# gau-nernst/llama-x

Hardware: AMD Instinct MI355X
Metric: train tokens/sec Llama-3.1-8B seq4096 at 1/2/4/8 MI355X; p50 step ms (higher is better)
Workload: dtype bf16; 1 GPU; Llama-3.1-8B text-only LoRA r=16 bf16, seq=4096, 1 sequence per GPU, causal mask, base+LM head frozen (BASELINE.json configs[1]); random-init weights at 8B dimensions; seq_len=4096, parallelism=dp1, launch=hipGraph replay (fwd+bwd+AdamW), lm_head_rows=labelled only

## Files before the change

### include/llx.h

```cpp
#ifndef LLX_H
#define LLX_H

#include <stdint.h>

#ifdef __cplusplus
extern "C" {
#endif

typedef void* llx_stream_t;

int llx_version(void);
const char* llx_last_error_string(void);
int llx_device_info(int device, char* name, int len);

int llx_rmsnorm_fwd(const void* x, const void* w, void* y, float* rstd, int64_t rows, int64_t dim, float eps, llx_stream_t s);
int llx_rmsnorm_fwd_quant(const void* x, const void* w, void* y, float* rstd, void* q, int64_t ldq, void* qscale, int64_t rows, int64_t dim,
                          float eps, llx_stream_t s);
int64_t llx_rmsnorm_bwd_workspace_bytes(int64_t rows, int64_t dim);
int llx_rmsnorm_bwd(const void* dy, const void* x, const void* w, const float* rstd, void* dx, void* dw ,
                    int dw_accumulate, void* workspace, const void* dres ,
                    int64_t rows, int64_t dim, llx_stream_t s);

int llx_gemm_nt_bf16(const void* A, int64_t lda, const void* B, int64_t ldb, void* C, int64_t ldc, int64_t M, int64_t N, int64_t K,
                     const void* A2, int64_t lda2, const void* B2, int64_t ldb2, int64_t K2, int epilogue, const void* E, int64_t lde,
                     llx_stream_t s);
int llx_gemm_nt_bf16_rows(const void* A, int64_t lda, const void* B, int64_t ldb, void* C, int64_t ldc, int64_t M, int64_t N, int64_t K,
                          const void* A2, int64_t lda2, const void* B2, int64_t ldb2, int64_t K2, int epilogue, const void* E, int64_t lde,
                          const int32_t* m_valid, llx_stream_t s);
int llx_gemm_nt_bf16_splitk(const void* A, int64_t lda, const void* B, int64_t ldb, float* partial, int64_t M, int64_t N, int64_t K, int splits,
                            const int32_t* m_valid, llx_stream_t s);
int llx_splitk_combine(const float* partial, int splits, int64_t M, int64_t N, const int32_t* inv, const float* scale, void* out, int64_t ld_out,
                       llx_stream_t s);
int llx_gemm_nt_bf16_rope(const void* A, int64_t lda, const void* B, int64_t ldb, void* C, int64_t ldc, int64_t M, int64_t N, int64_t K,
                          const void* A2, int64_t lda2, const void* B2, int64_t ldb2, int64_t K2, const float* rope_table, int64_t rope_S,
                          int64_t rope_cols, llx_stream_t s);

int llx_gemm_tn_bf16(const void* A, int64_t lda, const void* B, int64_t ldb, void* C, int64_t ldc, int64_t M, int64_t N1, int64_t N2,
                     llx_stream_t s);
int llx_gemm_tn_bf16_rows(const void* A, int64_t lda, const void* B, int64_t ldb, void* C, int64_t ldc, int64_t M, int64_t N1, int64_t N2,
                          const int32_t* m_valid, llx_stream_t s);

int llx_int8_mm_dequant(const void* A, int64_t lda, const void* B, int64_t ldb, void* C, int64_t ldc, int64_t M, int64_t N, int64_t K,
                        const void* a_scale, const void* b_scale, llx_stream_t s);
int llx_int8_mm_dequant_f32(const void* A, int64_t lda, const void* B, int64_t ldb, float* C, int64_t ldc, int64_t M, int64_t N, int64_t K,
                            const float* a_scale, const float* b_scale, llx_stream_t s);
int llx_int8_mm_dequant_ext(const void* A, int64_t lda, const void* B, int64_t ldb, void* C, int64_t ldc, int64_t M, int64_t N, int64_t K,
                            const void* a_scale, const void* b_scale, const void* A2, int64_t lda2, const void* B2, int64_t ldb2, int64_t K2,
                            int epilogue, const void* E, int64_t lde, const float* rope_table, int64_t rope_S, int64_t rope_cols,
                            llx_stream_t s);

int llx_quantize_int8_rowwise(const void* x, int64_t ldx, void* q, int64_t ldq, void* scale, int64_t rows, int64_t cols, int is_f32,
                              llx_stream_t s);

int64_t llx_attn_flags_bytes(int64_t B, int64_t S);
int llx_attn_tile_flags(const int* doc_ids, const int* prefix_len, void* flags, int64_t B, int64_t S, llx_stream_t s);
int llx_attn_fwd(const void* q, int64_t q_sb, int64_t q_ss, const void* k, int64_t k_sb, int64_t k_ss, const void* v, int64_t v_sb,
                 int64_t v_ss, void* o, int64_t o_sb, int64_t o_ss, float* lse, const int* doc_ids, const int* prefix_len,
                 const void* flags, int64_t B, int64_t S, int64_t H, int64_t KVH, int64_t head_dim, float scale, llx_stream_t s);
int64_t llx_attn_bwd_workspace_bytes(int64_t B, int64_t S, int64_t H, int64_t KVH);
int64_t llx_attn_bwd_ds_bytes(int64_t B, int64_t S, int64_t H);
int llx_attn_bwd(const void* q, int64_t q_sb, int64_t q_ss, const void* k, int64_t k_sb, int64_t k_ss, const void* v, int64_t v_sb,
                 int64_t v_ss, const void* o, int64_t o_sb, int64_t o_ss, const void* d_o, int64_t do_sb, int64_t do_ss, const float* lse,
                 float* delta , void* dq, int64_t dq_sb, int64_t dq_ss, void* dk, int64_t dk_sb, int64_t dk_ss,
                 void* dv, int64_t dv_sb, int64_t dv_ss, const int* doc_ids, const int* prefix_len, const void* flags,
                 const float* rope ,
                 void* ds ,
                 int64_t B, int64_t S, int64_t H, int64_t KVH, int64_t head_dim, float scale, llx_stream_t s);

int llx_attn_fwd_dropout(const void* q, int64_t q_sb, int64_t q_ss, const void* k, int64_t k_sb, int64_t k_ss, const void* v, int64_t v_sb,
                         int64_t v_ss, void* o, int64_t o_sb, int64_t o_ss, float* lse, const int* doc_ids, const int* prefix_len,
                         const void* flags, int64_t B, int64_t S, int64_t H, int64_t KVH, int64_t head_dim, float scale, int64_t threshold,
                         const void* rng, int64_t stream_id, llx_stream_t s);
int llx_attn_bwd_dropout(const void* q, int64_t q_sb, int64_t q_ss, const void* k, int64_t k_sb, int64_t k_ss, const void* v, int64_t v_sb,
                         int64_t v_ss, const void* o, int64_t o_sb, int64_t o_ss, const void* d_o, int64_t do_sb, int64_t do_ss,
                         const float* lse, float* delta, void* dq, int64_t dq_sb, int64_t dq_ss, void* dk, int64_t dk_sb, int64_t dk_ss,
                         void* dv, int64_t dv_sb, int64_t dv_ss, const int* doc_ids, const int* prefix_len, const void* flags,
                         const float* rope, void* ds, int64_t B, int64_t S, int64_t H, int64_t KVH, int64_t head_dim, float scale,
                         int64_t threshold, const void* rng, int64_t stream_id, llx_stream_t s);
int llx_attn_dropout_keep(void* keep, int64_t B, int64_t H, int64_t Sq, int64_t Skv, int64_t threshold, const void* rng, int64_t stream_id,
                          llx_stream_t s);

int llx_attn_dense_fwd(const void* q, int64_t q_sb, int64_t q_sh, int64_t q_ss, const void* k, int64_t k_sb, int64_t k_sh, int64_t k_ss,
                       const void* v, int64_t v_sb, int64_t v_sh, int64_t v_ss, void* o, int64_t o_sb, int64_t o_sh, int64_t o_ss,
                       const void* mask, int64_t m_sb, int64_t m_sh, int64_t m_sq, int64_t B, int64_t H, int64_t KVH, int64_t Sq, int64_t Skv,
                       int64_t head_dim, float scale, llx_stream_t s);

int64_t llx_attn_mask_flags_bytes(int64_t B, int64_t Sq, int64_t Skv);
int llx_attn_mask_tile_flags(const void* mask, int64_t m_sb, int64_t m_sq, void* flags, int64_t B, int64_t Sq, int64_t Skv, llx_stream_t s);
int llx_attn_mask_fwd(const void* q, int64_t q_sb, int64_t q_ss, const void* k, int64_t k_sb, int64_t k_sh, int64_t k_ss, const void* v,
                      int64_t v_sb, int64_t v_sh, int64_t v_ss, void* o, int64_t o_sb, int64_t o_ss, float* lse ,
                      const void* mask, int64_t m_sb, int64_t m_sq, const void* flags, int64_t B, int64_t Sq, int64_t Skv, int64_t H,
                      int64_t KVH, int64_t head_dim, float scale, llx_stream_t s);

int llx_attn_mask_bwd(const void* q, int64_t q_sb, int64_t q_ss, const void* k, int64_t k_sb, int64_t k_ss, const void* v, int64_t v_sb,
                      int64_t v_ss, const void* o, int64_t o_sb, int64_t o_ss, const void* d_o, int64_t do_sb, int64_t do_ss,
                      const float* lse, float* delta , void* dq, int64_t dq_sb,
                      int64_t dq_ss, void* dk, int64_t dk_sb, int64_t dk_ss, void* dv, int64_t dv_sb, int64_t dv_ss, const void* mask,
                      int64_t m_sb, int64_t m_sq, const void* flags, const float* rope , int64_t B,
                      int64_t S, int64_t H, int64_t KVH, int64_t head_dim, float scale, llx_stream_t s);

int llx_gemv_bf16(const void* w0, int64_t ldw0, int64_t n0, const void* w1, int64_t ldw1, int64_t n1, const void* w2, int64_t ldw2, int64_t n2,
                  const void* x, int64_t ldx, int64_t M, int64_t K, const void* norm_w, float eps, int epilogue, void* out, int64_t ldo,
                  const void* res, int64_t ldr, const float* rope, int64_t n_q, int64_t n_k, void* k_cache, void* v_cache, int64_t c_sh,
                  int64_t c_ss, const int64_t* input_pos, const void* bext0, const void* bext1, const void* bext2, int64_t rank0, int64_t rank1,
                  int64_t rank2, const void* t, int64_t ldt, float lora_scale, llx_stream_t s);
int llx_gemv_i8(const void* w0, int64_t ldw0, int64_t n0, const void* w1, int64_t ldw1, int64_t n1, const void* w2, int64_t ldw2, int64_t n2,
                const void* x, int64_t ldx, int64_t M, int64_t K, const void* norm_w, float eps, int epilogue, void* out, int64_t ldo,
                const void* res, int64_t ldr, const float* rope, int64_t n_q, int64_t n_k, void* k_cache, void* v_cache, int64_t c_sh,
// ... 19 lines not shown
                         int64_t c_sh, int64_t c_ss, int64_t Smax, const int64_t* pos, void* workspace, int64_t workspace_bytes, llx_stream_t s);
int64_t llx_gemm_rows16_i8_workspace_bytes(int64_t M, int64_t N, int64_t K, int epilogue);
int llx_gemm_rows16_i8(const void* w0, int64_t ldw0, int64_t n0, const void* w1, int64_t ldw1, int64_t n1, const void* w2, int64_t ldw2, int64_t n2,
                       const void* x, int64_t ldx, int64_t M, int64_t K, const void* norm_w, float eps, int epilogue, void* out, int64_t ldo,
                       const void* res, int64_t ldr, const float* rope, int64_t n_q, int64_t n_k, void* k_cache, void* v_cache, int64_t c_sb,
                       int64_t c_sh, int64_t c_ss, int64_t Smax, const int64_t* pos, void* workspace, int64_t workspace_bytes,
                       const void* scale0, const void* scale1, const void* scale2, llx_stream_t s);
int llx_gemm_rows16_bf16_lora(const void* w0, int64_t ldw0, int64_t n0, const void* w1, int64_t ldw1, int64_t n1, const void* w2, int64_t ldw2,
                              int64_t n2, const void* x, int64_t ldx, int64_t M, int64_t K, const void* norm_w, float eps, int epilogue, void* out,
                              int64_t ldo, const void* res, int64_t ldr, const float* rope, int64_t n_q, int64_t n_k, void* k_cache, void* v_cache,
                              int64_t c_sb, int64_t c_sh, int64_t c_ss, int64_t Smax, const int64_t* pos, void* workspace, int64_t workspace_bytes,
                              const void* bext0, const void* bext1, const void* bext2, int64_t rank0, int64_t rank1, int64_t rank2, const void* t,
                              int64_t ldt, float lora_scale, const void* colscale0, const void* colscale1, const void* colscale2, llx_stream_t s);
int llx_gemm_rows16_i8_lora(const void* w0, int64_t ldw0, int64_t n0, const void* w1, int64_t ldw1, int64_t n1, const void* w2, int64_t ldw2,
                            int64_t n2, const void* x, int64_t ldx, int64_t M, int64_t K, const void* norm_w, float eps, int epilogue, void* out,
                            int64_t ldo, const void* res, int64_t ldr, const float* rope, int64_t n_q, int64_t n_k, void* k_cache, void* v_cache,
                            int64_t c_sb, int64_t c_sh, int64_t c_ss, int64_t Smax, const int64_t* pos, void* workspace, int64_t workspace_bytes,
                            const void* scale0, const void* scale1, const void* scale2, const void* bext0, const void* bext1, const void* bext2,
                            int64_t rank0, int64_t rank1, int64_t rank2, const void* t, int64_t ldt, float lora_scale, llx_stream_t s);
int64_t llx_attn_decode_workspace_bytes(int64_t B, int64_t H, int64_t M, int64_t nsplit);
int llx_attn_decode(const void* q, int64_t q_sb, int64_t q_sh, int64_t q_ss, const void* k_cache, const void* v_cache, int64_t c_sb, int64_t c_sh,
                    int64_t c_ss, void* o, int64_t o_sb, int64_t o_sh, int64_t o_ss, const void* mask, int64_t m_sb, int64_t m_sh, int64_t m_sq,
                    const int* extent, float* workspace, int64_t B, int64_t H, int64_t KVH, int64_t M, int64_t Skv, int64_t nsplit,
                    int64_t head_dim, float scale, llx_stream_t s);

int llx_rope(const void* x, int64_t x_sb, int64_t x_ss, void* y, int64_t y_sb, int64_t y_ss, const float* table, int64_t B, int64_t S,
             int64_t nheads, int64_t head_dim, int backward, llx_stream_t s);

int llx_swiglu_fwd(const void* g, int64_t g_ld, const void* u, int64_t u_ld, void* h, int64_t h_ld, int64_t rows, int64_t cols, llx_stream_t s);
int llx_swiglu_bwd(const void* dh, int64_t dh_ld, const void* g, int64_t g_ld, const void* u, int64_t u_ld, void* dg, int64_t dg_ld,
                   void* du, int64_t du_ld, int64_t rows, int64_t cols, llx_stream_t s);

int llx_embedding_fwd(const int64_t* ids, const void* table, void* out, int64_t n_tok, int64_t dim, int64_t vocab, int64_t tok_per_batch,
                      int64_t out_sb, int64_t out_ss, llx_stream_t s);
int llx_embedding_bwd(const int64_t* ids, const void* dy, float* dtable_f32, int64_t n_tok, int64_t dim, int64_t vocab,
                      int64_t tok_per_batch, int64_t dy_sb, int64_t dy_ss, llx_stream_t s);

int64_t llx_ce_workspace_bytes(int64_t T);
int llx_ce_fwd_bwd(const void* logits, int64_t ld, void* dlogits, int64_t dld, const int64_t* labels, float* loss, void* workspace,
                   int64_t T, int64_t V, llx_stream_t s);
int llx_head_compact_index(const int64_t* labels, int32_t* idx, int32_t* inv, int64_t* labels_c, int32_t* count, int64_t T, llx_stream_t s);
int llx_gather_rows(const void* src, int64_t ld_src, const int32_t* idx, const int32_t* count, void* dst, int64_t ld_dst, int64_t T, int64_t D,
                    llx_stream_t s);
int llx_scatter_rows(const void* src, int64_t ld_src, const int32_t* inv, const float* scale , void* dst, int64_t ld_dst,
                     int64_t T, int64_t D, llx_stream_t s);
int llx_ce_fwd_bwd_rows(const void* logits, int64_t ld, void* dlogits, int64_t dld, const int64_t* labels, float* loss, void* workspace,
                        int64_t T, int64_t V, const int32_t* rows, llx_stream_t s);
int llx_ce_fwd_bwd_part(const void* logits, int64_t ld, void* dlogits, int64_t dld, const int64_t* labels, float* loss, void* workspace, int64_t T,
                        int64_t V, int64_t row0, int64_t nrows, const int32_t* rows, int phase, llx_stream_t s);

int llx_logprob_rows_fwd(const void* logits, int64_t ld, const int64_t* labels, float* logp, float* lse, int32_t* top1 ,
                         int64_t T, int64_t V, const int32_t* rows , llx_stream_t s);
int llx_logprob_rows_bwd(const void* logits, int64_t ld, void* dlogits, int64_t dld, const int64_t* labels, const float* lse, const float* g,
                         int64_t T, int64_t V, const int32_t* rows , llx_stream_t s);
int llx_logprob_map_rows(const int32_t* map, const float* src_f, float* dst_f, float fill_f, const int32_t* src_i ,
                         int32_t* dst_i , int32_t fill_i, int64_t T, llx_stream_t s);

int llx_skinny_nt(const void* X, int64_t ldx, const void* W, int64_t ldw, void* out, int64_t M, int64_t K, int64_t R,
                  const int32_t* kranges , llx_stream_t s);
int llx_skinny_nt_scaled(const void* X, int64_t ldx, const void* W, int64_t ldw, void* out, int64_t M, int64_t K, int64_t R,
                         const int32_t* kranges, const void* colscale, void* G, int64_t ldg, llx_stream_t s);
int llx_rmsnorm_skinny_nt(const void* x, const void* g, const void* W, int64_t ldw, void* y, float* rstd, void* t, int64_t M, int64_t D,
                          int64_t R, float eps, llx_stream_t s);
int64_t llx_skinny_tn_workspace_bytes(int64_t M, int64_t N, int64_t R);
int llx_skinny_tn(const void* U, const void* Y, int64_t ldy, void* out, int64_t out_ld, int64_t M, int64_t N, int64_t R, float scale,
                  int transpose_out, int accumulate, void* workspace,
                  const int32_t* segs , int seg_count, llx_stream_t s);
int llx_skinny_tn_partial(const void* U, const void* Y, int64_t ldy, int64_t M, int64_t N, int64_t R, void* workspace, const int32_t* segs,
                          int seg_count, llx_stream_t s);
int llx_skinny_tn_partial_many(int n, const void* const* U, const void* const* Y, const int64_t* ldy, const int64_t* M, const int64_t* N,
                               const int64_t* R, void* const* workspaces, const int32_t* const* segs, const int* seg_count, llx_stream_t s);
int64_t llx_skinny_u_workspace_bytes(int64_t M, int64_t N);
int llx_skinny_tn_partial_many_u(int n, const void* const* U, const void* const* Y, const int64_t* ldy, const int64_t* M, const int64_t* N,
                                 const int64_t* R, void* const* workspaces, const int32_t* const* segs, const int* seg_count,
                                 const void* const* Bt, const int64_t* ldb, void* const* upart, llx_stream_t s);
int llx_skinny_u_reduce(const void* upart, void* out, int64_t M, int64_t N, int64_t R, const int32_t* segs, int seg_count, llx_stream_t s);
int llx_skinny_tn_partial_many_us(int n, const void* const* U, const void* const* Y, const int64_t* ldy, const int64_t* M, const int64_t* N,
                                  const int64_t* R, void* const* workspaces, const int32_t* const* segs, const int* seg_count,
                                  const void* const* Bt, const int64_t* ldb, void* const* upart, const void* const* colscale,
                                  void* const* G, const int64_t* ldg, llx_stream_t s);
int llx_skinny_tn_reduce_many(int n, const void* const* workspaces, void* const* outs, const int64_t* out_ld, const int64_t* M, const int64_t* N,
                              const int64_t* R, const float* scale, const int* transpose_out, const int* accumulate,
                              const int32_t* const* segs, const int* seg_count, llx_stream_t s);
int llx_pad64(const void* in, int64_t ld, void* out, int64_t R, int64_t C, float scale, int transpose, llx_stream_t s);
int llx_lora_group_pack(const void* const* lora_a, const void* const* lora_b, const int64_t* Ns, const int64_t* ranks, int nm, int64_t K,
                        float scale, void* a_cat, void* b2, void* bT, void* a2t, llx_stream_t s);
int llx_lora_groups_pack(const void* const* lora_a, const void* const* lora_b, const int64_t* Ns, const int64_t* ranks, const int* nm,
                         const int64_t* K, const float* scale, void* const* a_cat, void* const* b2, void* const* bT, void* const* a2t, int ng,
                         llx_stream_t s);
int llx_lora_pack(const void* in, int64_t ld, void* out, int64_t out_ld, int64_t R, int64_t C, int64_t row_off, int64_t col_off, float scale,
                  int transpose, llx_stream_t s);

int llx_rownorm2(const void* W, int64_t ld, float* out, int64_t rows, int64_t cols, llx_stream_t s);
int llx_dora_colscale(const float* wn2, const void* G , const void* b2 , const void* AAt ,
                      const void* m , void* c , float* inv_norm , int64_t N, int64_t R, llx_stream_t s);
int64_t llx_colsum_mul_workspace_bytes(int64_t N);
int llx_colsum_mul(const void* a, int64_t lda, const void* b, int64_t ldb, const float* colscale , void* out ,
                   void* workspace, int64_t M, int64_t N, llx_stream_t s);
int llx_colscale_bias(const void* x, int64_t x_ld, void* y, int64_t y_ld, const void* colscale , const void* bias ,
                      int64_t rows, int64_t cols, llx_stream_t s);

int llx_mel_spectrogram(const float* audio, int64_t B, int64_t L, const float* twiddle, const float* window, const float* fbank, float* mel,
                        int64_t n_frames, int64_t hop, int64_t n_mels, llx_stream_t s);
int llx_logmel_cmn(const float* mel, void* feat , int64_t B, int64_t n_frames, int64_t n_mels, llx_stream_t s);
int llx_gelu_fwd(const void* z, int64_t z_ld, void* y, int64_t y_ld, int64_t rows, int64_t cols, llx_stream_t s);
int llx_gelu_bwd(const void* dy, int64_t dy_ld, const void* z, int64_t z_ld, void* dz, int64_t dz_ld, int64_t rows, int64_t cols, llx_stream_t s);
int llx_col2im3(const void* dA, void* dpad, int64_t M, int64_t C, int64_t P, int64_t stride, llx_stream_t s);
int llx_conv_w_reorder(const void* in, void* out, int64_t D, int64_t C, int to_gemm, llx_stream_t s);

int llx_sample_rows(const void* logits, int dtype, int64_t ld, int64_t R, int64_t V, float temperature, int64_t top_k, float top_p,
                    uint64_t seed, int64_t* pos, int64_t* token_out, int64_t* history, int64_t hist_ld, int64_t hist_cap, int64_t hist_base,
                    int advance, int64_t eos_id, int32_t* finished, float* aux_u, float* aux_thresh, int32_t* aux_kept, llx_stream_t s);

int llx_sample_rows_ext(const void* logits, int dtype, int64_t ld, int64_t R, int64_t V, float temperature, int64_t top_k, float top_p,
                        uint64_t seed, int64_t* pos, int64_t* token_out, int64_t* history, int64_t hist_ld, int64_t hist_cap, int64_t hist_base,
                        int advance, int64_t eos_id, int32_t* finished, float* aux_u, float* aux_thresh, int32_t* aux_kept, int32_t* counts,
                        int64_t ldc, float repetition_penalty, float presence_penalty, float frequency_penalty, float* logprob_history,
                        llx_stream_t s);

int llx_lookup_step(const int64_t* picks, int64_t* seq, int64_t cap, int64_t* len, int64_t* step_tok, int64_t* step_pos, int32_t* finished,
                    int64_t* counters, int64_t P, int64_t n, int k, int g, int64_t eos_id, int init, llx_stream_t s);

int llx_beam_rows(const void* logits, int dtype, int64_t ld, int64_t W, int64_t V, float* cand_score, int32_t* cand_token, llx_stream_t s);
int llx_beam_merge(const float* cand_score, const int32_t* cand_token, float* s, int32_t* parent, int64_t* tok, int64_t* hist, int64_t hist_ld,
                   int64_t* bank_tok, int64_t bank_ld, int32_t* bank_len, float* bank_score, int32_t* meta, int64_t W, int64_t n,
                   int64_t eos_id, float length_penalty, int init, llx_stream_t stream);
int llx_kv_reorder_rows(const void* const* table, int64_t n_caches, int64_t sb, int64_t sh, int64_t ss, const int32_t* parent, int64_t W,
                        int64_t KVH, int64_t len, int64_t Smax, int64_t head_dim, llx_stream_t s);

int llx_scale(const void* x, int64_t x_ld, void* y, int64_t y_ld, const float* dev_scalar, float host_scale, const void* colscale,
              int64_t rows, int64_t cols, llx_stream_t s);
int llx_add(const void* x, const void* y, void* z, int64_t n, llx_stream_t s);
int llx_transpose(const void* in, int64_t in_ld, void* out, int64_t out_ld, int64_t R, int64_t C, int src_is_i8, llx_stream_t s);
int llx_i8_to_bf16(const void* in, void* out, int64_t n, llx_stream_t s);

#ifdef __cplusplus
}
#endif
#endif
```

### llama-x_amd/csrc/common.h

```cpp
#pragma once
#include <hip/hip_runtime.h>
#include <stdint.h>
#include <stdarg.h>
#include <stdio.h>

#define LLX_OK 0
#define LLX_ERR_ARG -1
#define LLX_ERR_LAUNCH -2
#define LLX_ERR_UNSUPPORTED -3

void llx_set_error(const char* fmt, ...);

#define LLX_REQUIRE(cond, ...)            \
  do {                                    \
    if (!(cond)) {                        \
      llx_set_error(__VA_ARGS__);         \
      return LLX_ERR_ARG;                 \
    }                                     \
  } while (0)

#define LLX_LAUNCH_CHECK(name)                                              \
  do {                                                                      \
    hipError_t e__ = hipGetLastError();                                     \
    if (e__ != hipSuccess) {                                                \
// ... 110 lines not shown
      const float uu = p ? bfhi(uv[e]) : bflo(uv[e]);
      const float dd = p ? bfhi(dv[e]) : bflo(dv[e]);
      const float sg = sigmoidf_(gg);
      const float silu = bf2f(f2bf(gg * sg));
      dus[p] = dd * silu;
      const float ds = bf2f(f2bf(dd * uu));
      dgs[p] = ds * (sg * (1.f + gg * (1.f - sg)));
    }
    og[e] = pack_bf2(dgs[0], dgs[1]);
    ou[e] = pack_bf2(dus[0], dus[1]);
  }
}

__device__ __forceinline__ u32x4_t rope8(const u32x4_t& v, const f32x4_t& t0, const f32x4_t& t1, float sign) {
  const float cs[4] = {t0[0], t0[2], t1[0], t1[2]};
  const float sn[4] = {t0[1] * sign, t0[3] * sign, t1[1] * sign, t1[3] * sign};
  u32x4_t o;
#pragma unroll
  for (int e = 0; e < 4; ++e) {
    const float x0 = bflo(v[e]), x1 = bfhi(v[e]);
    o[e] = pack_bf2(x0 * cs[e] - x1 * sn[e], x1 * cs[e] + x0 * sn[e]);
  }
  return o;
}

__device__ __forceinline__ u32x4_t rope8(const u32x4_t& v, const float* __restrict__ tp, float sign) {
  const f32x4_t t0 = *reinterpret_cast<const f32x4_t*>(tp);
  const f32x4_t t1 = *reinterpret_cast<const f32x4_t*>(tp + 4);
  const float cs[4] = {t0[0], t0[2], t1[0], t1[2]};
  const float sn[4] = {t0[1] * sign, t0[3] * sign, t1[1] * sign, t1[3] * sign};
  u32x4_t o;
#pragma unroll
  for (int e = 0; e < 4; ++e) {
    const float x0 = bflo(v[e]), x1 = bfhi(v[e]);
    o[e] = pack_bf2(x0 * cs[e] - x1 * sn[e], x1 * cs[e] + x0 * sn[e]);
  }
  return o;
}

typedef __attribute__((ext_vector_type(8))) short llx_s16x8_t;
template <int OFF>
__device__ __forceinline__ void lds_tr_read(s16x4_t& dst, uint32_t addr) {
  asm volatile("ds_read_b64_tr_b16 %0, %1 offset:%2" : "=v"(dst) : "v"(addr), "n"(OFF));
}
__device__ __forceinline__ void lds_tr_read_rt(s16x4_t& dst, uint32_t addr, int off) {
  asm volatile("ds_read_b64_tr_b16 %0, %1 offset:%2" : "=v"(dst) : "v"(addr), "n"(off));
}
template <int N>
__device__ __forceinline__ void lds_tr_wait4(s16x4_t& a, s16x4_t& b, s16x4_t& c, s16x4_t& d) {
  asm volatile("s_waitcnt lgkmcnt(%4)" : "+v"(a), "+v"(b), "+v"(c), "+v"(d) : "n"(N));
  __builtin_amdgcn_sched_barrier(0);
}
template <int N>
__device__ __forceinline__ void lds_tr_wait8(s16x4_t (&c)[4], s16x4_t (&d)[4]) {
  asm volatile("s_waitcnt lgkmcnt(%8)" : "+v"(c[0]), "+v"(c[1]), "+v"(c[2]), "+v"(c[3]), "+v"(d[0]), "+v"(d[1]), "+v"(d[2]), "+v"(d[3]) : "n"(N));
  __builtin_amdgcn_sched_barrier(0);
}
__device__ __forceinline__ void lds_read16_rt(i32x4_t& dst, uint32_t addr, int off) {
  asm volatile("ds_read_b128 %0, %1 offset:%2" : "=v"(dst) : "v"(addr), "n"(off));
}
template <typename T>
__device__ __forceinline__ void lds_pin1(T& x) { asm volatile("" : "+v"(x)); }
template <typename T, int N>
__device__ __forceinline__ void lds_pin1(T (&x)[N]) {
#pragma unroll
  for (int i = 0; i < N; ++i) asm volatile("" : "+v"(x[i]));
}
template <typename... T>
__device__ __forceinline__ void lds_pin(T&... x) {
  (lds_pin1(x), ...);
  __builtin_amdgcn_sched_barrier(0);
}
template <int N, typename... T>
__device__ __forceinline__ void lds_wait(T&... x) {
  asm volatile("s_waitcnt lgkmcnt(%0)" : : "n"(N));
  (lds_pin1(x), ...);
  __builtin_amdgcn_sched_barrier(0);
}
__device__ __forceinline__ bf16x8_t frag_of(const s16x4_t& lo, const s16x4_t& hi) {
  const llx_s16x8_t v = {lo[0], lo[1], lo[2], lo[3], hi[0], hi[1], hi[2], hi[3]};
  return __builtin_bit_cast(bf16x8_t, v);
}

typedef __attribute__((address_space(3))) void llx_lds_void;
__device__ __forceinline__ __amdgpu_buffer_rsrc_t lds_dma_rsrc(const void* base, uint32_t bytes) {
  return __builtin_amdgcn_make_buffer_rsrc(const_cast<void*>(base), 0, (int)bytes, 0x00020000);
}
__device__ __forceinline__ void lds_dma16(__amdgpu_buffer_rsrc_t rsrc, llx_lds_void* dst, uint32_t lane_off, uint32_t wave_off) {
  __builtin_amdgcn_raw_ptr_buffer_load_lds(rsrc, dst, 16, (int)lane_off, (int)wave_off, 0, 0);
}
```

### llama-x_amd/csrc/gemm_bf16.hip

```cpp
#include "common.h"
#include <type_traits>
#include <mutex>

#define BM 256
#define BN 256
#define BK 64
#define STAGE_BYTES (2 * 256 * BK * 2)
#define A_TILE_BYTES (256 * BK * 2)
#define EPI_ROW_BYTES 528
#define GEMM_LDS_BYTES (256 * EPI_ROW_BYTES)

enum { EPI_NONE = 0, EPI_RESIDUAL = 1, EPI_BIAS = 2, EPI_BIAS_GELU = 3, EPI_COLSCALE = 4, EPI_ROWCOLSCALE = 5, EPI_SWIGLU_BWD = 6, EPI_SWIGLU_FWD = 7, EPI_ROPE = 8, EPI_SPLITK = 9, EPI_ROWCOLSCALE_F32 = 10 };

struct GemmArgs {
  const bf16_t* A; const bf16_t* B; bf16_t* C;
  const bf16_t* A2; const bf16_t* B2;
  const bf16_t* E;
  const bf16_t* E2;
  int64_t lda, ldb, ldc, lde, lda2, ldb2;
  int M, N, K, K2;
  int grid_m, grid_n;
  int col0, col_end;
  const bf16_t* sa; const bf16_t* sb;
  const float* rope;
  int rope_S, rope_cols;
  const int* m_valid;
  float* C32;
  int splits;
};

typedef __attribute__((address_space(3))) void lds_void;
typedef const __attribute__((address_space(1))) void gbl_void;

__device__ __forceinline__ float gelu_erf(float x) { return 0.5f * x * (1.0f + erff(x * 0.70710678118654752440f)); }

template <int EPI, bool I8, int PIPE, int BNT = 256>
__global__ __launch_bounds__(512, 2) void gemm_nt_kernel(const GemmArgs g) {
  static_assert(BNT == 256 || BNT == 128, "tile width");
  static_assert(PIPE == 1, "the four-phase main loop is the only one");
  static_assert(BNT == 256 || EPI != EPI_SWIGLU_FWD, "the SwiGLU-forward epilogue needs the full tile");
  constexpr int ESZ = I8 ? 1 : 2;
  constexpr int TK = 128 / ESZ;
  constexpr int WNG = BNT / 64;
  constexpr int WR = 256 / (8 / WNG);
  constexpr int MI = WR / 16;
  constexpr int MH = MI / 2;
  constexpr int BSI = BNT / 64;
  constexpr int EROW = BNT * 2 + 16;
  extern __shared__ __attribute__((aligned(16))) char smem[];
  const int tid = threadIdx.x;
  const int lane = tid & 63;
  const int wave = __builtin_amdgcn_readfirstlane(tid >> 6);
  const int wm = wave / WNG, wn = wave % WNG;

  int grid_m = g.grid_m;
  if (g.m_valid != nullptr) grid_m = min(grid_m, (*g.m_valid + BM - 1) / BM);
  const int nsplit = EPI == EPI_SPLITK ? g.splits : 1;
  const int nwg = grid_m * g.grid_n * nsplit;
  int bid = blockIdx.x;
  if (bid >= nwg) return;
  {
    const int q = nwg >> 3, r = nwg & 7, x = bid & 7;
    bid = (x < r ? x * (q + 1) : r * (q + 1) + (x - r) * q) + (bid >> 3);
  }
  const int split = EPI == EPI_SPLITK ? bid / (grid_m * g.grid_n) : 0;
  if constexpr (EPI == EPI_SPLITK) bid -= split * (grid_m * g.grid_n);
  const int GROUP_M = 4;
  const int width = GROUP_M * g.grid_n;
  const int group = bid / width;
  const int gsz = min(grid_m - group * GROUP_M, GROUP_M);
  const int pid_m = group * GROUP_M + ((bid % width) % gsz);
  const int pid_n = (bid % width) / gsz;
  constexpr bool SPLITN = EPI == EPI_SWIGLU_FWD;
  const int halfN = g.N >> 1;
  const int m0 = pid_m * BM, n0 = SPLITN ? pid_n * (BN / 2) : g.col0 + pid_n * BNT;
  auto col_of = [&](int nl) { return SPLITN ? (nl < BN / 2 ? n0 + nl : halfN + n0 + nl - BN / 2) : min(n0 + nl, g.col_end - 1); };

  const int srow = tid >> 3;
  const int schunk = (tid & 7) ^ ((tid >> 4) & 7);
  int arow[4], brow[4];
#pragma unroll
  for (int i = 0; i < 4; ++i) {
    arow[i] = min(m0 + i * 64 + srow, g.M - 1);
    brow[i] = SPLITN ? (i < 2 ? n0 + i * 64 + srow : halfN + n0 + (i - 2) * 64 + srow) : min(n0 + (i % BSI) * 64 + srow, g.col_end - 1);
  }
  const int nk1 = g.K / TK / nsplit;
  const int nk = nk1 + g.K2 / 64;
  const int kofs = split * nk1;

  uint32_t aoff[4], boff[4];
#pragma unroll
  for (int i = 0; i < 4; ++i) {
    aoff[i] = (uint32_t)((int64_t)arow[i] * g.lda * ESZ + schunk * 16);
    boff[i] = (uint32_t)((int64_t)brow[i] * g.ldb * ESZ + schunk * 16);
  }
  const __amdgpu_buffer_rsrc_t rsA = lds_dma_rsrc(g.A, (uint32_t)(((int64_t)(g.M - 1) * g.lda + g.K) * ESZ));
  const __amdgpu_buffer_rsrc_t rsB = lds_dma_rsrc(g.B, (uint32_t)(((int64_t)(g.N - 1) * g.ldb + g.K) * ESZ));

  const int frow = lane & 15;
  const int fsw = (lane >> 1) & 7;
  const int fq = lane >> 4;
  const int a_base = (wm * WR + frow) * 128;
  const int b_base = (wn * 64 + frow) * 128;
  const int slot0 = ((0 * 4 + fq) ^ fsw) * 16;
  const int slot1 = ((1 * 4 + fq) ^ fsw) * 16;
  const uint32_t sbase = (uint32_t)(uintptr_t)(__attribute__((address_space(3))) char*)smem;
  const uint32_t fa0 = sbase + a_base + slot0, fa1 = sbase + a_base + slot1;
  const uint32_t fb0 = sbase + A_TILE_BYTES + b_base + slot0, fb1 = sbase + A_TILE_BYTES + b_base + slot1;
  constexpr bool EARLY_AHI = !I8;

  using acc_t = typename std::conditional<I8, i32x4_t, f32x4_t>::type;
  acc_t acc[MI][4];
#pragma unroll
  for (int i = 0; i < MI; ++i)
#pragma unroll
    for (int j = 0; j < 4; ++j) acc[i][j] = acc_t{0, 0, 0, 0};

  auto stage_q = [&](auto steady_tag, int kt, int which) {
    constexpr bool steady = decltype(steady_tag)::value;
    if constexpr (!steady) {
      if (kt >= nk) return;
    }
    const int half = which >> 1, hi = which & 1;
    const int np = half ? BSI / 2 : 2;
    char* sT = smem + (kt & 1) * STAGE_BYTES + half * A_TILE_BYTES + hi * np * 8192;
    if (steady || kt < nk1) {
      const uint32_t koff = (uint32_t)(kt + kofs) * 128;
#pragma unroll
      for (int j = 0; j < 2; ++j) {
        if (j < np) {
          if (half) lds_dma16(rsB, (llx_lds_void*)(sT + (j * 512 + wave * 64) * 16), boff[np * hi + j], koff);
          else lds_dma16(rsA, (llx_lds_void*)(sT + (j * 512 + wave * 64) * 16), aoff[2 * hi + j], koff);
        }
      }
    } else {
      const char* base = (const char*)(half ? g.B2 : g.A2) + (int64_t)(kt - nk1) * 128;
      const int64_t l = (half ? g.ldb2 : g.lda2) * 2;
#pragma unroll
      for (int j = 0; j < 2; ++j) {
        if (j < np) {
          const char* src = base + (int64_t)(half ? brow[np * hi + j] : arow[2 * hi + j]) * l + schunk * 16;
          __builtin_amdgcn_global_load_lds((gbl_void*)src, (lds_void*)(sT + (j * 512 + wave * 64) * 16), 16, 0, 0);
        }
      }
    }
  };
  auto mfma_t = [&](auto ext_tag, const i32x4_t& b, const i32x4_t& a, acc_t& c) {
    constexpr bool ext_phase = decltype(ext_tag)::value;
    if constexpr (I8) {
      if constexpr (ext_phase) {
        f32x4_t cf = __builtin_bit_cast(f32x4_t, c);
        cf = __builtin_amdgcn_mfma_f32_16x16x32_bf16(__builtin_bit_cast(bf16x8_t, b), __builtin_bit_cast(bf16x8_t, a), cf, 0, 0, 0);
        c = __builtin_bit_cast(acc_t, cf);
      } else {
        c = __builtin_amdgcn_mfma_i32_16x16x64_i8(b, a, c, 0, 0, 0);
      }
// ... 96 lines not shown
    if constexpr (!EARLY_AHI) {
#pragma unroll
      for (int m4 = 0; m4 < MH; ++m4) lds_read16_rt(af[0][m4], pa0, (MH + m4) * 16 * 128);
    }
#pragma unroll
    for (int m4 = 0; m4 < MH; ++m4) lds_read16_rt(af[1][m4], pa1, (MH + m4) * 16 * 128);
    __builtin_amdgcn_s_setprio(1);
    lds_wait<MH>(ah);
#pragma unroll
    for (int m4 = 0; m4 < MH; ++m4)
#pragma unroll
      for (int n2 = 0; n2 < 2; ++n2) mfma(bfr[0][2 + n2], ah[m4], acc[MH + m4][2 + n2]);
    pin_acc(MH, 2);
    lds_wait<0>(af[1]);
#pragma unroll
    for (int m4 = 0; m4 < MH; ++m4)
#pragma unroll
      for (int n2 = 0; n2 < 2; ++n2) mfma(bfr[1][2 + n2], af[1][m4], acc[MH + m4][2 + n2]);
    __builtin_amdgcn_s_setprio(0);
    asm volatile("" ::: "memory");
    __builtin_amdgcn_s_barrier();
    asm volatile("" ::: "memory");
    stage_q(steady_tag, kt + 2, 0);
    __builtin_amdgcn_s_setprio(1);
#pragma unroll
    for (int ks = 0; ks < 2; ++ks)
#pragma unroll
      for (int m4 = 0; m4 < MH; ++m4)
#pragma unroll
        for (int n2 = 0; n2 < 2; ++n2) mfma(bfr[ks][n2], ks ? af[1][m4] : ah[m4], acc[MH + m4][n2]);
    __builtin_amdgcn_s_setprio(0);
  };
  const int nk_main = I8 ? nk1 : nk;
  int kt = 0;
#pragma unroll 1
  for (; kt + 2 < nk1; ++kt) ktile(kt, std::false_type{}, std::true_type{});
#pragma unroll 1
  for (; kt < nk_main; ++kt) ktile(kt, std::false_type{}, std::false_type{});
  if constexpr (I8) {
    if (nk > nk1) {
      dequant_in_place();
      for (kt = nk1; kt < nk; ++kt) ktile(kt, std::true_type{}, std::false_type{});
    }
  }
  __syncthreads();

  if constexpr (EPI == EPI_SPLITK) {
    float* P = g.C32 + (int64_t)split * g.M * g.N;
#pragma unroll
    for (int mi = 0; mi < MI; ++mi) {
      const int gm = m0 + wm * WR + mi * 16 + frow;
#pragma unroll
      for (int ni = 0; ni < 4; ++ni) {
        const int gn = n0 + wn * 64 + ni * 16 + fq * 4;
        if (gm < g.M && gn < g.col_end) *reinterpret_cast<f32x4_t*>(P + (int64_t)gm * g.N + gn) = acc[mi][ni];
      }
    }
    return;
  }
  if constexpr (EPI == EPI_ROWCOLSCALE_F32) {
    static_assert(I8, "int8 kernel only");
    float* Cf = reinterpret_cast<float*>(g.C);
    const float* saf = reinterpret_cast<const float*>(g.sa);
    const float* sbf = reinterpret_cast<const float*>(g.sb);
#pragma unroll
    for (int mi = 0; mi < MI; ++mi) {
      const int gm = m0 + wm * WR + mi * 16 + frow;
      const float rs = saf[min(gm, g.M - 1)];
#pragma unroll
      for (int ni = 0; ni < 4; ++ni) {
        const int gn = n0 + wn * 64 + ni * 16 + fq * 4;
        if (gm < g.M && gn < g.col_end) {
          const f32x4_t cs = *reinterpret_cast<const f32x4_t*>(sbf + gn);
          f32x4_t c;
#pragma unroll
          for (int e = 0; e < 4; ++e) c[e] = ((float)acc[mi][ni][e] * rs) * cs[e];
          *reinterpret_cast<f32x4_t*>(Cf + (int64_t)gm * g.ldc + gn) = c;
        }
      }
    }
    return;
  }
  constexpr int NIT = BNT / 16;
  constexpr int EB0 = (EPI == EPI_SWIGLU_BWD || EPI == EPI_ROPE) ? 4 : 8;
  constexpr int EB = EB0 < NIT / 2 ? EB0 : NIT / 2;
  constexpr bool AUX = EPI == EPI_RESIDUAL || EPI == EPI_BIAS || EPI == EPI_BIAS_GELU || EPI == EPI_SWIGLU_BWD || EPI == EPI_ROPE || EPI == EPI_COLSCALE;
  auto load_aux = [&](int it0, u32x4_t (&aux0)[EB], u32x4_t (&aux1)[EB]) {
    if constexpr (AUX) {
#pragma unroll
      for (int j = 0; j < EB; ++j) {
        const int q = (it0 + j) * 512 + tid;
        const int row = q / (BNT / 8), cc = q % (BNT / 8);
        const int gmc = min(m0 + row, g.M - 1), gnc = min(n0 + cc * 8, g.col_end - 8);
        if constexpr (EPI == EPI_RESIDUAL) {
          aux0[j] = *reinterpret_cast<const u32x4_t*>(g.E + (int64_t)gmc * g.lde + gnc);
        } else if constexpr (EPI == EPI_SWIGLU_BWD) {
          aux0[j] = *reinterpret_cast<const u32x4_t*>(g.E + (int64_t)gmc * g.lde + gnc);
          aux1[j] = *reinterpret_cast<const u32x4_t*>(g.E + (int64_t)gmc * g.lde + g.N + gnc);
        } else if constexpr (EPI == EPI_ROPE) {
          const float* tp = g.rope + ((int64_t)(gmc % g.rope_S) * 64 + ((gnc & 127) >> 1)) * 2;
          aux0[j] = *reinterpret_cast<const u32x4_t*>(tp);
          aux1[j] = *reinterpret_cast<const u32x4_t*>(tp + 4);
        } else {
          aux0[j] = *reinterpret_cast<const u32x4_t*>(g.E + gnc);
        }
      }
    }
  };
  u32x4_t auxA0[EB], auxA1[EB], auxB0[EB], auxB1[EB];
  if constexpr (!SPLITN) load_aux(0, auxA0, auxA1);
  float sbv[4][4], rsv[MI];
  if constexpr (I8) {
    if (g.K2 <= 0) {
#pragma unroll
      for (int ni = 0; ni < 4; ++ni)
#pragma unroll
        for (int e = 0; e < 4; ++e) sbv[ni][e] = bf2f(g.sb[col_of(wn * 64 + ni * 16 + fq * 4 + e)]);
#pragma unroll
      for (int mi = 0; mi < MI; ++mi) rsv[mi] = bf2f(g.sa[min(m0 + wm * WR + mi * 16 + frow, g.M - 1)]);
    }
  }
#pragma unroll
  for (int mi = 0; mi < MI; ++mi) {
    const int m = wm * WR + mi * 16 + frow;
    float rs = 1.f;
    if constexpr (I8) rs = rsv[mi];
#pragma unroll
    for (int ni = 0; ni < 4; ++ni) {
      const int n = wn * 64 + ni * 16 + fq * 4;
      float c[4];
      if constexpr (I8) {
        if (g.K2 > 0) {
          const f32x4_t cf = __builtin_bit_cast(f32x4_t, acc[mi][ni]);
#pragma unroll
          for (int e = 0; e < 4; ++e) c[e] = cf[e];
        } else {
#pragma unroll
          for (int e = 0; e < 4; ++e) c[e] = ((float)acc[mi][ni][e] * rs) * sbv[ni][e];
        }
      } else {
#pragma unroll
        for (int e = 0; e < 4; ++e) c[e] = acc[mi][ni][e];
      }
      u32x2_t pk;
      pk[0] = pack_bf2(c[0], c[1]);
      pk[1] = pack_bf2(c[2], c[3]);
      *reinterpret_cast<u32x2_t*>(smem + m * EROW + n * 2) = pk;
    }
  }
  __syncthreads();
  if constexpr (SPLITN) {
    bf16_t* H = const_cast<bf16_t*>(g.E);
#pragma unroll 4
    for (int it = 0; it < 8; ++it) {
      const int q = it * 512 + tid;
      const int row = q >> 4, cc = q & 15;
      const int gm = m0 + row, gn = n0 + cc * 8;
      if (gm < g.M) {
        const u32x4_t gv = *reinterpret_cast<const u32x4_t*>(smem + row * EPI_ROW_BYTES + cc * 16);
        const u32x4_t uv = *reinterpret_cast<const u32x4_t*>(smem + row * EPI_ROW_BYTES + (cc + 16) * 16);
        *reinterpret_cast<u32x4_t*>(g.C + (int64_t)gm * g.ldc + gn) = gv;
        *reinterpret_cast<u32x4_t*>(g.C + (int64_t)gm * g.ldc + halfN + gn) = uv;
        *reinterpret_cast<u32x4_t*>(H + (int64_t)gm * g.lde + gn) = swiglu_fwd8(gv, uv);
      }
    }
    return;
  }
  auto combine = [&](int it0, const u32x4_t (&aux0)[EB], const u32x4_t (&aux1)[EB]) {
#pragma unroll
    for (int j = 0; j < EB; ++j) {
      const int q = (it0 + j) * 512 + tid;
      const int row = q / (BNT / 8), cc = q % (BNT / 8);
      const int gm = m0 + row, gn = n0 + cc * 8;
      if (gm < g.M && gn < g.col_end) {
        u32x4_t v = *reinterpret_cast<const u32x4_t*>(smem + row * EROW + cc * 16);
        if constexpr (EPI == EPI_RESIDUAL) {
          const u32x4_t r = aux0[j];
#pragma unroll
          for (int e = 0; e < 4; ++e) v[e] = pack_bf2(bflo(v[e]) + bflo(r[e]), bfhi(v[e]) + bfhi(r[e]));
        } else if constexpr (EPI == EPI_BIAS || EPI == EPI_BIAS_GELU) {
          const u32x4_t bb = aux0[j];
#pragma unroll
          for (int e = 0; e < 4; ++e) {
            float lo = bflo(v[e]) + bflo(bb[e]), hi = bfhi(v[e]) + bfhi(bb[e]);
            if constexpr (EPI == EPI_BIAS_GELU) {
              lo = gelu_erf(bf2f(f2bf(lo)));
              hi = gelu_erf(bf2f(f2bf(hi)));
            }
            v[e] = pack_bf2(lo, hi);
          }
        } else if constexpr (EPI == EPI_SWIGLU_BWD) {
          u32x4_t og, ou;
          swiglu_bwd8(v, aux0[j], aux1[j], og, ou);
          *reinterpret_cast<u32x4_t*>(g.C + (int64_t)gm * g.ldc + g.N + gn) = ou;
          v = og;
        } else if constexpr (EPI == EPI_ROPE) {
          if (gn < g.rope_cols) v = rope8(v, __builtin_bit_cast(f32x4_t, aux0[j]), __builtin_bit_cast(f32x4_t, aux1[j]), 1.f);
        } else if constexpr (EPI == EPI_COLSCALE) {
          const u32x4_t sc = aux0[j];
#pragma unroll
          for (int e = 0; e < 4; ++e) v[e] = pack_bf2(bflo(v[e]) * bflo(sc[e]), bfhi(v[e]) * bfhi(sc[e]));
        }
        *reinterpret_cast<u32x4_t*>(g.C + (int64_t)gm * g.ldc + gn) = v;
      }
    }
  };
  static_assert((NIT / EB) % 2 == 0, "the batches alternate between two register sets");
#pragma unroll 1
  for (int it0 = 0; it0 < NIT; it0 += 2 * EB) {
    load_aux(it0 + EB, auxB0, auxB1);
    combine(it0, auxA0, auxA1);
    if (it0 + 2 * EB < NIT) load_aux(it0 + 2 * EB, auxA0, auxA1);
    combine(it0 + EB, auxB0, auxB1);
  }
}

template <int EPI, bool I8, int BNT = 256>
static int launch_gemm_p(const GemmArgs& a, hipStream_t stream) {
  auto kern = gemm_nt_kernel<EPI, I8, 1, BNT>;
  static std::once_flag attr_once;
  static hipError_t attr_err = hipSuccess;
  std::call_once(attr_once, [&] { attr_err = hipFuncSetAttribute((const void*)kern, hipFuncAttributeMaxDynamicSharedMemorySize, GEMM_LDS_BYTES); });
  if (attr_err != hipSuccess) {
    llx_set_error("llx_gemm_nt_bf16: cannot raise dynamic LDS limit: %s", hipGetErrorString(attr_err));
    return LLX_ERR_LAUNCH;
  }
  hipLaunchKernelGGL(kern, dim3(a.grid_m * a.grid_n * (EPI == EPI_SPLITK ? a.splits : 1)), dim3(512), GEMM_LDS_BYTES, stream, a);
  LLX_LAUNCH_CHECK("llx_gemm_nt_bf16");
  return LLX_OK;
}

template <int EPI, bool I8 = false>
static int launch_gemm(const GemmArgs& a, hipStream_t stream) {
  if constexpr (EPI != EPI_SWIGLU_FWD) {
    const int tiles = a.grid_m * a.grid_n, tail = tiles % 256;
    if (a.col0 == 0 && a.col_end == a.N && a.N % 256 == 0 && tiles > 256 && tail > 0 && tail <= 128 && tail % a.grid_m == 0) {
      const int tail_cols = tail / a.grid_m * 256;
      GemmArgs full = a, half = a;
      full.col_end = a.N - tail_cols;
      full.grid_n = a.grid_n - tail / a.grid_m;
      half.col0 = a.N - tail_cols;
      half.grid_n = tail_cols / 128;
      const int rc = launch_gemm_p<EPI, I8, 256>(full, stream);
      if (rc != LLX_OK) return rc;
      return launch_gemm_p<EPI, I8, 128>(half, stream);
    }
  }
  return launch_gemm_p<EPI, I8>(a, stream);
}

static GemmArgs make_args(const void* A, int64_t lda, const void* B, int64_t ldb, void* C, int64_t ldc, int64_t M, int64_t N, int64_t K) {
  GemmArgs a = {};
  a.A = (const bf16_t*)A; a.B = (const bf16_t*)B; a.C = (bf16_t*)C;
  a.lda = lda; a.ldb = ldb; a.ldc = ldc;
  a.M = (int)M; a.N = (int)N; a.K = (int)K;
  a.grid_m = (int)cdiv64(M, BM); a.grid_n = (int)cdiv64(N, BN);
  a.col_end = (int)N;
  a.splits = 1;
  return a;
}

static int check_extent(const char* who, int64_t M, int64_t N, int64_t K, int64_t lda, int64_t ldb, int esz) {
  LLX_REQUIRE(M < (1 << 30) && N < (1 << 30) && K < (1 << 30), "%s: dimension too large", who);
  LLX_REQUIRE(M * lda * esz < (int64_t)4294967296 && N * ldb * esz < (int64_t)4294967296, "%s: operand larger than 4 GiB (32-bit tile offsets)", who);
  return LLX_OK;
}

static int gemm_nt_bf16_impl(const void* A, int64_t lda, const void* B, int64_t ldb, void* C, int64_t ldc, int64_t M,
                             int64_t N, int64_t K, const void* A2, int64_t lda2, const void* B2, int64_t ldb2, int64_t K2,
                             int epilogue, const void* E, int64_t lde, const float* rope, int64_t rope_S, int64_t rope_cols,
                             hipStream_t stream, const int32_t* m_valid = nullptr) {
  LLX_REQUIRE(A && B && C, "llx_gemm_nt_bf16: null pointer");
  LLX_REQUIRE(M > 0 && N > 0 && K > 0, "llx_gemm_nt_bf16: empty problem M=%lld N=%lld K=%lld", (long long)M, (long long)N, (long long)K);
  LLX_REQUIRE(K % BK == 0 && K2 % BK == 0, "llx_gemm_nt_bf16: K=%lld and K2=%lld must be multiples of 64", (long long)K, (long long)K2);
  LLX_REQUIRE(N % 8 == 0, "llx_gemm_nt_bf16: N=%lld must be a multiple of 8", (long long)N);
  LLX_REQUIRE(lda % 8 == 0 && ldb % 8 == 0 && ldc % 8 == 0, "llx_gemm_nt_bf16: row strides must be multiples of 8 elements");
  LLX_REQUIRE(((uintptr_t)A | (uintptr_t)B | (uintptr_t)C) % 16 == 0, "llx_gemm_nt_bf16: pointers must be 16-byte aligned");
  LLX_REQUIRE(K2 == 0 || (A2 && B2 && lda2 % 8 == 0 && ldb2 % 8 == 0 && ((uintptr_t)A2 | (uintptr_t)B2) % 16 == 0),
              "llx_gemm_nt_bf16: bad K-extension operands");
  LLX_REQUIRE(epilogue == EPI_NONE || epilogue == EPI_ROPE || (E && (uintptr_t)E % 16 == 0), "llx_gemm_nt_bf16: epilogue operand missing/unaligned");
  LLX_REQUIRE(epilogue != EPI_ROPE || (rope && (uintptr_t)rope % 16 == 0 && rope_S > 0 && rope_cols >= 0 && rope_cols <= N && rope_cols % 128 == 0),
              "llx_gemm_nt_bf16_rope: need an aligned fp32 table, rope_S > 0 and rope_cols a multiple of 128 within N");
  LLX_REQUIRE((epilogue != EPI_RESIDUAL && epilogue != EPI_SWIGLU_BWD) || lde % 8 == 0, "llx_gemm_nt_bf16: residual / gate|up stride must be a multiple of 8");
  LLX_REQUIRE(epilogue != EPI_SWIGLU_BWD || (lde >= 2 * N && ldc >= 2 * N), "llx_gemm_nt_bf16: the SwiGLU-backward epilogue reads E[M,2N] (gate|up) and writes C[M,2N] (dg|du)");
  if (const int rc = check_extent("llx_gemm_nt_bf16", M, N, K, lda, ldb, 2); rc != LLX_OK) return rc;
  GemmArgs a = make_args(A, lda, B, ldb, C, ldc, M, N, K);
  a.A2 = (const bf16_t*)A2; a.B2 = (const bf16_t*)B2; a.lda2 = lda2; a.ldb2 = ldb2; a.K2 = (int)K2;
  a.E = (const bf16_t*)E; a.lde = lde;
  a.rope = rope; a.rope_S = (int)rope_S; a.rope_cols = (int)rope_cols;
  a.m_valid = m_valid;
  switch (epilogue) {
    case EPI_NONE: return launch_gemm<EPI_NONE>(a, stream);
    case EPI_RESIDUAL: return launch_gemm<EPI_RESIDUAL>(a, stream);
    case EPI_BIAS: return launch_gemm<EPI_BIAS>(a, stream);
    case EPI_BIAS_GELU: return launch_gemm<EPI_BIAS_GELU>(a, stream);
    case EPI_COLSCALE: return launch_gemm<EPI_COLSCALE>(a, stream);
    case EPI_SWIGLU_BWD: return launch_gemm<EPI_SWIGLU_BWD>(a, stream);
    case EPI_ROPE: return launch_gemm<EPI_ROPE>(a, stream);
    case EPI_SWIGLU_FWD:
      LLX_REQUIRE(N % 256 == 0 && lde % 8 == 0, "llx_gemm_nt_bf16: the SwiGLU-forward epilogue needs N = 2I with I a multiple of 128");
      a.grid_n = (int)(N / 256);
      return launch_gemm<EPI_SWIGLU_FWD>(a, stream);
    default: llx_set_error("llx_gemm_nt_bf16: unknown epilogue %d", epilogue); return LLX_ERR_UNSUPPORTED;
  }
}

extern "C" int llx_gemm_nt_bf16(const void* A, int64_t lda, const void* B, int64_t ldb, void* C, int64_t ldc, int64_t M,
                                int64_t N, int64_t K, const void* A2, int64_t lda2, const void* B2, int64_t ldb2, int64_t K2,
                                int epilogue, const void* E, int64_t lde, hipStream_t stream) {
  LLX_REQUIRE(epilogue != EPI_ROPE, "llx_gemm_nt_bf16: the RoPE epilogue is llx_gemm_nt_bf16_rope");
  return gemm_nt_bf16_impl(A, lda, B, ldb, C, ldc, M, N, K, A2, lda2, B2, ldb2, K2, epilogue, E, lde, nullptr, 0, 0, stream);
}

extern "C" int llx_gemm_nt_bf16_rows(const void* A, int64_t lda, const void* B, int64_t ldb, void* C, int64_t ldc, int64_t M,
                                     int64_t N, int64_t K, const void* A2, int64_t lda2, const void* B2, int64_t ldb2, int64_t K2,
                                     int epilogue, const void* E, int64_t lde, const int32_t* m_valid, hipStream_t stream) {
  LLX_REQUIRE(epilogue != EPI_ROPE, "llx_gemm_nt_bf16_rows: the RoPE epilogue is llx_gemm_nt_bf16_rope");
  LLX_REQUIRE(m_valid && (uintptr_t)m_valid % 4 == 0, "llx_gemm_nt_bf16_rows: m_valid must be a device int32 pointer");
  return gemm_nt_bf16_impl(A, lda, B, ldb, C, ldc, M, N, K, A2, lda2, B2, ldb2, K2, epilogue, E, lde, nullptr, 0, 0, stream, m_valid);
}

extern "C" int llx_gemm_nt_bf16_splitk(const void* A, int64_t lda, const void* B, int64_t ldb, float* partial, int64_t M, int64_t N,
                                       int64_t K, int splits, const int32_t* m_valid, hipStream_t stream) {
  LLX_REQUIRE(A && B && partial, "llx_gemm_nt_bf16_splitk: null pointer");
  LLX_REQUIRE(M > 0 && N > 0 && K > 0 && splits >= 1 && splits <= 16, "llx_gemm_nt_bf16_splitk: bad sizes");
  LLX_REQUIRE(K % ((int64_t)BK * splits) == 0, "llx_gemm_nt_bf16_splitk: K=%lld must be a multiple of 64 * splits (%d)", (long long)K, splits);
  LLX_REQUIRE(N % 8 == 0 && lda % 8 == 0 && ldb % 8 == 0, "llx_gemm_nt_bf16_splitk: N and the row strides must be multiples of 8");
  LLX_REQUIRE(((uintptr_t)A | (uintptr_t)B | (uintptr_t)partial) % 16 == 0, "llx_gemm_nt_bf16_splitk: pointers must be 16-byte aligned");
  if (const int rc = check_extent("llx_gemm_nt_bf16_splitk", M, N, K, lda, ldb, 2); rc != LLX_OK) return rc;
  LLX_REQUIRE(m_valid == nullptr || (uintptr_t)m_valid % 4 == 0, "llx_gemm_nt_bf16_splitk: m_valid must be a device int32 pointer");
  GemmArgs a = make_args(A, lda, B, ldb, nullptr, N, M, N, K);
  a.m_valid = m_valid;
  a.C32 = partial; a.splits = splits;
  return launch_gemm_p<EPI_SPLITK, false>(a, stream);
}

__global__ __launch_bounds__(256) void splitk_combine_kernel(const float* __restrict__ partial, int splits, int64_t MN, const int32_t* __restrict__ inv,
                                                             const float* __restrict__ scale, bf16_t* __restrict__ out, int64_t ldo, int N) {
  const int i = blockIdx.x, j = inv ? inv[i] : i;
  const float sc = scale ? scale[0] : 1.f;
  for (int c = threadIdx.x; c < (N >> 2); c += 256) {
    u32x2_t o = {0u, 0u};
    if (j >= 0) {
      f32x4_t v = *reinterpret_cast<const f32x4_t*>(partial + (int64_t)j * N + c * 4);
      for (int s2 = 1; s2 < splits; ++s2) {
        const f32x4_t w = *reinterpret_cast<const f32x4_t*>(partial + s2 * MN + (int64_t)j * N + c * 4);
#pragma unroll
        for (int e = 0; e < 4; ++e) v[e] += w[e];
      }
      if (scale) {
#pragma unroll
        for (int e = 0; e < 4; ++e) v[e] = bf2f(f2bf(v[e])) * sc;
      }
      o[0] = pack_bf2(v[0], v[1]);
      o[1] = pack_bf2(v[2], v[3]);
    }
    *reinterpret_cast<u32x2_t*>(out + (int64_t)i * ldo + c * 4) = o;
  }
}

extern "C" int llx_splitk_combine(const float* partial, int splits, int64_t M, int64_t N, const int32_t* inv, const float* scale, void* out,
                                  int64_t ld_out, hipStream_t stream) {
  LLX_REQUIRE(partial && out, "llx_splitk_combine: null pointer");
  LLX_REQUIRE(M > 0 && N > 0 && N % 4 == 0 && ld_out % 4 == 0 && splits >= 1 && splits <= 16, "llx_splitk_combine: bad sizes");
  LLX_REQUIRE(((uintptr_t)partial) % 16 == 0 && ((uintptr_t)out) % 8 == 0, "llx_splitk_combine: unaligned pointer");
  hipLaunchKernelGGL(splitk_combine_kernel, dim3((unsigned)M), dim3(256), 0, stream, partial, splits, M * N, inv, scale, (bf16_t*)out, ld_out, (int)N);
  LLX_LAUNCH_CHECK("llx_splitk_combine");
  return LLX_OK;
}

extern "C" int llx_gemm_nt_bf16_rope(const void* A, int64_t lda, const void* B, int64_t ldb, void* C, int64_t ldc, int64_t M, int64_t N,
                                     int64_t K, const void* A2, int64_t lda2, const void* B2, int64_t ldb2, int64_t K2,
                                     const float* rope_table, int64_t rope_S, int64_t rope_cols, hipStream_t stream) {
  return gemm_nt_bf16_impl(A, lda, B, ldb, C, ldc, M, N, K, A2, lda2, B2, ldb2, K2, EPI_ROPE, nullptr, 0, rope_table, rope_S, rope_cols, stream);
}

extern "C" int llx_int8_mm_dequant(const void* A, int64_t lda, const void* B, int64_t ldb, void* C, int64_t ldc, int64_t M, int64_t N,
                                   int64_t K, const void* a_scale, const void* b_scale, hipStream_t stream) {
  LLX_REQUIRE(A && B && C && a_scale && b_scale, "llx_int8_mm_dequant: null pointer");
  LLX_REQUIRE(M > 0 && N > 0 && K > 0, "llx_int8_mm_dequant: empty problem");
  LLX_REQUIRE(K % 128 == 0, "llx_int8_mm_dequant: K=%lld must be a multiple of 128", (long long)K);
  LLX_REQUIRE(N % 8 == 0 && ldc % 8 == 0, "llx_int8_mm_dequant: N and ldc must be multiples of 8");
  LLX_REQUIRE(lda % 16 == 0 && ldb % 16 == 0, "llx_int8_mm_dequant: int8 row strides must be multiples of 16");
  LLX_REQUIRE(((uintptr_t)A | (uintptr_t)B | (uintptr_t)C) % 16 == 0, "llx_int8_mm_dequant: pointers must be 16-byte aligned");
  if (const int rc = check_extent("llx_int8_mm_dequant", M, N, K, lda, ldb, 1); rc != LLX_OK) return rc;
  GemmArgs a = make_args(A, lda, B, ldb, C, ldc, M, N, K);
  a.sa = (const bf16_t*)a_scale; a.sb = (const bf16_t*)b_scale;
  return launch_gemm<EPI_ROWCOLSCALE, true>(a, stream);
}

extern "C" int llx_int8_mm_dequant_f32(const void* A, int64_t lda, const void* B, int64_t ldb, float* C, int64_t ldc, int64_t M, int64_t N,
                                       int64_t K, const float* a_scale, const float* b_scale, hipStream_t stream) {
  LLX_REQUIRE(A && B && C && a_scale && b_scale, "llx_int8_mm_dequant_f32: null pointer");
  LLX_REQUIRE(M > 0 && N > 0 && K > 0, "llx_int8_mm_dequant_f32: empty problem");
// ... 40 lines not shown
```

### llama-x_amd/csrc/skinny.hip

```cpp
#include "common.h"

typedef __attribute__((address_space(3))) s16x4_t lds_s16x4;
typedef __attribute__((ext_vector_type(8))) short s16x8_t;

#define SK_PAD 64

#define SNT_WAVES 8
#define SNT_UNROLL 8

struct SkinnyRanges { int lo[4], hi[4]; };

__device__ __forceinline__ void snt_scaled_store(const bf16x8_t& a, const bf16_t* cs, bf16_t* g) {
  const u32x4_t x = __builtin_bit_cast(u32x4_t, a);
  const u32x4_t c = *reinterpret_cast<const u32x4_t*>(cs);
  u32x4_t o;
#pragma unroll
  for (int e = 0; e < 4; ++e) o[e] = pack_bf2(bflo(x[e]) * bflo(c[e]), bfhi(x[e]) * bfhi(c[e]));
  *reinterpret_cast<u32x4_t*>(g) = o;
}

template <int NB, bool RANGED, bool SCALE = false>
__global__ __launch_bounds__(SNT_WAVES * 64) void skinny_nt_kernel(const bf16_t* __restrict__ X, int64_t ldx, const bf16_t* __restrict__ W,
                                                                   int64_t ldw, bf16_t* __restrict__ out, int M, int K, int R, SkinnyRanges kr,
                                                                   const bf16_t* __restrict__ cs = nullptr, bf16_t* __restrict__ G = nullptr,
                                                                   int64_t ldg = 0) {
  constexpr int SNT_UNROLL_ = NB == 4 ? 4 : SNT_UNROLL;
  __shared__ float part[SNT_WAVES][16][SK_PAD];
  const int lane = threadIdx.x & 63;
  const int wave = __builtin_amdgcn_readfirstlane(threadIdx.x >> 6);
  const int m0 = blockIdx.x * 16;
  const int fr = lane & 15, fq = lane >> 4;
  const bf16_t* xrow = X + (int64_t)min(m0 + fr, M - 1) * ldx;
  const bf16_t* wrow[NB];
#pragma unroll
  for (int nb = 0; nb < NB; ++nb) wrow[nb] = W + (int64_t)min(nb * 16 + fr, R - 1) * ldw;
  f32x4_t acc[NB];
#pragma unroll
  for (int nb = 0; nb < NB; ++nb) acc[nb] = f32x4_t{0.f, 0.f, 0.f, 0.f};
  const int npairs = K >> 6;
  const int rounds = npairs / ((SNT_UNROLL_ / 2) * SNT_WAVES);
  const int rot = rounds > 0 ? (int)((blockIdx.x * 7u + (blockIdx.x >> 3)) % (unsigned)rounds) : 0;
  for (int it0 = 0; it0 < rounds; ++it0) {
    const int it = (it0 + rot < rounds) ? it0 + rot : it0 + rot - rounds;
    const int pr = it * (SNT_UNROLL_ / 2) * SNT_WAVES + wave;
    bf16x8_t a[SNT_UNROLL_], b[SNT_UNROLL_][NB];
#pragma unroll
    for (int u = 0; u < SNT_UNROLL_; ++u) a[u] = *reinterpret_cast<const bf16x8_t*>(xrow + (pr + (u >> 1) * SNT_WAVES) * 64 + 16 * fq + 8 * (u & 1));
    if constexpr (SCALE) {
      if (m0 + fr < M) {
#pragma unroll
        for (int u = 0; u < SNT_UNROLL_; ++u) {
          const int k = (pr + (u >> 1) * SNT_WAVES) * 64 + 16 * fq + 8 * (u & 1);
          snt_scaled_store(a[u], cs + k, G + (int64_t)(m0 + fr) * ldg + k);
        }
      }
    }
#pragma unroll
    for (int u = 0; u < SNT_UNROLL_; ++u) {
      const int k0 = (pr + (u >> 1) * SNT_WAVES) * 64;
#pragma unroll
      for (int nb = 0; nb < NB; ++nb)
        if (!RANGED || (k0 >= kr.lo[nb] && k0 < kr.hi[nb])) b[u][nb] = *reinterpret_cast<const bf16x8_t*>(wrow[nb] + k0 + 16 * fq + 8 * (u & 1));
    }
#pragma unroll
    for (int u = 0; u < SNT_UNROLL_; ++u) {
      const int k0 = (pr + (u >> 1) * SNT_WAVES) * 64;
#pragma unroll
      for (int nb = 0; nb < NB; ++nb)
        if (!RANGED || (k0 >= kr.lo[nb] && k0 < kr.hi[nb])) acc[nb] = __builtin_amdgcn_mfma_f32_16x16x32_bf16(a[u], b[u][nb], acc[nb], 0, 0, 0);
    }
  }
  const int nks = K >> 5;
  {
    const int pr_done = rounds * (SNT_UNROLL_ / 2) * SNT_WAVES;
    for (int ks = 2 * pr_done + wave; ks < nks; ks += SNT_WAVES) {
      const bf16x8_t a = *reinterpret_cast<const bf16x8_t*>(xrow + ks * 32 + 8 * fq);
      if constexpr (SCALE) {
        if (m0 + fr < M) snt_scaled_store(a, cs + ks * 32 + 8 * fq, G + (int64_t)(m0 + fr) * ldg + ks * 32 + 8 * fq);
      }
#pragma unroll
      for (int nb = 0; nb < NB; ++nb) {
        if (RANGED && (ks * 32 < kr.lo[nb] || ks * 32 >= kr.hi[nb])) continue;
        const bf16x8_t b = *reinterpret_cast<const bf16x8_t*>(wrow[nb] + ks * 32 + 8 * fq);
        acc[nb] = __builtin_amdgcn_mfma_f32_16x16x32_bf16(a, b, acc[nb], 0, 0, 0);
      }
    }
  }
#pragma unroll
  for (int nb = 0; nb < NB; ++nb)
#pragma unroll
    for (int e = 0; e < 4; ++e) part[wave][fq * 4 + e][nb * 16 + fr] = acc[nb][e];
  __syncthreads();
  const int row = threadIdx.x >> 5, c0 = (threadIdx.x & 31) * 2;
  if (m0 + row < M) {
    float v[2];
#pragma unroll
    for (int e = 0; e < 2; ++e) {
      const int c = c0 + e;
      float s = 0.f;
      if (c < NB * 16 && c < R) {
#pragma unroll
        for (int w = 0; w < SNT_WAVES; ++w) s += part[w][row][c];
      }
      v[e] = s;
    }
    *reinterpret_cast<uint32_t*>(out + (int64_t)(m0 + row) * SK_PAD + c0) = pack_bf2(v[0], v[1]);
  }
}

extern "C" int llx_skinny_nt(const void* X, int64_t ldx, const void* W, int64_t ldw, void* out, int64_t M, int64_t K, int64_t R,
                             const int32_t* kranges, hipStream_t stream) {
  LLX_REQUIRE(X && W && out, "llx_skinny_nt: null pointer");
  LLX_REQUIRE(M > 0 && K > 0 && K % 32 == 0 && R > 0 && R <= 64, "llx_skinny_nt: need K%%32==0 and 0<R<=64 (K=%lld R=%lld)", (long long)K, (long long)R);
  LLX_REQUIRE(ldx % 8 == 0 && ldw % 8 == 0 && ((uintptr_t)X | (uintptr_t)W) % 16 == 0 && (uintptr_t)out % 8 == 0, "llx_skinny_nt: alignment");
  const dim3 grid((unsigned)cdiv64(M, 16)), block(SNT_WAVES * 64);
  const int nb = (int)cdiv64(R, 16);
  SkinnyRanges kr;
  for (int i = 0; i < 4; ++i) {
    kr.lo[i] = kranges ? kranges[2 * i] : 0;
    kr.hi[i] = kranges ? kranges[2 * i + 1] : (int)K;
    LLX_REQUIRE(kr.lo[i] % 64 == 0 && (kr.hi[i] % 64 == 0 || kr.hi[i] == (int)K) && kr.lo[i] >= 0 && kr.hi[i] <= (int)K,
                "llx_skinny_nt: k range %d of a block-diagonal W must be a multiple of 64 inside [0, K]", i);
  }
#define L(N, RG) hipLaunchKernelGGL((skinny_nt_kernel<N, RG>), grid, block, 0, stream, (const bf16_t*)X, ldx, (const bf16_t*)W, ldw, (bf16_t*)out, (int)M, (int)K, (int)R, kr)
  if (kranges) { if (nb == 1) L(1, true); else if (nb == 2) L(2, true); else L(4, true); }
  else { if (nb == 1) L(1, false); else if (nb == 2) L(2, false); else L(4, false); }
#undef L
  LLX_LAUNCH_CHECK("llx_skinny_nt");
  return LLX_OK;
}

extern "C" int llx_skinny_nt_scaled(const void* X, int64_t ldx, const void* W, int64_t ldw, void* out, int64_t M, int64_t K, int64_t R,
                                    const int32_t* kranges, const void* colscale, void* G, int64_t ldg, hipStream_t stream) {
  LLX_REQUIRE(X && W && out && colscale && G, "llx_skinny_nt_scaled: null pointer");
  LLX_REQUIRE(M > 0 && K > 0 && K % 32 == 0 && R > 0 && R <= 64, "llx_skinny_nt_scaled: need K%%32==0 and 0<R<=64 (K=%lld R=%lld)", (long long)K, (long long)R);
  LLX_REQUIRE(ldx % 8 == 0 && ldw % 8 == 0 && ldg % 8 == 0 && ((uintptr_t)X | (uintptr_t)W | (uintptr_t)colscale | (uintptr_t)G) % 16 == 0 && (uintptr_t)out % 8 == 0,
              "llx_skinny_nt_scaled: alignment");
  const dim3 grid((unsigned)cdiv64(M, 16)), block(SNT_WAVES * 64);
  const int nb = (int)cdiv64(R, 16);
  SkinnyRanges kr;
  for (int i = 0; i < 4; ++i) {
    kr.lo[i] = kranges ? kranges[2 * i] : 0;
    kr.hi[i] = kranges ? kranges[2 * i + 1] : (int)K;
    LLX_REQUIRE(kr.lo[i] % 64 == 0 && (kr.hi[i] % 64 == 0 || kr.hi[i] == (int)K) && kr.lo[i] >= 0 && kr.hi[i] <= (int)K,
                "llx_skinny_nt_scaled: k range %d of a block-diagonal W must be a multiple of 64 inside [0, K]", i);
  }
#define L(N, RG) hipLaunchKernelGGL((skinny_nt_kernel<N, RG, true>), grid, block, 0, stream, (const bf16_t*)X, ldx, (const bf16_t*)W, ldw, (bf16_t*)out, (int)M, (int)K, (int)R, kr, (const bf16_t*)colscale, (bf16_t*)G, ldg)
  if (kranges) { if (nb == 1) L(1, true); else if (nb == 2) L(2, true); else L(4, true); }
  else { if (nb == 1) L(1, false); else if (nb == 2) L(2, false); else L(4, false); }
#undef L
  LLX_LAUNCH_CHECK("llx_skinny_nt_scaled");
  return LLX_OK;
}

#define TN_NT 256
#define TN_MS 32
#define TN_YROW (TN_NT * 2 + 16)
#define TN_UROW (SK_PAD * 2 + 16)

__device__ __forceinline__ bf16x8_t tr16_frag(const char* tile, int rowbytes, int c0, int lane) {
  const int g = lane >> 4, i = lane & 15, q = i >> 2, p = i & 3;
  const char* base = tile + (8 * g + q) * rowbytes + (c0 + 4 * p) * 2;
  s16x4_t lo = __builtin_amdgcn_ds_read_tr16_b64_v4i16((lds_s16x4*)base);
  s16x4_t hi = __builtin_amdgcn_ds_read_tr16_b64_v4i16((lds_s16x4*)(base + 4 * rowbytes));
  s16x8_t v = {lo[0], lo[1], lo[2], lo[3], hi[0], hi[1], hi[2], hi[3]};
  return __builtin_bit_cast(bf16x8_t, v);
}

struct TnSegs { int n_lo[4], n_hi[4], r_lo[4], r_hi[4]; int64_t off[4]; int count; int rb_lo[4], rb_hi[4]; };

template <int NB>
__device__ __forceinline__ void skinny_tn_block(const bf16_t* __restrict__ U, const bf16_t* __restrict__ Y, int64_t ldy, float* __restrict__ partial,
                                                int M, int N, int rows_per_split, const TnSegs& sg, int ctile, int split, int nbl, char* sY, char* sU,
                                                const bf16_t* __restrict__ Bt = nullptr, int64_t ldb = 0, float* __restrict__ upart = nullptr, int brows = 0,
                                                const bf16_t* __restrict__ cs = nullptr, bf16_t* __restrict__ G = nullptr, int64_t ldg = 0) {
  const int tid = threadIdx.x, lane = tid & 63;
  const int wave = __builtin_amdgcn_readfirstlane(tid >> 6);
  const int n0 = ctile * TN_NT;
  const int m_begin = split * rows_per_split, m_end = min(M, m_begin + rows_per_split);
  const bool u_on = upart != nullptr && wave < nbl && n0 + TN_NT > sg.rb_lo[wave] && n0 < sg.rb_hi[wave];
  bf16x8_t ub[8];
  if (u_on) {
    const bf16_t* brow = Bt + (int64_t)min(wave * 16 + (lane & 15), brows - 1) * ldb;
#pragma unroll
    for (int ks = 0; ks < 8; ++ks) ub[ks] = *reinterpret_cast<const bf16x8_t*>(brow + min(n0 + ks * 32 + 8 * (lane >> 4), N - 8));
  }
  f32x4_t acc[NB][4];
#pragma unroll
  for (int rb = 0; rb < NB; ++rb)
#pragma unroll
    for (int cb = 0; cb < 4; ++cb) acc[rb][cb] = f32x4_t{0.f, 0.f, 0.f, 0.f};

  u32x4_t yv[2][4], uv[2];
  auto load_step = [&](int set, int ms) {
#pragma unroll
    for (int i = 0; i < 4; ++i) {
      const int q = i * 256 + tid;
      const int row = ms + (q >> 5), col = n0 + (q & 31) * 8;
      yv[set][i] = (row < m_end && col < N) ? *reinterpret_cast<const u32x4_t*>(Y + (int64_t)row * ldy + col) : u32x4_t{0u, 0u, 0u, 0u};
    }
    const int row = ms + (tid >> 3);
    uv[set] = (row < m_end) ? *reinterpret_cast<const u32x4_t*>(U + (int64_t)row * SK_PAD + (tid & 7) * 8) : u32x4_t{0u, 0u, 0u, 0u};
  };
  auto step = [&](int set, int ms) {
    __syncthreads();
#pragma unroll
    for (int i = 0; i < 4; ++i) {
      const int q = i * 256 + tid;
      *reinterpret_cast<u32x4_t*>(sY + (q >> 5) * TN_YROW + (q & 31) * 16) = yv[set][i];
      if (G) {
        const int row = ms + (q >> 5), col = n0 + (q & 31) * 8;
        if (row < m_end && col < N) {
          const u32x4_t c = *reinterpret_cast<const u32x4_t*>(cs + col);
          u32x4_t o;
#pragma unroll
          for (int e = 0; e < 4; ++e) o[e] = pack_bf2(bflo(yv[set][i][e]) * bflo(c[e]), bfhi(yv[set][i][e]) * bfhi(c[e]));
          *reinterpret_cast<u32x4_t*>(G + (int64_t)row * ldg + col) = o;
        }
      }
    }
    *reinterpret_cast<u32x4_t*>(sU + (tid >> 3) * TN_UROW + (tid & 7) * 16) = uv[set];
    __syncthreads();
    if (ms + 2 * TN_MS < m_end) load_step(set, ms + 2 * TN_MS);
    bf16x8_t a[NB];
#pragma unroll
    for (int rb = 0; rb < NB; ++rb) a[rb] = tr16_frag(sU, TN_UROW, rb * 16, lane);
#pragma unroll
    for (int cb = 0; cb < 4; ++cb) {
      const bf16x8_t b = tr16_frag(sY, TN_YROW, wave * 64 + cb * 16, lane);
#pragma unroll
      for (int rb = 0; rb < NB; ++rb)
        if (n0 + TN_NT > sg.rb_lo[rb] && n0 < sg.rb_hi[rb]) acc[rb][cb] = __builtin_amdgcn_mfma_f32_16x16x32_bf16(a[rb], b, acc[rb][cb], 0, 0, 0);
    }
    if (u_on) {
#pragma unroll
      for (int rf = 0; rf < 2; ++rf) {
        f32x4_t ua0 = {0.f, 0.f, 0.f, 0.f}, ua1 = {0.f, 0.f, 0.f, 0.f};
        const char* yrow = sY + (rf * 16 + (lane & 15)) * TN_YROW + (lane >> 4) * 16;
#pragma unroll
        for (int ks = 0; ks < 8; ks += 2) {
          ua0 = __builtin_amdgcn_mfma_f32_16x16x32_bf16(ub[ks], *reinterpret_cast<const bf16x8_t*>(yrow + ks * 64), ua0, 0, 0, 0);
          ua1 = __builtin_amdgcn_mfma_f32_16x16x32_bf16(ub[ks + 1], *reinterpret_cast<const bf16x8_t*>(yrow + (ks + 1) * 64), ua1, 0, 0, 0);
        }
        const int row = ms + rf * 16 + (lane & 15);
        if (row < m_end) {
#pragma unroll
          for (int e = 0; e < 4; ++e) upart[((int64_t)ctile * SK_PAD + wave * 16 + (lane >> 4) * 4 + e) * M + row] = ua0[e] + ua1[e];
        }
      }
    }
// ... 177 lines not shown
    const float* src = upart + (int64_t)c * M + min(m0 + ml, M - 1);
    int t = t_lo;
    for (; t + 8 <= t_hi; t += 8) {
      float v[8];
#pragma unroll
      for (int j = 0; j < 8; ++j) v[j] = src[(t + j) * stride];
#pragma unroll
      for (int j = 0; j < 8; ++j) sum += v[j];
    }
    for (; t < t_hi; ++t) sum += src[t * stride];
  }
  tile[cl][ml] = sum;
  __syncthreads();
  if (threadIdx.x < 64 && m0 + threadIdx.x < M) {
    u32x2_t pk;
    pk[0] = pack_bf2(tile[0][threadIdx.x], tile[1][threadIdx.x]);
    pk[1] = pack_bf2(tile[2][threadIdx.x], tile[3][threadIdx.x]);
    *reinterpret_cast<u32x2_t*>(out + (int64_t)(m0 + threadIdx.x) * SK_PAD + blockIdx.y * 4) = pk;
  }
}

extern "C" int llx_skinny_u_reduce(const void* upart, void* out, int64_t M, int64_t N, int64_t R, const int32_t* segs, int seg_count, hipStream_t stream) {
  LLX_REQUIRE(upart && out && M > 0 && N > 0 && R > 0 && R <= 64, "llx_skinny_u_reduce: bad arguments");
  TnSegs sg;
  int64_t total = 0;
  const int rc = tn_fill_segs(sg, segs, seg_count, N, R, &total);
  if (rc != LLX_OK) return rc;
  hipLaunchKernelGGL(skinny_u_reduce_kernel, dim3((unsigned)cdiv64(M, 64), SK_PAD / 4), dim3(256), 0, stream, (const float*)upart, (bf16_t*)out, (int)M, (int)R, sg);
  LLX_LAUNCH_CHECK("llx_skinny_u_reduce");
  return LLX_OK;
}

struct TnRed { const float* partial; bf16_t* out; int64_t out_ld, total; int nsplit, RP, R, N, transpose_out, accumulate, use_segs; float scale; TnSegs sg; };
struct TnRedMany { TnRed d[TN_MANY]; };

__global__ void skinny_tn_reduce_many_kernel(const TnRedMany m) {
  const TnRed& d = m.d[blockIdx.y];
  int64_t idx = (int64_t)blockIdx.x * blockDim.x + threadIdx.x;
  if (idx >= d.total) return;
  int r, n;
  bf16_t* dst;
  if (d.use_segs) {
    int s = 0;
    for (; s < d.sg.count; ++s) {
      const int64_t cnt = (int64_t)(d.sg.n_hi[s] - d.sg.n_lo[s]) * (d.sg.r_hi[s] - d.sg.r_lo[s]);
      if (idx < cnt) break;
      idx -= cnt;
    }
    if (s >= d.sg.count) return;
    const int rw = d.sg.r_hi[s] - d.sg.r_lo[s];
    n = d.sg.n_lo[s] + (int)(idx / rw);
    r = d.sg.r_lo[s] + (int)(idx % rw);
    dst = d.out + d.sg.off[s] + idx;
  } else {
    r = (int)(idx / d.N);
    n = (int)(idx % d.N);
    dst = d.transpose_out ? d.out + (int64_t)n * d.out_ld + r : d.out + (int64_t)r * d.out_ld + n;
  }
  float sum = 0.f;
  const float* src = d.partial + (int64_t)r * d.N + n;
  const int64_t stride = (int64_t)d.RP * d.N;
  int p = 0;
  for (; p + 8 <= d.nsplit; p += 8) {
    float v[8];
#pragma unroll
    for (int j = 0; j < 8; ++j) v[j] = src[(p + j) * stride];
#pragma unroll
    for (int j = 0; j < 8; ++j) sum += v[j];
  }
  if (p + 4 <= d.nsplit) {
    float v[4];
#pragma unroll
    for (int j = 0; j < 4; ++j) v[j] = src[(p + j) * stride];
#pragma unroll
    for (int j = 0; j < 4; ++j) sum += v[j];
    p += 4;
  }
  for (; p < d.nsplit; ++p) sum += src[p * stride];
  sum *= d.scale;
  if (d.accumulate) sum += bf2f(*dst);
  *dst = f2bf(sum);
}

extern "C" int llx_skinny_tn_reduce_many(int n, const void* const* workspaces, void* const* outs, const int64_t* out_ld, const int64_t* M,
                                         const int64_t* N, const int64_t* R, const float* scale, const int* transpose_out, const int* accumulate,
                                         const int32_t* const* segs, const int* seg_count, hipStream_t stream) {
  LLX_REQUIRE(n >= 1 && n <= TN_MANY && workspaces && outs && out_ld && M && N && R && scale && transpose_out && accumulate && segs && seg_count,
              "llx_skinny_tn_reduce_many: bad arguments (1..4 products)");
  TnRedMany m;
  int64_t most = 0;
  for (int i = 0; i < n; ++i) {
    TnRed& d = m.d[i];
    LLX_REQUIRE(workspaces[i] && outs[i] && M[i] > 0 && N[i] > 0 && R[i] > 0 && R[i] <= 64, "llx_skinny_tn_reduce_many: bad product %d", i);
    d.partial = (const float*)workspaces[i]; d.out = (bf16_t*)outs[i]; d.out_ld = out_ld[i];
    d.nsplit = tn_splits(M[i], N[i]); d.RP = (int)cdiv64(R[i], 16) * 16; d.R = (int)R[i]; d.N = (int)N[i];
    d.transpose_out = transpose_out[i]; d.accumulate = accumulate[i]; d.scale = scale[i];
    d.use_segs = segs[i] != nullptr;
    int64_t total = 0;
    const int rc = tn_fill_segs(d.sg, segs[i], seg_count[i], N[i], R[i], &total);
    if (rc != LLX_OK) return rc;
    d.total = d.use_segs ? total : R[i] * N[i];
    if (d.total > most) most = d.total;
  }
  hipLaunchKernelGGL(skinny_tn_reduce_many_kernel, dim3((unsigned)cdiv64(most, 256), (unsigned)n), dim3(256), 0, stream, m);
  LLX_LAUNCH_CHECK("llx_skinny_tn_reduce_many");
  return LLX_OK;
}

extern "C" int llx_skinny_tn(const void* U, const void* Y, int64_t ldy, void* out, int64_t out_ld, int64_t M, int64_t N, int64_t R,
                             float scale, int transpose_out, int accumulate, void* workspace, const int32_t* segs, int seg_count,
                             hipStream_t stream) {
  LLX_REQUIRE(out, "llx_skinny_tn: null pointer");
  int rc = llx_skinny_tn_partial(U, Y, ldy, M, N, R, workspace, segs, seg_count, stream);
  if (rc != LLX_OK) return rc;
  const void* ws[1] = {workspace};
  void* outs[1] = {out};
  return llx_skinny_tn_reduce_many(1, ws, outs, &out_ld, &M, &N, &R, &scale, &transpose_out, &accumulate, &segs, &seg_count, stream);
}

#define RSN_MAXPAIRS 8

template <int NB>
__global__ __launch_bounds__(SNT_WAVES * 64) void rmsnorm_skinny_nt_kernel(const bf16_t* __restrict__ X, const bf16_t* __restrict__ G,
                                                                           const bf16_t* __restrict__ W, int64_t ldw, bf16_t* __restrict__ Y,
                                                                           float* __restrict__ rstd_out, bf16_t* __restrict__ T, int M, int D,
                                                                           int R, float eps) {
  __shared__ float part[SNT_WAVES][16][SK_PAD];
  __shared__ float ssq[SNT_WAVES][16];
  const int lane = threadIdx.x & 63, wave = threadIdx.x >> 6;
  const int m0 = blockIdx.x * 16;
  const int fr = lane & 15, fq = lane >> 4;
  const int row = min(m0 + fr, M - 1);
  const int npw = D / (SNT_WAVES * 64);
  const bf16_t* xrow = X + (int64_t)row * D + wave * npw * 64 + 16 * fq;
  bf16x8_t a[RSN_MAXPAIRS][2];
  float ss = 0.f;
#pragma unroll
  for (int p = 0; p < RSN_MAXPAIRS; ++p) {
    if (p < npw) {
#pragma unroll
      for (int h = 0; h < 2; ++h) {
        a[p][h] = *reinterpret_cast<const bf16x8_t*>(xrow + p * 64 + 8 * h);
#pragma unroll
        for (int j = 0; j < 8; ++j) {
          const float v = (float)a[p][h][j];
          ss += v * v;
        }
      }
    }
  }
  const bf16_t* grow = G + wave * npw * 64 + 16 * fq;
  const bf16_t* wrow[NB];
#pragma unroll
  for (int nb = 0; nb < NB; ++nb) wrow[nb] = W + (int64_t)min(nb * 16 + fr, R - 1) * ldw + wave * npw * 64 + 16 * fq;
  bf16x8_t gv[RSN_MAXPAIRS][2];
#pragma unroll
  for (int p = 0; p < RSN_MAXPAIRS; ++p)
    if (p < npw) {
#pragma unroll
      for (int h = 0; h < 2; ++h) gv[p][h] = *reinterpret_cast<const bf16x8_t*>(grow + p * 64 + 8 * h);
    }
  constexpr int RSN_PRE = NB >= 3 ? 2 : 4;
  bf16x8_t bpre[RSN_PRE][2][NB];
#pragma unroll
  for (int p = 0; p < RSN_PRE; ++p)
    if (p < npw) {
#pragma unroll
      for (int h = 0; h < 2; ++h)
#pragma unroll
        for (int nb = 0; nb < NB; ++nb) bpre[p][h][nb] = *reinterpret_cast<const bf16x8_t*>(wrow[nb] + p * 64 + 8 * h);
    }
  ss += __shfl_xor(ss, 16, 64);
  ss += __shfl_xor(ss, 32, 64);
  if (fq == 0) ssq[wave][fr] = ss;
  __syncthreads();
  float tot = 0.f;
#pragma unroll
  for (int w = 0; w < SNT_WAVES; ++w) tot += ssq[w][fr];
  const float rstd = rsqrtf(tot / (float)D + eps);
  if (wave == 0 && fq == 0 && m0 + fr < M && rstd_out) rstd_out[m0 + fr] = rstd;
  bf16_t* yrow = Y + (int64_t)row * D + wave * npw * 64 + 16 * fq;
  f32x4_t acc[NB];
#pragma unroll
  for (int nb = 0; nb < NB; ++nb) acc[nb] = f32x4_t{0.f, 0.f, 0.f, 0.f};
#pragma unroll
  for (int p = 0; p < RSN_MAXPAIRS; ++p) {
    if (p < npw) {
#pragma unroll
      for (int h = 0; h < 2; ++h) {
// ... 51 lines not shown
```

### llama-x_amd/llx/_lib.py

```python
from __future__ import annotations

import ctypes
import os
from ctypes import c_char_p, c_float, c_int, c_int64, c_uint64, c_void_p

import torch

_HERE = os.path.dirname(os.path.abspath(__file__))
LIB_PATH = os.environ.get("LLX_LIB_PATH") or os.path.join(_HERE, "libllx_hip.so")

_lib = None

_P, _I, _L, _F = c_void_p, c_int, c_int64, c_float
SIGNATURES: dict[str, tuple] = {
    "llx_version": (c_int, []),
    "llx_last_error_string": (c_char_p, []),
    "llx_device_info": (c_int, [c_int, c_char_p, c_int]),
    "llx_rmsnorm_fwd": (c_int, [_P, _P, _P, _P, _L, _L, _F, _P]),
    "llx_rmsnorm_fwd_quant": (c_int, [_P, _P, _P, _P, _P, _L, _P, _L, _L, _F, _P]),
    "llx_rmsnorm_bwd_workspace_bytes": (c_int64, [_L, _L]),
    "llx_rmsnorm_bwd": (c_int, [_P, _P, _P, _P, _P, _P, _I, _P, _P, _L, _L, _P]),
    "llx_attn_flags_bytes": (c_int64, [_L, _L]),
    "llx_attn_tile_flags": (c_int, [_P, _P, _P, _L, _L, _P]),
    "llx_attn_fwd": (c_int, [_P, _L, _L, _P, _L, _L, _P, _L, _L, _P, _L, _L, _P, _P, _P, _P, _L, _L, _L, _L, _L, _F, _P]),
# ... 3 lines not shown
    "llx_attn_mask_flags_bytes": (c_int64, [_L, _L, _L]),
    "llx_attn_mask_tile_flags": (c_int, [_P, _L, _L, _P, _L, _L, _L, _P]),
    "llx_attn_mask_fwd": (c_int, [_P, _L, _L, _P, _L, _L, _L, _P, _L, _L, _L, _P, _L, _L, _P, _P, _L, _L, _P, _L, _L, _L, _L, _L, _L, _F, _P]),
    "llx_gemv_bf16": (c_int, [_P, _L, _L, _P, _L, _L, _P, _L, _L, _P, _L, _L, _L, _P, _F, _I, _P, _L, _P, _L, _P, _L, _L, _P, _P, _L, _L, _P,
                              _P, _P, _P, _L, _L, _L, _P, _L, _F, _P]),
    "llx_gemv_i8": (c_int, [_P, _L, _L, _P, _L, _L, _P, _L, _L, _P, _L, _L, _L, _P, _F, _I, _P, _L, _P, _L, _P, _L, _L, _P, _P, _L, _L, _P,
                            _P, _P, _P, _L, _L, _L, _P, _L, _F, _P, _P, _P, _I, _P]),
    "llx_gemv_bf16_dora": (c_int, [_P, _L, _L, _P, _L, _L, _P, _L, _L, _P, _L, _L, _L, _P, _F, _I, _P, _L, _P, _L, _P, _L, _L, _P, _P, _L, _L, _P,
                                   _P, _P, _P, _L, _L, _L, _P, _L, _F, _P, _P, _P, _P]),
    "llx_mask_extent": (c_int, [_P, _L, _L, _L, _P, _P]),
    "llx_kv_scatter": (c_int, [_P, _P, _L, _L, _L, _P, _P, _L, _L, _L, _P, _L, _L, _L, _L, _L, _P]),
    "llx_kv_scatter_rows": (c_int, [_P, _P, _L, _L, _L, _P, _P, _L, _L, _L, _P, _L, _L, _L, _L, _L, _L, _P]),
    "llx_gemm_rows16_workspace_bytes": (c_int64, [_L, _L, _L, _I]),
    "llx_gemm_rows16_bf16": (c_int, [_P, _L, _L, _P, _L, _L, _P, _L, _L, _P, _L, _L, _L, _P, _F, _I, _P, _L, _P, _L, _P, _L, _L, _P, _P, _L, _L, _L,
                                     _L, _P, _P, _L, _P]),
    "llx_gemm_rows16_i8_workspace_bytes": (c_int64, [_L, _L, _L, _I]),
    "llx_gemm_rows16_i8": (c_int, [_P, _L, _L, _P, _L, _L, _P, _L, _L, _P, _L, _L, _L, _P, _F, _I, _P, _L, _P, _L, _P, _L, _L, _P, _P, _L, _L, _L,
                                   _L, _P, _P, _L, _P, _P, _P, _P]),
    "llx_gemm_rows16_bf16_lora": (c_int, [_P, _L, _L, _P, _L, _L, _P, _L, _L, _P, _L, _L, _L, _P, _F, _I, _P, _L, _P, _L, _P, _L, _L, _P, _P, _L, _L, _L,
                                          _L, _P, _P, _L, _P, _P, _P, _L, _L, _L, _P, _L, _F, _P, _P, _P, _P]),
    "llx_gemm_rows16_i8_lora": (c_int, [_P, _L, _L, _P, _L, _L, _P, _L, _L, _P, _L, _L, _L, _P, _F, _I, _P, _L, _P, _L, _P, _L, _L, _P, _P, _L, _L, _L,
                                        _L, _P, _P, _L, _P, _P, _P, _P, _P, _P, _L, _L, _L, _P, _L, _F, _P]),
    "llx_attn_decode_workspace_bytes": (c_int64, [_L, _L, _L, _L]),
    "llx_attn_decode": (c_int, [_P, _L, _L, _L, _P, _P, _L, _L, _L, _P, _L, _L, _L, _P, _L, _L, _L, _P, _P, _L, _L, _L, _L, _L, _L, _L, _F, _P]),
    "llx_attn_bwd_workspace_bytes": (c_int64, [_L, _L, _L, _L]),
    "llx_attn_bwd_ds_bytes": (c_int64, [_L, _L, _L]),
    "llx_attn_bwd": (c_int, [_P, _L, _L, _P, _L, _L, _P, _L, _L, _P, _L, _L, _P, _L, _L, _P, _P, _P, _L, _L, _P, _L, _L, _P, _L, _L,
                             _P, _P, _P, _P, _P, _L, _L, _L, _L, _L, _F, _P]),
    "llx_attn_bwd_dropout": (c_int, [_P, _L, _L, _P, _L, _L, _P, _L, _L, _P, _L, _L, _P, _L, _L, _P, _P, _P, _L, _L, _P, _L, _L, _P, _L, _L,
                                     _P, _P, _P, _P, _P, _L, _L, _L, _L, _L, _F, _L, _P, _L, _P]),
    "llx_attn_mask_bwd": (c_int, [_P, _L, _L, _P, _L, _L, _P, _L, _L, _P, _L, _L, _P, _L, _L, _P, _P, _P, _L, _L, _P, _L, _L, _P, _L, _L,
                                  _P, _L, _L, _P, _P, _L, _L, _L, _L, _L, _F, _P]),
    "llx_embedding_fwd": (c_int, [_P, _P, _P, _L, _L, _L, _L, _L, _L, _P]),
    "llx_embedding_bwd": (c_int, [_P, _P, _P, _L, _L, _L, _L, _L, _L, _P]),
    "llx_rope": (c_int, [_P, _L, _L, _P, _L, _L, _P, _L, _L, _L, _L, _I, _P]),
    "llx_swiglu_fwd": (c_int, [_P, _L, _P, _L, _P, _L, _L, _L, _P]),
    "llx_swiglu_bwd": (c_int, [_P, _L, _P, _L, _P, _L, _P, _L, _P, _L, _L, _L, _P]),
    "llx_scale": (c_int, [_P, _L, _P, _L, _P, _F, _P, _L, _L, _P]),
    "llx_add": (c_int, [_P, _P, _P, _L, _P]),
    "llx_transpose": (c_int, [_P, _L, _P, _L, _L, _L, _I, _P]),
    "llx_i8_to_bf16": (c_int, [_P, _P, _L, _P]),
    "llx_quantize_int8_rowwise": (c_int, [_P, _L, _P, _L, _P, _L, _L, _I, _P]),
    "llx_int8_mm_dequant": (c_int, [_P, _L, _P, _L, _P, _L, _L, _L, _L, _P, _P, _P]),
    "llx_int8_mm_dequant_f32": (c_int, [_P, _L, _P, _L, _P, _L, _L, _L, _L, _P, _P, _P]),
    "llx_int8_mm_dequant_ext": (c_int, [_P, _L, _P, _L, _P, _L, _L, _L, _L, _P, _P, _P, _L, _P, _L, _L, _I, _P, _L, _P, _L, _L, _P]),
    "llx_mel_spectrogram": (c_int, [_P, _L, _L, _P, _P, _P, _P, _L, _L, _L, _P]),
    "llx_logmel_cmn": (c_int, [_P, _P, _L, _L, _L, _P]),
    "llx_gelu_fwd": (c_int, [_P, _L, _P, _L, _L, _L, _P]),
    "llx_gelu_bwd": (c_int, [_P, _L, _P, _L, _P, _L, _L, _L, _P]),
    "llx_col2im3": (c_int, [_P, _P, _L, _L, _L, _L, _P]),
    "llx_conv_w_reorder": (c_int, [_P, _P, _L, _L, _I, _P]),
    "llx_lora_group_pack": (c_int, [_P, _P, _P, _P, _I, _L, _F, _P, _P, _P, _P, _P]),
    "llx_lora_groups_pack": (c_int, [_P, _P, _P, _P, _P, _P, _P, _P, _P, _P, _P, _I, _P]),
    "llx_lora_pack": (c_int, [_P, _L, _P, _L, _L, _L, _L, _L, _F, _I, _P]),
    "llx_pad64": (c_int, [_P, _L, _P, _L, _L, _F, _I, _P]),
    "llx_rownorm2": (c_int, [_P, _L, _P, _L, _L, _P]),
    "llx_dora_colscale": (c_int, [_P, _P, _P, _P, _P, _P, _P, _L, _L, _P]),
    "llx_colsum_mul_workspace_bytes": (c_int64, [_L]),
    "llx_colsum_mul": (c_int, [_P, _L, _P, _L, _P, _P, _P, _L, _L, _P]),
    "llx_colscale_bias": (c_int, [_P, _L, _P, _L, _P, _P, _L, _L, _P]),
    "llx_ce_workspace_bytes": (c_int64, [_L]),
    "llx_ce_fwd_bwd": (c_int, [_P, _L, _P, _L, _P, _P, _P, _L, _L, _P]),
    "llx_ce_fwd_bwd_rows": (c_int, [_P, _L, _P, _L, _P, _P, _P, _L, _L, _P, _P]),
    "llx_ce_fwd_bwd_part": (c_int, [_P, _L, _P, _L, _P, _P, _P, _L, _L, _L, _L, _P, _I, _P]),
    "llx_logprob_rows_fwd": (c_int, [_P, _L, _P, _P, _P, _P, _L, _L, _P, _P]),
    "llx_logprob_rows_bwd": (c_int, [_P, _L, _P, _L, _P, _P, _P, _L, _L, _P, _P]),
    "llx_logprob_map_rows": (c_int, [_P, _P, _P, _F, _P, _P, _I, _L, _P]),
    "llx_head_compact_index": (c_int, [_P, _P, _P, _P, _P, _L, _P]),
    "llx_gather_rows": (c_int, [_P, _L, _P, _P, _P, _L, _L, _L, _P]),
    "llx_scatter_rows": (c_int, [_P, _L, _P, _P, _P, _L, _L, _L, _P]),
    "llx_skinny_nt": (c_int, [_P, _L, _P, _L, _P, _L, _L, _L, _P, _P]),
    "llx_skinny_nt_scaled": (c_int, [_P, _L, _P, _L, _P, _L, _L, _L, _P, _P, _P, _L, _P]),
    "llx_rmsnorm_skinny_nt": (c_int, [_P, _P, _P, _L, _P, _P, _P, _L, _L, _L, _F, _P]),
    "llx_skinny_tn_workspace_bytes": (c_int64, [_L, _L, _L]),
    "llx_skinny_tn": (c_int, [_P, _P, _L, _P, _L, _L, _L, _L, _F, _I, _I, _P, _P, _I, _P]),
    "llx_skinny_tn_partial": (c_int, [_P, _P, _L, _L, _L, _L, _P, _P, _I, _P]),
    "llx_skinny_tn_partial_many": (c_int, [_I, _P, _P, _P, _P, _P, _P, _P, _P, _P, _P]),
    "llx_skinny_u_workspace_bytes": (_L, [_L, _L]),
    "llx_skinny_tn_partial_many_u": (c_int, [_I, _P, _P, _P, _P, _P, _P, _P, _P, _P, _P, _P, _P, _P]),
    "llx_skinny_u_reduce": (c_int, [_P, _P, _L, _L, _L, _P, _I, _P]),
    "llx_skinny_tn_partial_many_us": (c_int, [_I, _P, _P, _P, _P, _P, _P, _P, _P, _P, _P, _P, _P, _P, _P, _P, _P]),
    "llx_skinny_tn_reduce_many": (c_int, [_I, _P, _P, _P, _P, _P, _P, _P, _P, _P, _P, _P, _P]),
    "llx_gemm_nt_bf16": (c_int, [_P, _L, _P, _L, _P, _L, _L, _L, _L, _P, _L, _P, _L, _L, _I, _P, _L, _P]),
    "llx_gemm_nt_bf16_splitk": (c_int, [_P, _L, _P, _L, _P, _L, _L, _L, _I, _P, _P]),
    "llx_splitk_combine": (c_int, [_P, _I, _L, _L, _P, _P, _P, _L, _P]),
    "llx_gemm_nt_bf16_rows": (c_int, [_P, _L, _P, _L, _P, _L, _L, _L, _L, _P, _L, _P, _L, _L, _I, _P, _L, _P, _P]),
    "llx_gemm_tn_bf16": (c_int, [_P, _L, _P, _L, _P, _L, _L, _L, _L, _P]),
    "llx_gemm_tn_bf16_rows": (c_int, [_P, _L, _P, _L, _P, _L, _L, _L, _L, _P, _P]),
    "llx_gemm_nt_bf16_rope": (c_int, [_P, _L, _P, _L, _P, _L, _L, _L, _L, _P, _L, _P, _L, _L, _P, _L, _L, _P]),
    "llx_sample_rows": (c_int, [_P, _I, _L, _L, _L, _F, _L, _F, c_uint64, _P, _P, _P, _L, _L, _L, _I, _L, _P, _P, _P, _P, _P]),
    "llx_sample_rows_ext": (c_int, [_P, _I, _L, _L, _L, _F, _L, _F, c_uint64, _P, _P, _P, _L, _L, _L, _I, _L, _P, _P, _P, _P, _P, _L, _F, _F, _F,
                                    _P, _P]),
    "llx_lookup_step": (c_int, [_P, _P, _L, _P, _P, _P, _P, _P, _L, _L, _I, _I, _L, _I, _P]),
    "llx_beam_rows": (c_int, [_P, _I, _L, _L, _L, _P, _P, _P]),
    "llx_beam_merge": (c_int, [_P, _P, _P, _P, _P, _P, _L, _P, _L, _P, _P, _P, _L, _L, _L, _F, _I, _P]),
    "llx_kv_reorder_rows": (c_int, [_P, _L, _L, _L, _L, _P, _L, _L, _L, _L, _L, _P]),
}

DEBUG_SIGNATURES: dict[str, tuple] = {
    "llx_debug_attn_fwd_occupancy": (c_int, []),
    "llx_debug_attn_bwd_set_stamps": (c_int, [_P]),
    "llx_debug_attn_fwd_stamps": (c_int, [_P, _P, _P, _P, _L, _L, _L, _P, _P]),
}


class LlxError(RuntimeError):
    pass


def load():
    global _lib
    if _lib is not None:
        return _lib
    if not os.path.exists(LIB_PATH):
        raise LlxError(
            f"{LIB_PATH} is missing: build it with `python -c 'import __graft_entry__ as g; g.build()'` "
            "(or `make -C llama-x_amd/csrc`). There is no fallback path."
        )
    lib = ctypes.CDLL(LIB_PATH)
    for name, (res, args) in {**SIGNATURES, **DEBUG_SIGNATURES}.items():
        fn = getattr(lib, name)
        fn.restype = res
        fn.argtypes = args
    _lib = lib
    return lib


def check(rc: int, what: str = ""):
    if rc != 0:
        msg = load().llx_last_error_string()
        raise LlxError(f"{what} failed (code {rc}): {msg.decode() if msg else '?'}")


_raw_stream = getattr(torch._C, "_cuda_getCurrentRawStream", None)


def stream() -> c_void_p:
    if _raw_stream is not None:
        return c_void_p(_raw_stream(torch.cuda.current_device()))
    return c_void_p(torch.cuda.current_stream().cuda_stream)


def ptr(t) -> c_void_p:
    if t is None:
        return c_void_p(0)
    return c_void_p(t.data_ptr())


def require_cuda(*tensors):
    for t in tensors:
        if t is not None and not t.is_cuda:
            raise LlxError("llx ops run on the HIP device only (tensor on %s); there is no CPU path" % t.device)
```

### llama-x_amd/llx/kernels.py

```python
from __future__ import annotations

import ctypes
import math
import os
from dataclasses import dataclass
from typing import Optional, Sequence

import torch
from torch import Tensor

from . import _lib as L

BF16 = torch.bfloat16
EPI_NONE, EPI_RESIDUAL, EPI_BIAS, EPI_BIAS_GELU, EPI_COLSCALE = 0, 1, 2, 3, 4
EPI_SWIGLU_BWD = 6
EPI_SWIGLU_FWD = 7
SK_PAD = 64
GEMM_TRACE = None
ATTN_TRACE = None


def _trace_begin(trace):
    if trace is None:
        return None
    ev = (torch.cuda.Event(enable_timing=True), torch.cuda.Event(enable_timing=True))
    ev[0].record()
    return ev


def _trace_end(trace, ev, *info):
    if ev is not None:
        ev[1].record()
        trace.append((ev[0], ev[1], *info))


def _lib():
    return L.load()


def gemm_kernel_launches(M: int, N: int, epilogue: int) -> int:
    gm, gn = -(-M // 256), -(-N // 256)
    tail = (gm * gn) % 256
    split = epilogue != EPI_SWIGLU_FWD and N % 256 == 0 and gm * gn > 256 and 0 < tail <= 128 and tail % gm == 0
    return 2 if split else 1


def _rows2d(x: Tensor) -> Tensor:
    if x.dim() == 2:
        return x if x.stride(1) == 1 else x.contiguous()
    y = x.reshape(-1, x.shape[-1])
    return y if y.stride(1) == 1 else y.contiguous()


def _chk_bf16(*ts):
    for t in ts:
        if t is not None:
            assert t.dtype is BF16, f"llx kernels compute in bf16 (got {t.dtype})"
    L.require_cuda(*ts)


def rmsnorm_fwd(x: Tensor, w: Tensor, eps: float, quant: bool = False):
    _chk_bf16(x, w)
    x2 = _rows2d(x)
    assert x2.stride(0) == x2.shape[1], "rmsnorm input rows must be dense"
    rows, dim = x2.shape
    assert w.shape == (dim,) and w.is_contiguous()
    y = torch.empty_like(x2)
    rstd = torch.empty(rows, device=x.device, dtype=torch.float32)
    if quant:
        q = torch.empty(rows, dim, device=x.device, dtype=torch.int8)
        qs = torch.empty(rows, device=x.device, dtype=BF16)
        L.check(_lib().llx_rmsnorm_fwd_quant(L.ptr(x2), L.ptr(w), L.ptr(y), L.ptr(rstd), L.ptr(q), dim, L.ptr(qs), rows, dim, eps, L.stream()),
                "llx_rmsnorm_fwd_quant")
        return y.view(x.shape), rstd, q, qs
    L.check(_lib().llx_rmsnorm_fwd(L.ptr(x2), L.ptr(w), L.ptr(y), L.ptr(rstd), rows, dim, eps, L.stream()), "llx_rmsnorm_fwd")
    return y.view(x.shape), rstd


def rmsnorm_skinny_ok(dim: int) -> bool:
    return dim % 512 == 0 and dim <= 4096


def rmsnorm_skinny_nt(x: Tensor, w: Tensor, eps: float, a_cat: Tensor) -> tuple[Tensor, Tensor, Tensor]:
    _chk_bf16(x, w, a_cat)
    x2 = _rows2d(x)
    rows, dim = x2.shape
    assert x2.stride(0) == dim and w.shape == (dim,) and w.is_contiguous() and rmsnorm_skinny_ok(dim)
    assert a_cat.dim() == 2 and a_cat.shape[1] == dim and a_cat.stride(1) == 1 and a_cat.shape[0] <= SK_PAD
    y = torch.empty_like(x2)
    rstd = torch.empty(rows, device=x.device, dtype=torch.float32)
    t = torch.empty(rows, SK_PAD, device=x.device, dtype=BF16)
    L.check(_lib().llx_rmsnorm_skinny_nt(L.ptr(x2), L.ptr(w), L.ptr(a_cat), a_cat.stride(0), L.ptr(y), L.ptr(rstd), L.ptr(t), rows, dim,
                                         a_cat.shape[0], eps, L.stream()), "llx_rmsnorm_skinny_nt")
    return y.view(x.shape), rstd, t


def rmsnorm_bwd(dy: Tensor, x: Tensor, w: Tensor, rstd: Tensor, need_dw: bool, dres: Optional[Tensor] = None,
                dw_out: Optional[Tensor] = None) -> tuple[Tensor, Optional[Tensor]]:
    _chk_bf16(dy, x, w, dres)
    x2, dy2 = _rows2d(x), _rows2d(dy)
    if dy2.stride(0) != dy2.shape[1]:
        dy2 = dy2.contiguous()
    rows, dim = x2.shape
    dx = torch.empty_like(x2)
    dw = ws = None
    if need_dw:
        dw = dw_out if dw_out is not None else torch.empty(dim, device=x.device, dtype=BF16)
        assert dw.shape == (dim,) and dw.is_contiguous() and dw.dtype is BF16
        ws = torch.empty(_lib().llx_rmsnorm_bwd_workspace_bytes(rows, dim), device=x.device, dtype=torch.uint8)
    if dres is not None:
        dres = _rows2d(dres)
        assert dres.shape == x2.shape and dres.stride(0) == dim
    L.check(_lib().llx_rmsnorm_bwd(L.ptr(dy2), L.ptr(x2), L.ptr(w), L.ptr(rstd), L.ptr(dx), L.ptr(dw), 0, L.ptr(ws), L.ptr(dres), rows, dim,
                                   L.stream()), "llx_rmsnorm_bwd")
    return dx.view(x.shape), dw


def gemm_nt(a: Tensor, b: Tensor, *, out: Optional[Tensor] = None, a2: Optional[Tensor] = None, b2: Optional[Tensor] = None,
            epilogue: int = EPI_NONE, e: Optional[Tensor] = None, rope: Optional[tuple[Tensor, int, int]] = None,
            k2_eff: Optional[float] = None, m_valid: Optional[Tensor] = None, m_expect: Optional[float] = None) -> Tensor:
    _chk_bf16(a, b, a2, b2, e, out)
    assert a.dim() == 2 and b.dim() == 2 and a.shape[1] == b.shape[1], (a.shape, b.shape)
    assert a.stride(1) == 1 and b.stride(1) == 1
    M, K = a.shape
    N = b.shape[0]
    if epilogue == EPI_SWIGLU_BWD:
        assert out is not None and e is not None and out.shape == (M, 2 * N) and e.shape == (M, 2 * N) and out.stride(1) == 1 and e.stride(1) == 1
    else:
        if out is None:
            out = torch.empty(M, N, device=a.device, dtype=BF16)
        assert out.shape == (M, N) and out.stride(1) == 1
    K2 = 0
    if a2 is not None:
        assert b2 is not None and a2.shape[0] == M and b2.shape[0] == N and a2.shape[1] == b2.shape[1]
        assert a2.stride(1) == 1 and b2.stride(1) == 1
        K2 = a2.shape[1]
    lde = 0
    if epilogue == EPI_RESIDUAL:
        assert e is not None and e.shape == (M, N) and e.stride(1) == 1
        lde = e.stride(0)
    elif epilogue == EPI_SWIGLU_BWD:
        lde = e.stride(0)
    elif epilogue == EPI_SWIGLU_FWD:
        assert e is not None and N % 256 == 0 and e.shape == (M, N // 2) and e.stride(1) == 1
        lde = e.stride(0)
    elif epilogue != EPI_NONE:
        assert e is not None and e.shape == (N,) and e.is_contiguous()
    ev = _trace_begin(GEMM_TRACE)
    if rope is not None:
        table, rs, rc = rope
        assert epilogue == EPI_NONE and table.dtype is torch.float32 and table.is_contiguous() and table.shape[0] >= rs and table.shape[1:] == (64, 2)
        L.check(_lib().llx_gemm_nt_bf16_rope(L.ptr(a), a.stride(0), L.ptr(b), b.stride(0), L.ptr(out), out.stride(0), M, N, K,
                                             L.ptr(a2), a2.stride(0) if a2 is not None else 0, L.ptr(b2), b2.stride(0) if b2 is not None else 0, K2,
                                             L.ptr(table), rs, rc, L.stream()), "llx_gemm_nt_bf16_rope")
    elif m_valid is not None:
        assert m_valid.dtype is torch.int32 and m_valid.numel() == 1 and m_valid.device == a.device
        L.check(_lib().llx_gemm_nt_bf16_rows(L.ptr(a), a.stride(0), L.ptr(b), b.stride(0), L.ptr(out), out.stride(0), M, N, K,
                                             L.ptr(a2), a2.stride(0) if a2 is not None else 0, L.ptr(b2), b2.stride(0) if b2 is not None else 0, K2,
                                             epilogue, L.ptr(e), lde, L.ptr(m_valid), L.stream()), "llx_gemm_nt_bf16_rows")
    else:
        L.check(_lib().llx_gemm_nt_bf16(L.ptr(a), a.stride(0), L.ptr(b), b.stride(0), L.ptr(out), out.stride(0), M, N, K,
                                        L.ptr(a2), a2.stride(0) if a2 is not None else 0, L.ptr(b2), b2.stride(0) if b2 is not None else 0, K2,
                                        epilogue, L.ptr(e), lde, L.stream()), "llx_gemm_nt_bf16")
    if ev is not None:
        kk = K + (K2 if k2_eff is None else min(float(k2_eff), K2))
        Mw = M if m_expect is None else float(m_expect)
        _trace_end(GEMM_TRACE, ev, 2.0 * Mw * N * kk, 2.0 * (Mw * kk + N * kk + Mw * N * (2 if epilogue == EPI_RESIDUAL else 1)), "bf16",
                   gemm_kernel_launches(M, N, 8 if rope is not None else epilogue))
    return out


def gemm_nt_splitk(a: Tensor, b: Tensor, splits: int, *, m_valid: Optional[Tensor] = None, inv: Optional[Tensor] = None,
                   dev_scalar: Optional[Tensor] = None, m_expect: Optional[float] = None) -> Tensor:
    _chk_bf16(a, b)
    assert a.dim() == 2 and b.dim() == 2 and a.shape[1] == b.shape[1] and a.stride(1) == 1 and b.stride(1) == 1
    M, K = a.shape
    N = b.shape[0]
    part = torch.empty(splits, M, N, device=a.device, dtype=torch.float32)
    ev = _trace_begin(GEMM_TRACE)
    L.check(_lib().llx_gemm_nt_bf16_splitk(L.ptr(a), a.stride(0), L.ptr(b), b.stride(0), L.ptr(part), M, N, K, splits, L.ptr(m_valid), L.stream()),
            "llx_gemm_nt_bf16_splitk")
    if ev is not None:
        Mw = M if m_expect is None else float(m_expect)
        _trace_end(GEMM_TRACE, ev, 2.0 * Mw * N * K, 2.0 * (Mw * K + N * K) + 4.0 * splits * Mw * N, "bf16", 1)
    out = torch.empty(M, N, device=a.device, dtype=BF16)
    assert inv is None or (inv.dtype is torch.int32 and inv.numel() == M)
    assert dev_scalar is None or (dev_scalar.dtype is torch.float32 and dev_scalar.numel() == 1)
    L.check(_lib().llx_splitk_combine(L.ptr(part), splits, M, N, L.ptr(inv), L.ptr(dev_scalar), L.ptr(out), N, L.stream()), "llx_splitk_combine")
    return out


def transpose(x: Tensor, pad_to: int = 1) -> Tensor:
    L.require_cuda(x)
    assert x.dim() == 2 and x.stride(1) == 1 and x.dtype in (BF16, torch.int8)
    R, C = x.shape
    Rp = (R + pad_to - 1) // pad_to * pad_to
    out = (torch.zeros if Rp != R else torch.empty)(C, Rp, device=x.device, dtype=BF16)
    L.check(_lib().llx_transpose(L.ptr(x), x.stride(0), L.ptr(out), Rp, R, C, int(x.dtype is torch.int8), L.stream()), "llx_transpose")
    return out


def pad64(x: Tensor, scale_: float = 1.0, transposed: bool = False) -> Tensor:
    _chk_bf16(x)
    assert x.dim() == 2 and x.stride(1) == 1
    R, C = (x.shape[1], x.shape[0]) if transposed else x.shape
    out = torch.empty(R, SK_PAD, device=x.device, dtype=BF16)
    L.check(_lib().llx_pad64(L.ptr(x), x.stride(0), L.ptr(out), R, C, scale_, int(transposed), L.stream()), "llx_pad64")
    return out


def lora_pack(x: Tensor, out: Tensor, row_off: int, col_off: int, scale_: float = 1.0, transposed: bool = False) -> None:
    _chk_bf16(x, out)
    assert x.dim() == 2 and x.stride(1) == 1 and out.dim() == 2 and out.stride(1) == 1
    R, C = x.shape
    rr, cc = (C, R) if transposed else (R, C)
    assert row_off + rr <= out.shape[0] and col_off + cc <= out.shape[1], (x.shape, out.shape, row_off, col_off, transposed)
    L.check(_lib().llx_lora_pack(L.ptr(x), x.stride(0), L.ptr(out), out.stride(0), R, C, row_off, col_off, scale_, int(transposed), L.stream()),
            "llx_lora_pack")


def lora_group_pack(lora_as: list, lora_bs: list, K_in: int, scale_: float):
    nm = len(lora_as)
    Ns = [b.shape[0] for b in lora_bs]
    ranks = [a.shape[0] for a in lora_as]
    for a, b in zip(lora_as, lora_bs):
        _chk_bf16(a, b)
        assert a.is_contiguous() and b.is_contiguous() and a.shape[1] == K_in and b.shape[1] == a.shape[0]
    N, R = sum(Ns), sum(ranks)
    dev = lora_as[0].device
    buf = torch.empty(R * K_in + N * SK_PAD + R * N + K_in * SK_PAD, device=dev, dtype=BF16)
    a_cat = buf[: R * K_in].view(R, K_in)
    o = R * K_in
    b2 = buf[o : o + N * SK_PAD].view(N, SK_PAD)
    o += N * SK_PAD
    bT = buf[o : o + R * N].view(R, N)
    o += R * N
    a2t = buf[o:].view(K_in, SK_PAD)
    PA = (ctypes.c_void_p * nm)(*[a.data_ptr() for a in lora_as])
    PB = (ctypes.c_void_p * nm)(*[b.data_ptr() for b in lora_bs])
    NS = (ctypes.c_int64 * nm)(*Ns)
    RS = (ctypes.c_int64 * nm)(*ranks)
    L.check(_lib().llx_lora_group_pack(PA, PB, NS, RS, nm, K_in, scale_, L.ptr(a_cat), L.ptr(b2), L.ptr(bT), L.ptr(a2t), L.stream()),
            "llx_lora_group_pack")
    return a_cat, b2, bT, a2t


def lora_groups_pack(groups: list) -> list:
    ng = len(groups)
    assert 1 <= ng <= 4
    sizes, metas = [], []
    for las, lbs, K_in, _ in groups:
# ... 872 lines not shown
    return logits if write_grad else None


def logprob_rows_fwd(logits: Tensor, labels: Tensor, rows: Optional[Tensor] = None, want_top1: bool = False):
    _chk_bf16(logits)
    L.require_cuda(labels)
    assert logits.dim() == 2 and logits.stride(1) == 1
    T, V = logits.shape
    labels = labels.reshape(-1).contiguous()
    assert labels.dtype is torch.int64 and labels.numel() == T and labels.device == logits.device
    assert rows is None or (rows.dtype is torch.int32 and rows.numel() == 1 and rows.device == logits.device)
    logp = torch.empty(T, device=logits.device, dtype=torch.float32)
    lse = torch.empty(T, device=logits.device, dtype=torch.float32)
    top1 = torch.empty(T, device=logits.device, dtype=torch.int32) if want_top1 else None
    L.check(_lib().llx_logprob_rows_fwd(L.ptr(logits), logits.stride(0), L.ptr(labels), L.ptr(logp), L.ptr(lse), L.ptr(top1), T, V, L.ptr(rows),
                                        L.stream()), "llx_logprob_rows_fwd")
    return logp, lse, top1


def logprob_rows_bwd(logits: Tensor, labels: Tensor, lse: Tensor, g: Tensor, rows: Optional[Tensor] = None, out: Optional[Tensor] = None) -> Tensor:
    _chk_bf16(logits, out)
    L.require_cuda(labels, lse, g)
    assert logits.dim() == 2 and logits.stride(1) == 1
    T, V = logits.shape
    labels = labels.reshape(-1).contiguous()
    assert labels.dtype is torch.int64 and labels.numel() == T and labels.device == logits.device
    assert lse.dtype is torch.float32 and lse.is_contiguous() and lse.numel() == T and lse.device == logits.device
    assert g.dtype is torch.float32 and g.is_contiguous() and g.numel() == T and g.device == logits.device
    assert rows is None or (rows.dtype is torch.int32 and rows.numel() == 1 and rows.device == logits.device)
    if out is None:
        out = logits
    assert out.shape == logits.shape and out.stride(1) == 1 and out.device == logits.device
    L.check(_lib().llx_logprob_rows_bwd(L.ptr(logits), logits.stride(0), L.ptr(out), out.stride(0), L.ptr(labels), L.ptr(lse), L.ptr(g), T, V,
                                        L.ptr(rows), L.stream()), "llx_logprob_rows_bwd")
    return out


def logprob_map_rows(index: Tensor, src: Tensor, fill: float = 0.0, src_i: Optional[Tensor] = None, fill_i: int = 0):
    L.require_cuda(index, src, src_i)
    T = index.numel()
    assert index.dtype is torch.int32 and index.is_contiguous() and src.dtype is torch.float32 and src.is_contiguous() and src.numel() == T
    assert src_i is None or (src_i.dtype is torch.int32 and src_i.is_contiguous() and src_i.numel() == T)
    dst = torch.empty_like(src)
    dst_i = torch.empty_like(src_i) if src_i is not None else None
    L.check(_lib().llx_logprob_map_rows(L.ptr(index), L.ptr(src), L.ptr(dst), float(fill), L.ptr(src_i), L.ptr(dst_i), int(fill_i), T, L.stream()),
            "llx_logprob_map_rows")
    return dst, dst_i


def skinny_nt(x: Tensor, w: Tensor, kranges: Optional[Sequence[int]] = None, colscale: Optional[Tensor] = None):
    _chk_bf16(x, w, colscale)
    assert x.dim() == 2 and w.dim() == 2 and x.shape[1] == w.shape[1] and x.stride(1) == 1 and w.stride(1) == 1
    M, K = x.shape
    R = w.shape[0]
    out = torch.empty(M, SK_PAD, device=x.device, dtype=BF16)
    kr = None
    if kranges is not None:
        assert len(kranges) == 8
        kr = (ctypes.c_int32 * 8)(*[int(v) for v in kranges])
    if colscale is not None:
        assert colscale.shape == (K,) and colscale.is_contiguous()
        g = torch.empty(M, K, device=x.device, dtype=BF16)
        L.check(_lib().llx_skinny_nt_scaled(L.ptr(x), x.stride(0), L.ptr(w), w.stride(0), L.ptr(out), M, K, R, kr, L.ptr(colscale), L.ptr(g), K,
                                            L.stream()), "llx_skinny_nt_scaled")
        return out, g
    L.check(_lib().llx_skinny_nt(L.ptr(x), x.stride(0), L.ptr(w), w.stride(0), L.ptr(out), M, K, R, kr, L.stream()), "llx_skinny_nt")
    return out


@dataclass
class TnQueued:
    ws: Tensor
    out: Tensor
    out_ld: int
    M: int
    N: int
    R: int
    scale: float
    transpose_out: int
    accumulate: int
    segs: Optional[ctypes.Array]
    n_segs: int
    upart: Optional[Tensor] = None


def skinny_tn(u: Tensor, y: Tensor, R: int, scale_: float, out: Tensor, transpose_out: bool, accumulate: bool = False,
              segs: Optional[Sequence[tuple[int, int, int, int]]] = None, pending: Optional[list] = None,
              u_from: Optional[Tensor] = None, scaled: Optional[tuple[Tensor, Tensor]] = None) -> Tensor:
    _chk_bf16(u, y, out)
    M, N = y.shape
    assert u.shape == (M, SK_PAD) and u.is_contiguous() and y.stride(1) == 1 and out.stride(-1) == 1
    sp, ns = None, 0
    if segs is not None:
        ns = len(segs)
        assert 1 <= ns <= 4 and out.is_contiguous() and out.numel() == sum((b - a) * (d - c) for a, b, c, d in segs)
        sp = (ctypes.c_int32 * (4 * ns))(*[int(v) for sgm in segs for v in sgm])
    else:
        assert out.shape == ((N, R) if transpose_out else (R, N))
    ws = torch.empty(_lib().llx_skinny_tn_workspace_bytes(M, N, R), device=y.device, dtype=torch.uint8)
    out_ld = out.stride(0) if out.dim() == 2 else 0
    if pending is None:
        assert u_from is None and scaled is None, "the fused u / scaled-copy outputs need the queued (pending=) form"
        L.check(_lib().llx_skinny_tn(L.ptr(u), L.ptr(y), y.stride(0), L.ptr(out), out_ld, M, N, R, scale_, int(transpose_out), int(accumulate),
                                     L.ptr(ws), sp, ns, L.stream()), "llx_skinny_tn")
        return out
    q = TnQueued(ws, out, out_ld, M, N, R, scale_, int(transpose_out), int(accumulate), sp, ns)
    if u_from is None:
        assert scaled is None
        L.check(_lib().llx_skinny_tn_partial(L.ptr(u), L.ptr(y), y.stride(0), M, N, R, L.ptr(ws), sp, ns, L.stream()), "llx_skinny_tn_partial")
    else:
        assert u_from.dtype is BF16 and u_from.dim() == 2 and u_from.shape == (R, N) and u_from.stride(1) == 1
        q.upart = torch.empty(_lib().llx_skinny_u_workspace_bytes(M, N) // 4, device=y.device, dtype=torch.float32)
        cs = g = None
        if scaled is not None:
            cs, g = scaled
            assert cs.dtype is BF16 and cs.numel() == N and g.shape == (M, N) and g.stride(1) == 1
        one = lambda ctype, v: (ctype * 1)(v)
        ptr = lambda t: one(ctypes.c_void_p, t.data_ptr() if t is not None else None)
        L.check(_lib().llx_skinny_tn_partial_many_us(1, ptr(u), ptr(y), one(ctypes.c_int64, y.stride(0)), one(ctypes.c_int64, M), one(ctypes.c_int64, N),
                                                     one(ctypes.c_int64, R), ptr(ws), one(ctypes.c_void_p, ctypes.cast(sp, ctypes.c_void_p).value if sp is not None else None),
                                                     one(ctypes.c_int, ns), ptr(u_from), one(ctypes.c_int64, u_from.stride(0)), ptr(q.upart), ptr(cs), ptr(g),
                                                     one(ctypes.c_int64, g.stride(0) if g is not None else 0), L.stream()), "llx_skinny_tn_partial_many")
    pending.append(q)
    if len(pending) == 4:
        skinny_tn_flush(pending)
    return out


def skinny_u_reduce(q: TnQueued) -> Tensor:
    assert q.upart is not None, "the product must have been queued with u_from"
    out = torch.empty(q.M, SK_PAD, device=q.upart.device, dtype=BF16)
    L.check(_lib().llx_skinny_u_reduce(L.ptr(q.upart), L.ptr(out), q.M, q.N, q.R, q.segs, q.n_segs, L.stream()), "llx_skinny_u_reduce")
    return out


def skinny_tn_flush(pending: list) -> None:
    while pending:
        chunk, pending[:] = pending[:4], pending[4:]
        n = len(chunk)
        WS = (ctypes.c_void_p * n)(*[q.ws.data_ptr() for q in chunk])
        OUT = (ctypes.c_void_p * n)(*[q.out.data_ptr() for q in chunk])
        LD = (ctypes.c_int64 * n)(*[q.out_ld for q in chunk])
        MM = (ctypes.c_int64 * n)(*[q.M for q in chunk])
        NN = (ctypes.c_int64 * n)(*[q.N for q in chunk])
        RR = (ctypes.c_int64 * n)(*[q.R for q in chunk])
        SC = (ctypes.c_float * n)(*[q.scale for q in chunk])
        TR = (ctypes.c_int * n)(*[q.transpose_out for q in chunk])
        AC = (ctypes.c_int * n)(*[q.accumulate for q in chunk])
        SG = (ctypes.c_void_p * n)(*[ctypes.cast(q.segs, ctypes.c_void_p).value if q.segs is not None else None for q in chunk])
        NS = (ctypes.c_int * n)(*[q.n_segs for q in chunk])
        L.check(_lib().llx_skinny_tn_reduce_many(n, WS, OUT, LD, MM, NN, RR, SC, TR, AC, SG, NS, L.stream()), "llx_skinny_tn_reduce_many")
```

### llama-x_amd/llx/ops.py

```python
from __future__ import annotations

import os

from typing import NamedTuple, Optional, Sequence

import torch
from torch import Tensor, nn
from torch.autograd import Function

from . import kernels as K
from ._lib import LlxError

BF16 = torch.bfloat16


def _cached_multi(tensors: Sequence[Tensor], tag: str, build):
    store = tensors[0].__dict__.setdefault("_llx_cache", {})
    key = tuple((t._version, str(t.device)) for t in tensors)
    hit = store.get(tag)
    if hit is not None and hit[0] == key:
        return hit[1]
    val = build()
    store[tag] = (key, val)
    return val
# ... 133 lines not shown


def dora_colscale(members: Sequence[LinearPlan], w_cat: Tensor, a_cat: Tensor, b2: Tensor, wn2_tag: str = "wn2") -> tuple[Tensor, Tensor]:
    N, R = w_cat.shape[0], a_cat.shape[0]
    wn2 = _cached_multi([m.weight for m in members], wn2_tag, lambda: K.rownorm2(w_cat))
    G = K.skinny_nt(w_cat, a_cat)
    AAt = K.skinny_nt(a_cat, a_cat)
    c = torch.empty(N, device=w_cat.device, dtype=BF16)
    inv = torch.empty(N, device=w_cat.device, dtype=torch.float32)
    off = 0
    for m in members:
        sl = slice(off, off + m.N)
        K.dora_colscale(wn2[sl], G[sl], b2[sl], AAt, m.dora_m.detach(), c[sl], inv[sl], R)
        off += m.N
    return c, inv


def dora_scale_cached(m) -> Tensor:
    plan = m if isinstance(m, LinearPlan) else None
    mag = plan.dora_m if plan is not None else m.m

    def build():
        p = plan if plan is not None else LinearPlan(m)
        c, _ = dora_colscale([p], p.weight.detach(), p.lora_a.detach(), K.pad64(p.lora_b.detach(), p.scale), wn2_tag="wn2m")
        return c

    return _cached_multi([m.weight, m.lora_a, m.lora_b, mag], "dora_c", build)


class GroupPlan:

    def __init__(self, mods: Sequence[nn.Linear]):
        self.members = [LinearPlan(m) for m in mods]
        m0 = self.members[0]
        self.K = m0.K
        self.Ns = [m.N for m in self.members]
        self.N = sum(self.Ns)
        self.n_off = [sum(self.Ns[:i]) for i in range(len(self.Ns))]
        self.ranks = [m.rank for m in self.members]
        self.R = sum(self.ranks)
        self.r_off = [sum(self.ranks[:i]) for i in range(len(self.ranks))]
        same_kind = all((m.int8, m.dynamic) == (m0.int8, m0.dynamic) for m in self.members)
        same_scale = len({m.scale for m in self.members if m.rank > 0}) <= 1
        lora_all_or_none = all(r > 0 for r in self.ranks) or self.R == 0
        dora_all_or_none = len({m.dora_m is not None for m in self.members}) == 1
        self.dora = all(m.dora_m is not None for m in self.members)
        self.fused = (same_kind and same_scale and lora_all_or_none and dora_all_or_none and self.R <= 64
                      and all(m.bias is None for m in self.members) and all(m.K == self.K for m in self.members))
        self.int8, self.dynamic = m0.int8, m0.dynamic
        self.packed = None
        self.scale = next((m.scale for m in self.members if m.rank > 0), 1.0)
        self.k2_fwd = sum(n * r for n, r in zip(self.Ns, self.ranks)) / self.N

    def tensors(self) -> list[Tensor]:
        return [t for m in self.members for t in m.tensors()]

    def _weights(self):
        return [(m.weight.int_data if m.int8 else m.weight) for m in self.members]

    def w_cat(self) -> Tensor:
        ws = self._weights()
        if self.int8 and self.dynamic:
            return _cached_multi(ws, "cat_i8", lambda: torch.cat([w.detach() for w in ws], 0))
        if self.int8:
            return _cached_multi(ws, "cat_bf16", lambda: K.i8_to_bf16(torch.cat([w.detach() for w in ws], 0)))
        return _cached_multi(ws, "cat", lambda: torch.cat([w.detach() for w in ws], 0) if len(ws) > 1 else ws[0].detach())

    def wt_cat(self) -> Tensor:
        ws = self._weights()
        return _cached_multi(ws, "cat_t", lambda: K.transpose(torch.cat([w.detach() for w in ws], 0) if len(ws) > 1 else ws[0].detach()))

    def scale_cat(self) -> Tensor:
        ss = [m.weight.scale for m in self.members]
        return _cached_multi(ss, "cat_scale", lambda: torch.cat(ss, 0) if len(ss) > 1 else ss[0])

    def dora_scale_cached(self) -> Tensor:
        if len(self.members) == 1:
            return dora_scale_cached(self.members[0])
        srcs = [t for m in self.members for t in (m.weight, m.lora_a, m.lora_b, m.dora_m)]
        return _cached_multi(srcs, "dora_c_cat", lambda: torch.cat([dora_scale_cached(m) for m in self.members], 0))

    def forward(self, x: Tensor, out: Optional[Tensor] = None, residual: Optional[Tensor] = None, swiglu_h: Optional[Tensor] = None,
                rope: Optional[tuple[Tensor, int, int]] = None, xq: Optional[tuple[Tensor, Tensor]] = None, t_pre: Optional[Tensor] = None,
                cached_scale: bool = False):
        if out is None:
            out = torch.empty(x.shape[0], self.N, device=x.device, dtype=BF16)
        return out, self._forward(x, out, residual, swiglu_h, rope, xq, t_pre, cached_scale)

    def norm_can_make_t(self, dim: int) -> bool:
        return self.fused and self.R > 0 and self.packed is not None and K.rmsnorm_skinny_ok(dim)

    def wants_quantized_input(self) -> bool:
        return self.fused and self.int8 and self.dynamic

    def rope_fusable(self) -> bool:
        return self.fused and (not self.int8 or self.dynamic) and not self.dora

    def swiglu_fusable(self) -> bool:
        return self.fused and (not self.int8 or self.dynamic) and not self.dora and len(self.members) == 2 and self.Ns[0] % 128 == 0

    def _forward(self, x: Tensor, out: Tensor, residual: Optional[Tensor], swiglu_h: Optional[Tensor] = None,
                 rope: Optional[tuple[Tensor, int, int]] = None, xq: Optional[tuple[Tensor, Tensor]] = None, t_pre: Optional[Tensor] = None,
                 cached_scale: bool = False):
        if not self.fused:
            assert residual is None or len(self.members) == 1
            return [m.forward(x, out=out[:, o : o + n], residual=residual, cached_scale=cached_scale)[1]
                    for m, o, n in zip(self.members, self.n_off, self.Ns)]
        t = b2 = None
        if self.R > 0:
            a_cat, b2, bT, a2t = self.packed or K.lora_group_pack([m.lora_a.detach() for m in self.members],
                                                                  [m.lora_b.detach() for m in self.members], self.K, self.scale)
            t = (t_pre if t_pre is not None else K.skinny_nt(x, a_cat), bT, a2t)
        if self.dora:
            assert swiglu_h is None and rope is None
            c, inv = (self.dora_scale_cached(), None) if cached_scale else dora_colscale(self.members, self.w_cat(), a_cat, b2)
            z = K.gemm_nt(x, self.w_cat(), a2=t[0], b2=b2, k2_eff=self.k2_fwd)
            K.scale(z, colscale=c, out=out)
            if residual is not None:
                K.add(out, residual, out=out)
            return (*t, z, c, inv)
        if not self.int8:
            if residual is not None:
                K.gemm_nt(x, self.w_cat(), out=out, a2=t[0] if t else None, b2=b2, epilogue=K.EPI_RESIDUAL, e=residual, k2_eff=self.k2_fwd)
            elif swiglu_h is not None:
                K.gemm_nt(x, self.w_cat(), out=out, a2=t[0] if t else None, b2=b2, epilogue=K.EPI_SWIGLU_FWD, e=swiglu_h, k2_eff=self.k2_fwd)
            else:
                K.gemm_nt(x, self.w_cat(), out=out, a2=t[0] if t else None, b2=b2, rope=rope, k2_eff=self.k2_fwd)
            return t
        if self.dynamic:
            from subclasses.int8 import quantize_int8_rowwise
            from subclasses.int8_mm import _launch as i8_gemm

            xi, xs = xq if xq is not None else quantize_int8_rowwise(x)
            a2, bb = (t[0], b2) if self.R > 0 else (None, None)
            if residual is not None:
                i8_gemm(xi, self.w_cat(), xs, self.scale_cat(), out=out, a2=a2, b2=bb, epilogue=K.EPI_RESIDUAL, e=residual)
            elif swiglu_h is not None:
                i8_gemm(xi, self.w_cat(), xs, self.scale_cat(), out=out, a2=a2, b2=bb, epilogue=K.EPI_SWIGLU_FWD, e=swiglu_h)
            else:
                i8_gemm(xi, self.w_cat(), xs, self.scale_cat(), out=out, a2=a2, b2=bb, rope=rope)
            return t
        else:
            direct = self.R == 0 and residual is None
            y0 = K.gemm_nt(x, self.w_cat(), out=out if direct else None, epilogue=K.EPI_COLSCALE, e=self.scale_cat())
        if self.R > 0:
            y0 = K.gemm_nt(t[0], b2, out=out if residual is None else None, epilogue=K.EPI_RESIDUAL, e=y0, k2_eff=0)
        if residual is not None:
            K.add(y0, residual, out=out)
        return t

    def _tn_segs(self) -> Optional[list[tuple[int, int, int, int]]]:
        if getattr(self, "_segs", None) is None:
            segs = [(no, no + n, ro, ro + r) for ro, r, no, n in zip(self.r_off, self.ranks, self.n_off, self.Ns) if r > 0]
            ok = 1 <= len(segs) <= 4 and all(a % 256 == 0 and (b % 256 == 0 or b == self.N) for a, b, _, _ in segs)
            self._segs = segs if ok else False
        return self._segs or None

    def _kranges(self) -> Optional[list[int]]:
        if getattr(self, "_kr", None) is None and len(self.members) == 1:
            self._kr = False
        if getattr(self, "_kr", None) is None:
            kr: list[int] = []
            for nb in range(4):
                lo, hi = None, None
                for ro, r, no, n in zip(self.r_off, self.ranks, self.n_off, self.Ns):
                    if r > 0 and ro < 16 * nb + 16 and ro + r > 16 * nb:
                        lo = no if lo is None else min(lo, no)
                        hi = no + n if hi is None else max(hi, no + n)
                kr += [lo or 0, hi or 0] if lo is not None else [0, 0]
            ok = all(v % 64 == 0 for v in kr)
            self._kr = kr if ok else False
        return self._kr or None

    def backward(self, dy: Tensor, x: Tensor, saved, needs: Sequence[bool], need_dx: bool, dx_out: Optional[Tensor] = None,
                 swiglu: Optional[tuple[Tensor, Tensor]] = None, pending: Optional[list] = None):
        if not self.fused:
            grads, dx, first = [], None, True
            ni = 0
            for m, o, n, t in zip(self.members, self.n_off, self.Ns, saved):
                cnt = len(m.tensors())
                d, g = m.backward(dy[:, o : o + n], x, t, needs[ni : ni + cnt], need_dx, dx_out, not first)
                ni += cnt
                grads += g
                dx = d if d is not None else dx
                first = False
            return dx, grads
        gM = None
        ni = iter(needs)
        need = []
        for m in self.members:
            cnt = len(m.tensors())
            need.append([next(ni) for _ in range(cnt)])
        ia = -3 if self.dora else -2
        dy_out = dy
        z = inv = None
        if self.dora:
            t, bT, a2t, z, c, inv = saved
            dy = K.scale(dy_out, colscale=c)
        else:
            t, bT, a2t = saved if saved is not None else (None, None, None)
        u = gA = gBt = g_scaled = None
        gB_views: Optional[list[Optional[Tensor]]] = None
        need_a, need_b = self.R > 0 and any(nd[ia] for nd in need), self.R > 0 and any(nd[ia + 1] for nd in need)
        if self.dora and any(nd[-1] for nd in need):
            gM = K.colsum_mul(dy_out, z, inv)
        if need_b:
            segs = self._tn_segs()
            if segs is not None:
                flat = _grad_dst([m.lora_b for m in self.members if m.rank > 0])
                if flat is None:
                    flat = torch.empty(sum((b - a) * (d - c_) for a, b, c_, d in segs), device=dy.device, dtype=BF16)
                sc = None
                if self.int8 and need_dx:
                    g_scaled = torch.empty_like(dy)
                    sc = (self.scale_cat(), g_scaled)
                K.skinny_tn(t, dy, self.R, self.scale, flat, transpose_out=True, segs=segs, pending=pending, u_from=bT, scaled=sc)
                u = K.skinny_u_reduce(pending[-1])
                gB_views, off = [], 0
                for m_, (a, b, c_, d) in zip([m for m in self.members if m.rank > 0], segs):
                    gB_views.append(flat[off : off + (b - a) * (d - c_)].view(b - a, d - c_))
                    off += (b - a) * (d - c_)
            else:
                gBt = torch.empty(self.N, self.R, device=dy.device, dtype=BF16)
                K.skinny_tn(t, dy, self.R, self.scale, gBt, transpose_out=True)
        if self.R > 0:
            if u is not None:
                pass
            elif self.int8 and need_dx:
                u, g_scaled = K.skinny_nt(dy, bT, self._kranges(), colscale=self.scale_cat())
            else:
                u = K.skinny_nt(dy, bT, self._kranges())
            if need_a:
                gA = _grad_dst([m.lora_a for m in self.members if m.rank > 0], (self.R, self.K))
                if gA is None:
                    gA = torch.empty(self.R, self.K, device=dy.device, dtype=BF16)
                K.skinny_tn(u, x, self.R, self.scale, gA, transpose_out=False, pending=pending)
        dx = None
        if need_dx:
            if self.int8:
                g = g_scaled if g_scaled is not None else K.scale(dy, colscale=self.scale_cat())
            else:
                g = dy
            if swiglu is not None:
                dx = K.gemm_nt(g, self.wt_cat(), out=swiglu[1], a2=u, b2=a2t if self.R > 0 else None, epilogue=K.EPI_SWIGLU_BWD, e=swiglu[0], k2_eff=self.R)
            else:
                dx = K.gemm_nt(g, self.wt_cat(), out=dx_out, a2=u, b2=a2t if self.R > 0 else None, k2_eff=self.R)
        grads: list[Optional[Tensor]] = []
        gb_i = 0
        for m, nd, ro, no, n in zip(self.members, need, self.r_off, self.n_off, self.Ns):
            j = 0
            if not m.int8:
                grads.append(K.gemm_tn(dy[:, no : no + n], x) if nd[j] else None)
                j += 1
            if m.rank > 0:
                grads.append(gA[ro : ro + m.rank] if nd[j] else None)
                if gB_views is not None:
                    grads.append(gB_views[gb_i] if nd[j + 1] else None)
                    gb_i += 1
                else:
                    grads.append(gBt[no : no + n, ro : ro + m.rank].contiguous() if nd[j + 1] else None)
                j += 2
            if m.dora_m is not None:
                grads.append(gM[no : no + n] if nd[j] else None)
        return dx, grads


def _grad_dst(params: Sequence[Optional[Tensor]], shape: Optional[tuple] = None) -> Optional[Tensor]:
    g0 = first = end = None
    for p in params:
        slot = getattr(p, "_llx_slot", None)
        if slot is None or p.grad is not None or getattr(p, "_llx_claimed", False):
            return None
        G, off, n = slot
        if g0 is None:
            g0, first = G, off
        elif G is not g0 or off != end:
            return None
        end = off + n
    if g0 is None:
        return None
    for p in params:
        p._llx_claimed = True
    out = g0[first:end]
    return out.view(shape) if shape is not None else out


def _enc(o, flat: list):
    if isinstance(o, Tensor):
        flat.append(o)
        return ("t", len(flat) - 1)
    if isinstance(o, (tuple, list)):
        return ("l", [_enc(x, flat) for x in o])
    return ("c", o)


def _dec(sp, flat):
    kind, v = sp
    if kind == "t":
        return flat[v]
    if kind == "l":
        return tuple(_dec(x, flat) for x in v)
    return v


def _save(ctx, *objs) -> None:
    flat: list[Tensor] = []
    ctx._llx_spec = [_enc(o, flat) for o in objs]
    ctx.save_for_backward(*flat)


def _load(ctx) -> list:
    flat = ctx.saved_tensors
    return [_dec(sp, flat) for sp in ctx._llx_spec]


def prepack(plans: Sequence[GroupPlan]) -> None:
    todo = [p for p in plans if p.fused and p.R > 0]
    for i in range(0, len(todo), 4):
        chunk = todo[i : i + 4]
        if len(chunk) < 2:
            break
        imgs = K.lora_groups_pack([([m.lora_a.detach() for m in p.members], [m.lora_b.detach() for m in p.members], p.K, p.scale) for p in chunk])
        for p, im in zip(chunk, imgs):
            p.packed = im


def _norm_prologue(meta, plan: GroupPlan, x2: Tensor, norm_w: Optional[Tensor]):
# ... 112 lines not shown
class AttnBlockFn(Function):
    @staticmethod
    def forward(ctx, x: Tensor, rope: Tensor, norm_w: Optional[Tensor], meta: AttnBlockMeta, ticket: Optional[Tensor], *tensors):
        K.L.require_cuda(x)
        B, S, D = x.shape
        H, KVH, hd = meta.H, meta.KVH, meta.hd
        x2 = K._rows2d(x.contiguous())
        xn, rstd, xq, t_pre = _norm_prologue(meta, meta.qkv, x2, norm_w)
        W = (H + 2 * KVH) * hd
        qkv = torch.empty(B * S, W, device=x.device, dtype=BF16)
        fuse_rope = meta.qkv.rope_fusable()
        infer = meta.no_grad or not any(ctx.needs_input_grad)
        _, tqkv = meta.qkv.forward(xn, qkv, rope=(rope, S, (H + KVH) * hd) if fuse_rope else None, xq=xq, t_pre=t_pre, cached_scale=infer)
        qkv3 = qkv.view(B, S, W)
        if not fuse_rope:
            K.rope_(qkv3, rope, H + KVH)
        q = qkv3[..., : H * hd].unflatten(-1, (H, hd))
        k = qkv3[..., H * hd : (H + KVH) * hd].unflatten(-1, (KVH, hd))
        v = qkv3[..., (H + KVH) * hd :].unflatten(-1, (KVH, hd))
        o, lse = K.attn_fwd(q, k, v, meta.mask, dropout=(meta.dropout[0], ticket, meta.dropout[1]) if meta.dropout else None)
        o2 = o.view(B * S, H * hd)
        y, to = meta.wo.forward(o2, None, x2 if meta.fuse_residual else None, cached_scale=infer)
        ctx.meta = meta
        _save(ctx, x, rope, norm_w, x2, xn if meta.fuse_norm else None, rstd, qkv3, o, lse, tqkv, to, ticket if meta.dropout else None)
        return y.view(B, S, D)

    @staticmethod
    def backward(ctx, dy: Tensor):
        meta: AttnBlockMeta = ctx.meta
        x, rope, norm_w, x2, xn, rstd, qkv3, o, lse, tqkv, to, ticket = _load(ctx)
        if xn is None:
            xn = x2
        B, S, D = x.shape
        H, KVH, hd = meta.H, meta.KVH, meta.hd
        dy2 = K._rows2d(dy.contiguous())
        needs = list(ctx.needs_input_grad[5:])
        n_qkv = len(meta.qkv.tensors())
        nqkv, no = needs[:n_qkv], needs[n_qkv:]
        pend = []
        do2, g_o = meta.wo.backward(dy2, o.view(B * S, H * hd), to, no, True, pending=pend)
        W = (H + 2 * KVH) * hd
        dqkv = torch.empty(B, S, W, device=x.device, dtype=BF16)
        q = qkv3[..., : H * hd].unflatten(-1, (H, hd))
        k = qkv3[..., H * hd : (H + KVH) * hd].unflatten(-1, (KVH, hd))
        v = qkv3[..., (H + KVH) * hd :].unflatten(-1, (KVH, hd))
        dq = dqkv[..., : H * hd].unflatten(-1, (H, hd))
        dk = dqkv[..., H * hd : (H + KVH) * hd].unflatten(-1, (KVH, hd))
        dv = dqkv[..., (H + KVH) * hd :].unflatten(-1, (KVH, hd))
        K.attn_bwd(q, k, v, o, do2.view(B, S, H, hd), lse, dq, dk, dv, meta.mask, rope=rope,
                   dropout=(meta.dropout[0], ticket, meta.dropout[1]) if meta.dropout else None)
        d2 = dqkv.view(B * S, W)
        need_dx = ctx.needs_input_grad[0]
        need_dxn = need_dx or (meta.fuse_norm and ctx.needs_input_grad[2])
        dxn = torch.empty(B * S, D, device=x.device, dtype=BF16) if need_dxn else None
        _, g_qkv = meta.qkv.backward(d2, xn, tqkv, nqkv, need_dxn, dxn, pending=pend)
        K.skinny_tn_flush(pend)
        dx, dnw = _norm_epilogue(dxn, x2, norm_w, rstd, ctx.needs_input_grad[2], dy2 if (need_dx and meta.fuse_residual) else None, meta.fuse_norm)
        return (dx.view(B, S, D) if (dx is not None and need_dx) else None, None, dnw, None, None, *g_qkv, *g_o)


_HEAD_COMPACT = os.environ.get("LLX_HEAD_COMPACT", "1") != "0"
_HEAD_SPLITK = max(1, int(os.environ.get("LLX_HEAD_SPLITK", "4")))
_HEAD_CHUNK_FORCED = "LLX_HEAD_CHUNK_ROWS" in os.environ
_HEAD_CHUNK_ROWS = max(256, int(os.environ.get("LLX_HEAD_CHUNK_ROWS", "8192")) // 256 * 256)


class MLPBlockMeta:
    def __init__(self, w13: GroupPlan, w2: GroupPlan, eps, fuse_norm, fuse_residual):
        self.w13, self.w2 = w13, w2
        self.eps, self.fuse_norm, self.fuse_residual = eps, fuse_norm, fuse_residual
        self.no_grad = not torch.is_grad_enabled()


class MLPBlockFn(Function):
    @staticmethod
    def forward(ctx, x: Tensor, norm_w: Optional[Tensor], meta: MLPBlockMeta, *tensors):
        K.L.require_cuda(x)
        shape = x.shape
        x2 = K._rows2d(x.contiguous())
        xn, rstd, xq, t_pre = _norm_prologue(meta, meta.w13, x2, norm_w)
        T, I = x2.shape[0], meta.w13.Ns[0]
        gu = torch.empty(T, 2 * I, device=x.device, dtype=BF16)
        infer = meta.no_grad or not any(ctx.needs_input_grad)
        if meta.w13.swiglu_fusable():
            h = torch.empty(T, I, device=x.device, dtype=BF16)
            _, t13 = meta.w13.forward(xn, gu, swiglu_h=h, xq=xq, t_pre=t_pre, cached_scale=infer)
        else:
            _, t13 = meta.w13.forward(xn, gu, xq=xq, t_pre=t_pre, cached_scale=infer)
            h = K.swiglu_fwd(gu[:, :I], gu[:, I:])
        y, t2 = meta.w2.forward(h, None, x2 if meta.fuse_residual else None, cached_scale=infer)
        ctx.meta = meta
        _save(ctx, x, norm_w, x2, xn if meta.fuse_norm else None, rstd, gu, h, t13, t2)
        return y.view(shape)

    @staticmethod
    def backward(ctx, dy: Tensor):
        meta: MLPBlockMeta = ctx.meta
        x, norm_w, x2, xn, rstd, gu, h, t13, t2 = _load(ctx)
        if xn is None:
            xn = x2
        T, I = x2.shape[0], meta.w13.Ns[0]
        dy2 = K._rows2d(dy.contiguous())
        needs = list(ctx.needs_input_grad[3:])
        n_13 = len(meta.w13.tensors())
        n13, n2 = needs[:n_13], needs[n_13:]
        dgu = torch.empty(T, 2 * I, device=x.device, dtype=BF16)
        pend = []
        if meta.w2.fused:
            _, g_2 = meta.w2.backward(dy2, h, t2, n2, True, swiglu=(gu, dgu), pending=pend)
        else:
            dh, g_2 = meta.w2.backward(dy2, h, t2, n2, True)
            K.swiglu_bwd(dh, gu[:, :I], gu[:, I:], dgu[:, :I], dgu[:, I:])
        need_dx = ctx.needs_input_grad[0]
        need_dxn = need_dx or (meta.fuse_norm and ctx.needs_input_grad[1])
        dxn = torch.empty_like(x2) if need_dxn else None
        _, g_13 = meta.w13.backward(dgu, xn, t13, n13, need_dxn, dxn, pending=pend)
        K.skinny_tn_flush(pend)
        dx, dnw = _norm_epilogue(dxn, x2, norm_w, rstd, ctx.needs_input_grad[1], dy2 if (need_dx and meta.fuse_residual) else None, meta.fuse_norm)
        return (dx.view(x.shape) if (dx is not None and need_dx) else None, dnw, None, *g_13, *g_2)


class HeadRoute(NamedTuple):
    plain_head: bool
    plain_trainable: bool
    compact: bool
    chunk: int


def _head_route(plan, weight_needs: bool, T: int, V: int) -> HeadRoute:
    plain = not plan.int8 and plan.rank == 0 and plan.bias is None and plan.dora_m is None
    chunk = _HEAD_CHUNK_ROWS if (_HEAD_CHUNK_FORCED or T * V * 2 >= 2**32) else 0
    return HeadRoute(plain and not weight_needs, plain and weight_needs and _HEAD_COMPACT, plain and _HEAD_COMPACT, chunk if T > chunk else 0)


def _head_rows(xn: Tensor, labels: Tensor, route: HeadRoute):
    if not route.compact:
        return xn, labels.reshape(-1).contiguous(), None, None, None
    idx, inv, labels_c, cnt = K.head_compact_index(labels)
    return K.gather_rows(xn, idx, cnt), labels_c, idx, inv, cnt


def _head_logits(plan: LinearPlan, rows_in: Tensor, route: HeadRoute, cnt: Optional[Tensor]):
    T = rows_in.shape[0]
    step = route.chunk or T
    for r0 in range(0, T, step):
        r1 = min(T, r0 + step)
        if not route.compact:
            logits, t = plan.forward(rows_in[r0:r1])
            yield r0, r1, logits, None, t, None
            continue
        m_expect = None
        if route.chunk:
            cnt_c = torch.clamp(cnt - r0, min=0, max=r1 - r0).to(torch.int32)
        else:
            cnt_c = cnt
            m_expect = float(cnt.item()) if K.GEMM_TRACE is not None else None
        logits = torch.empty(r1 - r0, plan.N, device=rows_in.device, dtype=BF16)
        K.gemm_nt(rows_in[r0:r1], plan.weight.detach(), out=logits, m_valid=cnt_c, m_expect=m_expect)
        yield r0, r1, logits, cnt_c, None, m_expect


def _head_dhidden(route: HeadRoute, plan: LinearPlan, dlogits, cnt, inv: Optional[Tensor], scalar: Optional[Tensor], m_expect) -> Tensor:
    wt = weight_t(plan.weight)
    split = wt.shape[1] % (64 * _HEAD_SPLITK) == 0
    if route.chunk:
        dxc = torch.empty(sum(dl.shape[0] for dl in dlogits), wt.shape[0], device=wt.device, dtype=BF16)
        for i, (dl, cnt_c) in enumerate(zip(dlogits, cnt)):
            part = K.gemm_nt_splitk(dl, wt, _HEAD_SPLITK, m_valid=cnt_c) if split else K.gemm_nt(dl, wt, m_valid=cnt_c)
            dxc[i * route.chunk : i * route.chunk + dl.shape[0]].copy_(part)
    elif split:
        return K.gemm_nt_splitk(dlogits, wt, _HEAD_SPLITK, m_valid=cnt, inv=inv, dev_scalar=scalar, m_expect=m_expect)
    else:
        dxc = K.gemm_nt(dlogits, wt, m_valid=cnt, m_expect=m_expect)
    if inv is not None:
        return K.scatter_rows(dxc, inv, scalar)
    return dxc if scalar is None else K.scale(dxc, dev_scalar=scalar)


def _head_backward(ctx, n_lead: int, saved, dlogits, inv, cnt, t, scalar: Optional[Tensor]):
    route, plan = ctx.route, ctx.plan
    x, norm_w, x2, xn, rstd = saved
    needs = ctx.needs_input_grad[n_lead:]
    need_dxn = ctx.needs_input_grad[0] or ctx.needs_input_grad[1]
    if route.plain_head or route.plain_trainable:
        dx = dnw = gw = None
        if need_dxn:
            dx, dnw = _norm_epilogue(_head_dhidden(route, plan, dlogits, cnt, inv, scalar, ctx.m_expect), x2, norm_w, rstd, ctx.needs_input_grad[1])
        if route.plain_trainable:
            gw = K.gemm_tn(dlogits, xn, m_valid=cnt, m_expect=ctx.m_expect)
            gw = gw if scalar is None else K.scale(gw, dev_scalar=scalar)
        grads = [gw] + [None] * (len(needs) - 1) if needs else []
    else:
        dxn, grads = plan.backward(dlogits, xn, t, needs, need_dx=need_dxn)
        if scalar is not None:
            grads = [None if g is None else K.scale(g, dev_scalar=scalar) for g in grads]
            if dxn is not None:
                K.scale(dxn, dev_scalar=scalar, out=dxn)
        dx, dnw = _norm_epilogue(dxn, x2, norm_w, rstd, ctx.needs_input_grad[1])
    return (dx.view(x.shape) if dx is not None else None, dnw, *([None] * (n_lead - 2)), *grads)
# ... 105 lines not shown
```

Baseline: 32450 tokens/s.

## Fuse LoRA adapter projections into SwiGLU forward and backward GEMM epilogues

The forward gate/up GEMM epilogue now also multiplies the freshly computed SwiGLU output h by the down-projection LoRA A matrix in-tile. It writes partial t products that are reduced instead of running a separate skinny pass over h. In the backward pass, the down-projection dgrad GEMM's SwiGLU-backward epilogue computes the gate/up LoRA partials, u = dgu·B^T and the dB weight partials from t13, using extra LDS and ds_read_tr16 transposed fragment loads. This removes re-reading the large T×2I activations in separate skinny kernels, at the cost of heavier epilogues, more LDS per block (possible occupancy loss), extra partial workspaces and reductions.

```diff
diff --git a/include/llx.h b/include/llx.h
--- a/include/llx.h
+++ b/include/llx.h
@@ -24,6 +24,14 @@
 int llx_gemm_nt_bf16(const void* A, int64_t lda, const void* B, int64_t ldb, void* C, int64_t ldc, int64_t M, int64_t N, int64_t K,
                      const void* A2, int64_t lda2, const void* B2, int64_t ldb2, int64_t K2, int epilogue, const void* E, int64_t lde,
                      llx_stream_t s);
+int llx_gemm_nt_bf16_swiglu_t(const void* A, int64_t lda, const void* B, int64_t ldb, void* C, int64_t ldc, int64_t M, int64_t N, int64_t K,
+                              const void* A2, int64_t lda2, const void* B2, int64_t ldb2, int64_t K2, void* H, int64_t ldh, const void* TA,
+                              int64_t ldta, int64_t R, float* tpart, llx_stream_t s);
+int64_t llx_gemm_swiglu_bwd_t_upart_bytes(int64_t M, int64_t N);
+int64_t llx_gemm_swiglu_bwd_t_wpart_bytes(int64_t M, int64_t N, int64_t R);
+int llx_gemm_nt_bf16_swiglu_bwd_t(const void* A, int64_t lda, const void* B, int64_t ldb, void* C, int64_t ldc, int64_t M, int64_t N, int64_t K,
+                                  const void* A2, int64_t lda2, const void* B2, int64_t ldb2, int64_t K2, const void* E, int64_t lde,
+                                  const void* T13, const void* BT, int64_t R1, int64_t R3, float* upart, float* wpart, llx_stream_t s);
 int llx_gemm_nt_bf16_rows(const void* A, int64_t lda, const void* B, int64_t ldb, void* C, int64_t ldc, int64_t M, int64_t N, int64_t K,
                           const void* A2, int64_t lda2, const void* B2, int64_t ldb2, int64_t K2, int epilogue, const void* E, int64_t lde,
                           const int32_t* m_valid, llx_stream_t s);
@@ -209,6 +217,9 @@
 int llx_skinny_tn_reduce_many(int n, const void* const* workspaces, void* const* outs, const int64_t* out_ld, const int64_t* M, const int64_t* N,
                               const int64_t* R, const float* scale, const int* transpose_out, const int* accumulate,
                               const int32_t* const* segs, const int* seg_count, llx_stream_t s);
+int llx_skinny_tn_reduce_many_splits(int n, const void* const* workspaces, void* const* outs, const int64_t* out_ld, const int64_t* M,
+                                     const int64_t* N, const int64_t* R, const float* scale, const int* transpose_out, const int* accumulate,
+                                     const int32_t* const* segs, const int* seg_count, const int* nsplit, llx_stream_t s);
 int llx_pad64(const void* in, int64_t ld, void* out, int64_t R, int64_t C, float scale, int transpose, llx_stream_t s);
 int llx_lora_group_pack(const void* const* lora_a, const void* const* lora_b, const int64_t* Ns, const int64_t* ranks, int nm, int64_t K,
                         float scale, void* a_cat, void* b2, void* bT, void* a2t, llx_stream_t s);
diff --git a/llama-x_amd/csrc/common.h b/llama-x_amd/csrc/common.h
--- a/llama-x_amd/csrc/common.h
+++ b/llama-x_amd/csrc/common.h
@@ -216,6 +216,17 @@
   return __builtin_bit_cast(bf16x8_t, v);
 }
 
+typedef __attribute__((address_space(3))) s16x4_t lds_s16x4;
+typedef __attribute__((ext_vector_type(8))) short s16x8_t;
+__device__ __forceinline__ bf16x8_t tr16_frag(const char* tile, int rowbytes, int c0, int lane) {
+  const int g = lane >> 4, i = lane & 15, q = i >> 2, p = i & 3;
+  const char* base = tile + (8 * g + q) * rowbytes + (c0 + 4 * p) * 2;
+  s16x4_t lo = __builtin_amdgcn_ds_read_tr16_b64_v4i16((lds_s16x4*)base);
+  s16x4_t hi = __builtin_amdgcn_ds_read_tr16_b64_v4i16((lds_s16x4*)(base + 4 * rowbytes));
+  s16x8_t v = {lo[0], lo[1], lo[2], lo[3], hi[0], hi[1], hi[2], hi[3]};
+  return __builtin_bit_cast(bf16x8_t, v);
+}
+
 typedef __attribute__((address_space(3))) void llx_lds_void;
 __device__ __forceinline__ __amdgpu_buffer_rsrc_t lds_dma_rsrc(const void* base, uint32_t bytes) {
   return __builtin_amdgcn_make_buffer_rsrc(const_cast<void*>(base), 0, (int)bytes, 0x00020000);
diff --git a/llama-x_amd/csrc/gemm_bf16.hip b/llama-x_amd/csrc/gemm_bf16.hip
--- a/llama-x_amd/csrc/gemm_bf16.hip
+++ b/llama-x_amd/csrc/gemm_bf16.hip
@@ -9,24 +9,55 @@
 #define A_TILE_BYTES (256 * BK * 2)
 #define EPI_ROW_BYTES 528
 #define GEMM_LDS_BYTES (256 * EPI_ROW_BYTES)
-
-enum { EPI_NONE = 0, EPI_RESIDUAL = 1, EPI_BIAS = 2, EPI_BIAS_GELU = 3, EPI_COLSCALE = 4, EPI_ROWCOLSCALE = 5, EPI_SWIGLU_BWD = 6, EPI_SWIGLU_FWD = 7, EPI_ROPE = 8, EPI_SPLITK = 9, EPI_ROWCOLSCALE_F32 = 10 };
+#define EPI_TROW_BYTES 80
+#define GEMM_LDS_BYTES_T (GEMM_LDS_BYTES + 256 * EPI_TROW_BYTES)
+
+enum { EPI_NONE = 0, EPI_RESIDUAL = 1, EPI_BIAS = 2, EPI_BIAS_GELU = 3, EPI_COLSCALE = 4, EPI_ROWCOLSCALE = 5, EPI_SWIGLU_BWD = 6, EPI_SWIGLU_FWD = 7, EPI_ROPE = 8, EPI_SPLITK = 9, EPI_ROWCOLSCALE_F32 = 10, EPI_SWIGLU_FWD_T = 11, EPI_SWIGLU_BWD_T = 12 };
 
 struct GemmArgs {
   const bf16_t* A; const bf16_t* B; bf16_t* C;
   const bf16_t* A2; const bf16_t* B2;
   const bf16_t* E;
-  const bf16_t* E2;
+  union {
+    const bf16_t* E2;
+    const bf16_t* TA;
+    const bf16_t* T13;
+  };
   int64_t lda, ldb, ldc, lde, lda2, ldb2;
   int M, N, K, K2;
   int grid_m, grid_n;
   int col0, col_end;
-  const bf16_t* sa; const bf16_t* sb;
-  const float* rope;
-  int rope_S, rope_cols;
+  union {
+    const bf16_t* sa;
+    const bf16_t* BT;
+  };
+  union {
+    const bf16_t* sb;
+    float* upart;
+  };
+  union {
+    const float* rope;
+    int64_t ldta;
+  };
+  union {
+    int rope_S;
+    int r1;
+  };
+  union {
+    int r3;
+    int rope_cols;
+    int tr;
+  };
   const int* m_valid;
-  float* C32;
-  int splits;
+  union {
+    float* C32;
+    float* tpart;
+    float* wpart;
+  };
+  union {
+    int splits;
+    int slot0;
+  };
 };
 
 typedef __attribute__((address_space(3))) void lds_void;
@@ -38,7 +69,8 @@
 __global__ __launch_bounds__(512, 2) void gemm_nt_kernel(const GemmArgs g) {
   static_assert(BNT == 256 || BNT == 128, "tile width");
   static_assert(PIPE == 1, "the four-phase main loop is the only one");
-  static_assert(BNT == 256 || EPI != EPI_SWIGLU_FWD, "the SwiGLU-forward epilogue needs the full tile");
+  static_assert(BNT == 256 || (EPI != EPI_SWIGLU_FWD && EPI != EPI_SWIGLU_FWD_T), "the SwiGLU-forward epilogues need the full tile");
+  static_assert(!I8 || EPI != EPI_SWIGLU_FWD_T, "the h . A^T partials ride in the bf16 kernel only");
   constexpr int ESZ = I8 ? 1 : 2;
   constexpr int TK = 128 / ESZ;
   constexpr int WNG = BNT / 64;
@@ -71,7 +103,11 @@
   const int gsz = min(grid_m - group * GROUP_M, GROUP_M);
   const int pid_m = group * GROUP_M + ((bid % width) % gsz);
   const int pid_n = (bid % width) / gsz;
-  constexpr bool SPLITN = EPI == EPI_SWIGLU_FWD;
+  constexpr bool SPLITN = EPI == EPI_SWIGLU_FWD || EPI == EPI_SWIGLU_FWD_T;
+  constexpr bool TFUSE = EPI == EPI_SWIGLU_FWD_T;
+  constexpr bool BWD = EPI == EPI_SWIGLU_BWD || EPI == EPI_SWIGLU_BWD_T;
+  constexpr bool TB = EPI == EPI_SWIGLU_BWD_T;
+  static_assert(!I8 || !TB, "the adapter partials ride in the bf16 kernel only");
   const int halfN = g.N >> 1;
   const int m0 = pid_m * BM, n0 = SPLITN ? pid_n * (BN / 2) : g.col0 + pid_n * BNT;
   auto col_of = [&](int nl) { return SPLITN ? (nl < BN / 2 ? n0 + nl : halfN + n0 + nl - BN / 2) : min(n0 + nl, g.col_end - 1); };
@@ -334,9 +370,9 @@
     return;
   }
   constexpr int NIT = BNT / 16;
-  constexpr int EB0 = (EPI == EPI_SWIGLU_BWD || EPI == EPI_ROPE) ? 4 : 8;
+  constexpr int EB0 = (BWD || EPI == EPI_ROPE) ? 4 : 8;
   constexpr int EB = EB0 < NIT / 2 ? EB0 : NIT / 2;
-  constexpr bool AUX = EPI == EPI_RESIDUAL || EPI == EPI_BIAS || EPI == EPI_BIAS_GELU || EPI == EPI_SWIGLU_BWD || EPI == EPI_ROPE || EPI == EPI_COLSCALE;
+  constexpr bool AUX = EPI == EPI_RESIDUAL || EPI == EPI_BIAS || EPI == EPI_BIAS_GELU || BWD || EPI == EPI_ROPE || EPI == EPI_COLSCALE;
   auto load_aux = [&](int it0, u32x4_t (&aux0)[EB], u32x4_t (&aux1)[EB]) {
     if constexpr (AUX) {
 #pragma unroll
@@ -346,7 +382,7 @@
         const int gmc = min(m0 + row, g.M - 1), gnc = min(n0 + cc * 8, g.col_end - 8);
         if constexpr (EPI == EPI_RESIDUAL) {
           aux0[j] = *reinterpret_cast<const u32x4_t*>(g.E + (int64_t)gmc * g.lde + gnc);
-        } else if constexpr (EPI == EPI_SWIGLU_BWD) {
+        } else if constexpr (BWD) {
           aux0[j] = *reinterpret_cast<const u32x4_t*>(g.E + (int64_t)gmc * g.lde + gnc);
           aux1[j] = *reinterpret_cast<const u32x4_t*>(g.E + (int64_t)gmc * g.lde + g.N + gnc);
         } else if constexpr (EPI == EPI_ROPE) {
@@ -361,6 +397,31 @@
   };
   u32x4_t auxA0[EB], auxA1[EB], auxB0[EB], auxB1[EB];
   if constexpr (!SPLITN) load_aux(0, auxA0, auxA1);
+  bf16x8_t taf[4];
+  if constexpr (TFUSE) {
+    const bf16_t* trow = g.TA + (int64_t)min(frow, g.tr - 1) * g.ldta + n0 + 8 * fq;
+#pragma unroll
+    for (int ks = 0; ks < 4; ++ks) taf[ks] = *reinterpret_cast<const bf16x8_t*>(trow + ks * 32);
+  }
+  constexpr int KSB = BNT / 32;
+  char* const sT = smem + GEMM_LDS_BYTES;
+  const int rAll = TB ? g.r1 + g.r3 : 0;
+  auto load_bt = [&](int h, int rb, bf16x8_t (&f)[KSB]) {
+    const bf16_t* brow = g.BT + (int64_t)min(rb * 16 + frow, rAll - 1) * (2 * g.N) + h * g.N;
+#pragma unroll
+    for (int ks = 0; ks < KSB; ++ks) f[ks] = *reinterpret_cast<const bf16x8_t*>(brow + min(n0 + ks * 32 + 8 * fq, g.col_end - 8));
+  };
+  bf16x8_t btf[KSB];
+  if constexpr (TB) {
+#pragma unroll
+    for (int j = 0; j < 2; ++j) {
+      const int q = j * 512 + tid, row = q >> 2, ch = q & 3;
+      u32x4_t v = {0u, 0u, 0u, 0u};
+      if (m0 + row < g.M) v = *reinterpret_cast<const u32x4_t*>(g.T13 + (int64_t)(m0 + row) * 64 + ch * 8);
+      *reinterpret_cast<u32x4_t*>(sT + row * EPI_TROW_BYTES + ch * 16) = v;
+    }
+    load_bt(0, 0, btf);
+  }
   float sbv[4][4], rsv[MI];
   if constexpr (I8) {
     if (g.K2 <= 0) {
@@ -413,11 +474,34 @@
         const u32x4_t uv = *reinterpret_cast<const u32x4_t*>(smem + row * EPI_ROW_BYTES + (cc + 16) * 16);
         *reinterpret_cast<u32x4_t*>(g.C + (int64_t)gm * g.ldc + gn) = gv;
         *reinterpret_cast<u32x4_t*>(g.C + (int64_t)gm * g.ldc + halfN + gn) = uv;
-        *reinterpret_cast<u32x4_t*>(H + (int64_t)gm * g.lde + gn) = swiglu_fwd8(gv, uv);
+        const u32x4_t hv = swiglu_fwd8(gv, uv);
+        *reinterpret_cast<u32x4_t*>(H + (int64_t)gm * g.lde + gn) = hv;
+        if constexpr (TFUSE) *reinterpret_cast<u32x4_t*>(smem + row * EPI_ROW_BYTES + cc * 16) = hv;
+      }
+    }
+    if constexpr (TFUSE) {
+      __syncthreads();
+#pragma unroll
+      for (int rf = 0; rf < 2; ++rf) {
+        const int rl = (wave * 2 + rf) * 16 + frow;
+        const char* hrow = smem + rl * EPI_ROW_BYTES + fq * 16;
+        f32x4_t t0 = {0.f, 0.f, 0.f, 0.f}, t1 = {0.f, 0.f, 0.f, 0.f};
+#pragma unroll
+        for (int ks = 0; ks < 4; ks += 2) {
+          t0 = __builtin_amdgcn_mfma_f32_16x16x32_bf16(taf[ks], *reinterpret_cast<const bf16x8_t*>(hrow + ks * 64), t0, 0, 0, 0);
+          t1 = __builtin_amdgcn_mfma_f32_16x16x32_bf16(taf[ks + 1], *reinterpret_cast<const bf16x8_t*>(hrow + (ks + 1) * 64), t1, 0, 0, 0);
+        }
+        const int gm = m0 + rl;
+        if (gm < g.M) {
+#pragma unroll
+          for (int e = 0; e < 4; ++e)
+            if (fq * 4 + e < g.tr) g.tpart[((int64_t)pid_n * 64 + fq * 4 + e) * g.M + gm] = t0[e] + t1[e];
+        }
       }
     }
     return;
   }
+  u32x4_t ouK[TB ? NIT : 1];
   auto combine = [&](int it0, const u32x4_t (&aux0)[EB], const u32x4_t (&aux1)[EB]) {
 #pragma unroll
     for (int j = 0; j < EB; ++j) {
@@ -441,11 +525,15 @@
             }
             v[e] = pack_bf2(lo, hi);
           }
-        } else if constexpr (EPI == EPI_SWIGLU_BWD) {
+        } else if constexpr (BWD) {
           u32x4_t og, ou;
           swiglu_bwd8(v, aux0[j], aux1[j], og, ou);
           *reinterpret_cast<u32x4_t*>(g.C + (int64_t)gm * g.ldc + g.N + gn) = ou;
           v = og;
+          if constexpr (TB) {
+            ouK[it0 + j] = ou;
+            *reinterpret_cast<u32x4_t*>(smem + row * EROW + cc * 16) = og;
+          }
         } else if constexpr (EPI == EPI_ROPE) {
           if (gn < g.rope_cols) v = rope8(v, __builtin_bit_cast(f32x4_t, aux0[j]), __builtin_bit_cast(f32x4_t, aux1[j]), 1.f);
         } else if constexpr (EPI == EPI_COLSCALE) {
@@ -454,16 +542,92 @@
           for (int e = 0; e < 4; ++e) v[e] = pack_bf2(bflo(v[e]) * bflo(sc[e]), bfhi(v[e]) * bfhi(sc[e]));
         }
         *reinterpret_cast<u32x4_t*>(g.C + (int64_t)gm * g.ldc + gn) = v;
+      } else if constexpr (TB) {
+        ouK[it0 + j] = u32x4_t{0u, 0u, 0u, 0u};
+        *reinterpret_cast<u32x4_t*>(smem + row * EROW + cc * 16) = u32x4_t{0u, 0u, 0u, 0u};
       }
     }
   };
   static_assert((NIT / EB) % 2 == 0, "the batches alternate between two register sets");
+  if constexpr (!TB) {
 #pragma unroll 1
-  for (int it0 = 0; it0 < NIT; it0 += 2 * EB) {
-    load_aux(it0 + EB, auxB0, auxB1);
-    combine(it0, auxA0, auxA1);
-    if (it0 + 2 * EB < NIT) load_aux(it0 + 2 * EB, auxA0, auxA1);
-    combine(it0 + EB, auxB0, auxB1);
+    for (int it0 = 0; it0 < NIT; it0 += 2 * EB) {
+      load_aux(it0 + EB, auxB0, auxB1);
+      combine(it0, auxA0, auxA1);
+      if (it0 + 2 * EB < NIT) load_aux(it0 + 2 * EB, auxA0, auxA1);
+      combine(it0 + EB, auxB0, auxB1);
+    }
+  } else {
+#pragma unroll
+    for (int it0 = 0; it0 < NIT; it0 += 2 * EB) {
+      load_aux(it0 + EB, auxB0, auxB1);
+      combine(it0, auxA0, auxA1);
+      if (it0 + 2 * EB < NIT) load_aux(it0 + 2 * EB, auxA0, auxA1);
+      combine(it0 + EB, auxB0, auxB1);
+    }
+    constexpr int CBW = BNT / 128;
+    const int nbl16 = ((rAll + 15) >> 4) * 16;
+    f32x4_t uacc[2][2];
+#pragma unroll
+    for (int rb = 0; rb < 2; ++rb)
+#pragma unroll
+      for (int rf = 0; rf < 2; ++rf) uacc[rb][rf] = f32x4_t{0.f, 0.f, 0.f, 0.f};
+#pragma unroll
+    for (int h = 0; h < 2; ++h) {
+      const int rlo = h ? g.r1 : 0, rhi = h ? rAll : g.r1;
+      if (h == 1) {
+        load_bt(1, rlo >> 4, btf);
+        __syncthreads();
+#pragma unroll
+        for (int it = 0; it < NIT; ++it) {
+          const int q = it * 512 + tid;
+          *reinterpret_cast<u32x4_t*>(smem + (q / (BNT / 8)) * EROW + (q % (BNT / 8)) * 16) = ouK[it];
+        }
+      }
+      __syncthreads();
+#pragma unroll
+      for (int rb = 0; rb < 2; ++rb) {
+        if (rb * 16 < rhi && rb * 16 + 16 > rlo) {
+          if (rb != (rlo >> 4)) load_bt(h, rb, btf);
+#pragma unroll
+          for (int ks = 0; ks < KSB; ++ks)
+#pragma unroll
+            for (int rf = 0; rf < 2; ++rf) {
+              const char* yrow = smem + ((wave * 2 + rf) * 16 + frow) * EROW + fq * 16;
+              uacc[rb][rf] = __builtin_amdgcn_mfma_f32_16x16x32_bf16(btf[ks], *reinterpret_cast<const bf16x8_t*>(yrow + ks * 64), uacc[rb][rf], 0, 0, 0);
+            }
+          f32x4_t bacc[CBW];
+#pragma unroll
+          for (int c = 0; c < CBW; ++c) bacc[c] = f32x4_t{0.f, 0.f, 0.f, 0.f};
+#pragma unroll
+          for (int ks = 0; ks < 8; ++ks) {
+            const bf16x8_t a = tr16_frag(sT + ks * 32 * EPI_TROW_BYTES, EPI_TROW_BYTES, rb * 16, lane);
+#pragma unroll
+            for (int c = 0; c < CBW; ++c)
+              bacc[c] = __builtin_amdgcn_mfma_f32_16x16x32_bf16(a, tr16_frag(smem + ks * 32 * EROW, EROW, (wave * CBW + c) * 16, lane), bacc[c], 0, 0, 0);
+          }
+#pragma unroll
+          for (int c = 0; c < CBW; ++c) {
+            const int gn = n0 + (wave * CBW + c) * 16 + frow;
+            if (gn < g.col_end) {
+#pragma unroll
+              for (int e = 0; e < 4; ++e) g.wpart[((int64_t)pid_m * nbl16 + rb * 16 + fq * 4 + e) * (2 * g.N) + h * g.N + gn] = bacc[c][e];
+            }
+          }
+        }
+      }
+    }
+#pragma unroll
+    for (int rb = 0; rb < 2; ++rb)
+#pragma unroll
+      for (int rf = 0; rf < 2; ++rf) {
+        const int gm = m0 + (wave * 2 + rf) * 16 + frow;
+        if (gm < g.M) {
+#pragma unroll
+          for (int e = 0; e < 4; ++e)
+            if (rb * 16 + fq * 4 + e < rAll) g.upart[((int64_t)(g.slot0 + pid_n) * 64 + rb * 16 + fq * 4 + e) * g.M + gm] = uacc[rb][rf][e];
+        }
+      }
   }
 }
 
@@ -472,19 +636,20 @@
   auto kern = gemm_nt_kernel<EPI, I8, 1, BNT>;
   static std::once_flag attr_once;
   static hipError_t attr_err = hipSuccess;
-  std::call_once(attr_once, [&] { attr_err = hipFuncSetAttribute((const void*)kern, hipFuncAttributeMaxDynamicSharedMemorySize, GEMM_LDS_BYTES); });
+  constexpr int lds_bytes = EPI == EPI_SWIGLU_BWD_T ? GEMM_LDS_BYTES_T : GEMM_LDS_BYTES;
+  std::call_once(attr_once, [&] { attr_err = hipFuncSetAttribute((const void*)kern, hipFuncAttributeMaxDynamicSharedMemorySize, lds_bytes); });
   if (attr_err != hipSuccess) {
     llx_set_error("llx_gemm_nt_bf16: cannot raise dynamic LDS limit: %s", hipGetErrorString(attr_err));
     return LLX_ERR_LAUNCH;
   }
-  hipLaunchKernelGGL(kern, dim3(a.grid_m * a.grid_n * (EPI == EPI_SPLITK ? a.splits : 1)), dim3(512), GEMM_LDS_BYTES, stream, a);
+  hipLaunchKernelGGL(kern, dim3(a.grid_m * a.grid_n * (EPI == EPI_SPLITK ? a.splits : 1)), dim3(512), lds_bytes, stream, a);
   LLX_LAUNCH_CHECK("llx_gemm_nt_bf16");
   return LLX_OK;
 }
 
 template <int EPI, bool I8 = false>
 static int launch_gemm(const GemmArgs& a, hipStream_t stream) {
-  if constexpr (EPI != EPI_SWIGLU_FWD) {
+  if constexpr (EPI != EPI_SWIGLU_FWD && EPI != EPI_SWIGLU_FWD_T) {
     const int tiles = a.grid_m * a.grid_n, tail = tiles % 256;
     if (a.col0 == 0 && a.col_end == a.N && a.N % 256 == 0 && tiles > 256 && tail > 0 && tail <= 128 && tail % a.grid_m == 0) {
       const int tail_cols = tail / a.grid_m * 256;
@@ -493,6 +658,7 @@
       full.grid_n = a.grid_n - tail / a.grid_m;
       half.col0 = a.N - tail_cols;
       half.grid_n = tail_cols / 128;
+      if constexpr (EPI == EPI_SWIGLU_BWD_T) half.slot0 = full.grid_n;
       const int rc = launch_gemm_p<EPI, I8, 256>(full, stream);
       if (rc != LLX_OK) return rc;
       return launch_gemm_p<EPI, I8, 128>(half, stream);
@@ -518,10 +684,20 @@
   return LLX_OK;
 }
 
+struct AdapterEpi { const void* TA; int64_t ldta, TR; float* tpart; const void* T13; const void* BT; int64_t R1, R3; float* upart; float* wpart; };
+
+static int64_t gemm_column_tiles(int64_t M, int64_t N) {
+  const int64_t gm = cdiv64(M, BM), gn = cdiv64(N, BN), tiles = gm * gn, tail = tiles % 256;
+  if (N % 256 == 0 && tiles > 256 && tail > 0 && tail <= 128 && tail % gm == 0) return gn + tail / gm;
+  return gn;
+}
+extern "C" int64_t llx_gemm_swiglu_bwd_t_upart_bytes(int64_t M, int64_t N) { return gemm_column_tiles(M, N) * 64 * M * 4; }
+extern "C" int64_t llx_gemm_swiglu_bwd_t_wpart_bytes(int64_t M, int64_t N, int64_t R) { return cdiv64(M, BM) * cdiv64(R, 16) * 16 * 2 * N * 4; }
+
 static int gemm_nt_bf16_impl(const void* A, int64_t lda, const void* B, int64_t ldb, void* C, int64_t ldc, int64_t M,
                              int64_t N, int64_t K, const void* A2, int64_t lda2, const void* B2, int64_t ldb2, int64_t K2,
                              int epilogue, const void* E, int64_t lde, const float* rope, int64_t rope_S, int64_t rope_cols,
-                             hipStream_t stream, const int32_t* m_valid = nullptr) {
+                             hipStream_t stream, const int32_t* m_valid = nullptr, const AdapterEpi* ad = nullptr) {
   LLX_REQUIRE(A && B && C, "llx_gemm_nt_bf16: null pointer");
   LLX_REQUIRE(M > 0 && N > 0 && K > 0, "llx_gemm_nt_bf16: empty problem M=%lld N=%lld K=%lld", (long long)M, (long long)N, (long long)K);
   LLX_REQUIRE(K % BK == 0 && K2 % BK == 0, "llx_gemm_nt_bf16: K=%lld and K2=%lld must be multiples of 64", (long long)K, (long long)K2);
@@ -533,7 +709,7 @@
   LLX_REQUIRE(epilogue == EPI_NONE || epilogue == EPI_ROPE || (E && (uintptr_t)E % 16 == 0), "llx_gemm_nt_bf16: epilogue operand missing/unaligned");
   LLX_REQUIRE(epilogue != EPI_ROPE || (rope && (uintptr_t)rope % 16 == 0 && rope_S > 0 && rope_cols >= 0 && rope_cols <= N && rope_cols % 128 == 0),
               "llx_gemm_nt_bf16_rope: need an aligned fp32 table, rope_S > 0 and rope_cols a multiple of 128 within N");
-  LLX_REQUIRE((epilogue != EPI_RESIDUAL && epilogue != EPI_SWIGLU_BWD) || lde % 8 == 0, "llx_gemm_nt_bf16: residual / gate|up stride must be a multiple of 8");
+  LLX_REQUIRE((epilogue != EPI_RESIDUAL && epilogue != EPI_SWIGLU_BWD && epilogue != EPI_SWIGLU_BWD_T) || lde % 8 == 0, "llx_gemm_nt_bf16: residual / gate|up stride must be a multiple of 8");
   LLX_REQUIRE(epilogue != EPI_SWIGLU_BWD || (lde >= 2 * N && ldc >= 2 * N), "llx_gemm_nt_bf16: the SwiGLU-backward epilogue reads E[M,2N] (gate|up) and writes C[M,2N] (dg|du)");
   if (const int rc = check_extent("llx_gemm_nt_bf16", M, N, K, lda, ldb, 2); rc != LLX_OK) return rc;
   GemmArgs a = make_args(A, lda, B, ldb, C, ldc, M, N, K);
@@ -553,6 +729,22 @@
       LLX_REQUIRE(N % 256 == 0 && lde % 8 == 0, "llx_gemm_nt_bf16: the SwiGLU-forward epilogue needs N = 2I with I a multiple of 128");
       a.grid_n = (int)(N / 256);
       return launch_gemm<EPI_SWIGLU_FWD>(a, stream);
+    case EPI_SWIGLU_FWD_T:
+      LLX_REQUIRE(N % 256 == 0 && lde % 8 == 0, "llx_gemm_nt_bf16_swiglu_t: the SwiGLU-forward epilogue needs N = 2I with I a multiple of 128");
+      LLX_REQUIRE(ad && ad->TA && ad->tpart && ad->TR >= 1 && ad->TR <= 16 && ad->ldta >= N / 2 && ad->ldta % 8 == 0 && (uintptr_t)ad->TA % 16 == 0 &&
+                      (uintptr_t)ad->tpart % 4 == 0,
+                  "llx_gemm_nt_bf16_swiglu_t: need lora_a [R <= 16, N/2] with an aligned row stride and the partial buffer");
+      a.grid_n = (int)(N / 256);
+      a.TA = (const bf16_t*)ad->TA; a.ldta = ad->ldta; a.tr = (int)ad->TR; a.tpart = ad->tpart;
+      return launch_gemm<EPI_SWIGLU_FWD_T>(a, stream);
+    case EPI_SWIGLU_BWD_T:
+      LLX_REQUIRE(lde % 8 == 0 && lde >= 2 * N && ldc >= 2 * N, "llx_gemm_nt_bf16_swiglu_bwd_t: E[M,2N] (gate|up) and C[M,2N] (dg|du)");
+      LLX_REQUIRE(ad && ad->T13 && ad->BT && ad->upart && ad->wpart && ad->R1 >= 1 && ad->R1 <= 16 && ad->R3 >= 1 && ad->R3 <= 16,
+                  "llx_gemm_nt_bf16_swiglu_bwd_t: need t, B^T, both partial buffers and ranks 1..16");
+      LLX_REQUIRE(((uintptr_t)ad->T13 | (uintptr_t)ad->BT | (uintptr_t)ad->upart | (uintptr_t)ad->wpart) % 16 == 0, "llx_gemm_nt_bf16_swiglu_bwd_t: unaligned pointer");
+      a.T13 = (const bf16_t*)ad->T13; a.BT = (const bf16_t*)ad->BT; a.upart = ad->upart; a.wpart = ad->wpart;
+      a.r1 = (int)ad->R1; a.r3 = (int)ad->R3; a.slot0 = 0;
+      return launch_gemm<EPI_SWIGLU_BWD_T>(a, stream);
     default: llx_set_error("llx_gemm_nt_bf16: unknown epilogue %d", epilogue); return LLX_ERR_UNSUPPORTED;
   }
 }
@@ -561,7 +753,25 @@
                                 int64_t N, int64_t K, const void* A2, int64_t lda2, const void* B2, int64_t ldb2, int64_t K2,
                                 int epilogue, const void* E, int64_t lde, hipStream_t stream) {
   LLX_REQUIRE(epilogue != EPI_ROPE, "llx_gemm_nt_bf16: the RoPE epilogue is llx_gemm_nt_bf16_rope");
+  LLX_REQUIRE(epilogue != EPI_SWIGLU_FWD_T && epilogue != EPI_SWIGLU_BWD_T, "llx_gemm_nt_bf16: epilogues 11 / 12 are llx_gemm_nt_bf16_swiglu_t / _swiglu_bwd_t");
   return gemm_nt_bf16_impl(A, lda, B, ldb, C, ldc, M, N, K, A2, lda2, B2, ldb2, K2, epilogue, E, lde, nullptr, 0, 0, stream);
+}
+
+extern "C" int llx_gemm_nt_bf16_swiglu_t(const void* A, int64_t lda, const void* B, int64_t ldb, void* C, int64_t ldc, int64_t M, int64_t N,
+                                         int64_t K, const void* A2, int64_t lda2, const void* B2, int64_t ldb2, int64_t K2, void* H, int64_t ldh,
+                                         const void* TA, int64_t ldta, int64_t R, float* tpart, hipStream_t stream) {
+  AdapterEpi ad = {};
+  ad.TA = TA; ad.ldta = ldta; ad.TR = R; ad.tpart = tpart;
+  return gemm_nt_bf16_impl(A, lda, B, ldb, C, ldc, M, N, K, A2, lda2, B2, ldb2, K2, EPI_SWIGLU_FWD_T, H, ldh, nullptr, 0, 0, stream, nullptr, &ad);
+}
+
+extern "C" int llx_gemm_nt_bf16_swiglu_bwd_t(const void* A, int64_t lda, const void* B, int64_t ldb, void* C, int64_t ldc, int64_t M, int64_t N,
+                                             int64_t K, const void* A2, int64_t lda2, const void* B2, int64_t ldb2, int64_t K2, const void* E,
+                                             int64_t lde, const void* T13, const void* BT, int64_t R1, int64_t R3, float* upart, float* wpart,
+                                             hipStream_t stream) {
+  AdapterEpi ad = {};
+  ad.T13 = T13; ad.BT = BT; ad.R1 = R1; ad.R3 = R3; ad.upart = upart; ad.wpart = wpart;
+  return gemm_nt_bf16_impl(A, lda, B, ldb, C, ldc, M, N, K, A2, lda2, B2, ldb2, K2, EPI_SWIGLU_BWD_T, E, lde, nullptr, 0, 0, stream, nullptr, &ad);
 }
 
 extern "C" int llx_gemm_nt_bf16_rows(const void* A, int64_t lda, const void* B, int64_t ldb, void* C, int64_t ldc, int64_t M,
diff --git a/llama-x_amd/csrc/skinny.hip b/llama-x_amd/csrc/skinny.hip
--- a/llama-x_amd/csrc/skinny.hip
+++ b/llama-x_amd/csrc/skinny.hip
@@ -1,7 +1,5 @@
 #include "common.h"
 
-typedef __attribute__((address_space(3))) s16x4_t lds_s16x4;
-typedef __attribute__((ext_vector_type(8))) short s16x8_t;
 
 #define SK_PAD 64
 
@@ -157,15 +155,6 @@
 #define TN_MS 32
 #define TN_YROW (TN_NT * 2 + 16)
 #define TN_UROW (SK_PAD * 2 + 16)
-
-__device__ __forceinline__ bf16x8_t tr16_frag(const char* tile, int rowbytes, int c0, int lane) {
-  const int g = lane >> 4, i = lane & 15, q = i >> 2, p = i & 3;
-  const char* base = tile + (8 * g + q) * rowbytes + (c0 + 4 * p) * 2;
-  s16x4_t lo = __builtin_amdgcn_ds_read_tr16_b64_v4i16((lds_s16x4*)base);
-  s16x4_t hi = __builtin_amdgcn_ds_read_tr16_b64_v4i16((lds_s16x4*)(base + 4 * rowbytes));
-  s16x8_t v = {lo[0], lo[1], lo[2], lo[3], hi[0], hi[1], hi[2], hi[3]};
-  return __builtin_bit_cast(bf16x8_t, v);
-}
 
 struct TnSegs { int n_lo[4], n_hi[4], r_lo[4], r_hi[4]; int64_t off[4]; int count; int rb_lo[4], rb_hi[4]; };
 
@@ -509,9 +498,10 @@
   *dst = f2bf(sum);
 }
 
-extern "C" int llx_skinny_tn_reduce_many(int n, const void* const* workspaces, void* const* outs, const int64_t* out_ld, const int64_t* M,
-                                         const int64_t* N, const int64_t* R, const float* scale, const int* transpose_out, const int* accumulate,
-                                         const int32_t* const* segs, const int* seg_count, hipStream_t stream) {
+extern "C" int llx_skinny_tn_reduce_many_splits(int n, const void* const* workspaces, void* const* outs, const int64_t* out_ld, const int64_t* M,
+                                                const int64_t* N, const int64_t* R, const float* scale, const int* transpose_out,
+                                                const int* accumulate, const int32_t* const* segs, const int* seg_count, const int* nsplit,
+                                                hipStream_t stream) {
   LLX_REQUIRE(n >= 1 && n <= TN_MANY && workspaces && outs && out_ld && M && N && R && scale && transpose_out && accumulate && segs && seg_count,
               "llx_skinny_tn_reduce_many: bad arguments (1..4 products)");
   TnRedMany m;
@@ -520,7 +510,7 @@
     TnRed& d = m.d[i];
     LLX_REQUIRE(workspaces[i] && outs[i] && M[i] > 0 && N[i] > 0 && R[i] > 0 && R[i] <= 64, "llx_skinny_tn_reduce_many: bad product %d", i);
     d.partial = (const float*)workspaces[i]; d.out = (bf16_t*)outs[i]; d.out_ld = out_ld[i];
-    d.nsplit = tn_splits(M[i], N[i]); d.RP = (int)cdiv64(R[i], 16) * 16; d.R = (int)R[i]; d.N = (int)N[i];
+    d.nsplit = (nsplit && nsplit[i] > 0) ? nsplit[i] : tn_splits(M[i], N[i]); d.RP = (int)cdiv64(R[i], 16) * 16; d.R = (int)R[i]; d.N = (int)N[i];
     d.transpose_out = transpose_out[i]; d.accumulate = accumulate[i]; d.scale = scale[i];
     d.use_segs = segs[i] != nullptr;
     int64_t total = 0;
@@ -532,6 +522,12 @@
   hipLaunchKernelGGL(skinny_tn_reduce_many_kernel, dim3((unsigned)cdiv64(most, 256), (unsigned)n), dim3(256), 0, stream, m);
   LLX_LAUNCH_CHECK("llx_skinny_tn_reduce_many");
   return LLX_OK;
+}
+
+extern "C" int llx_skinny_tn_reduce_many(int n, const void* const* workspaces, void* const* outs, const int64_t* out_ld, const int64_t* M,
+                                         const int64_t* N, const int64_t* R, const float* scale, const int* transpose_out, const int* accumulate,
+                                         const int32_t* const* segs, const int* seg_count, hipStream_t stream) {
+  return llx_skinny_tn_reduce_many_splits(n, workspaces, outs, out_ld, M, N, R, scale, transpose_out, accumulate, segs, seg_count, nullptr, stream);
 }
 
 extern "C" int llx_skinny_tn(const void* U, const void* Y, int64_t ldy, void* out, int64_t out_ld, int64_t M, int64_t N, int64_t R,
diff --git a/llama-x_amd/llx/_lib.py b/llama-x_amd/llx/_lib.py
--- a/llama-x_amd/llx/_lib.py
+++ b/llama-x_amd/llx/_lib.py
@@ -109,6 +109,11 @@
     "llx_skinny_tn_partial_many_us": (c_int, [_I, _P, _P, _P, _P, _P, _P, _P, _P, _P, _P, _P, _P, _P, _P, _P, _P]),
     "llx_skinny_tn_reduce_many": (c_int, [_I, _P, _P, _P, _P, _P, _P, _P, _P, _P, _P, _P, _P]),
     "llx_gemm_nt_bf16": (c_int, [_P, _L, _P, _L, _P, _L, _L, _L, _L, _P, _L, _P, _L, _L, _I, _P, _L, _P]),
+    "llx_gemm_nt_bf16_swiglu_t": (c_int, [_P, _L, _P, _L, _P, _L, _L, _L, _L, _P, _L, _P, _L, _L, _P, _L, _P, _L, _L, _P, _P]),
+    "llx_gemm_swiglu_bwd_t_upart_bytes": (_L, [_L, _L]),
+    "llx_gemm_swiglu_bwd_t_wpart_bytes": (_L, [_L, _L, _L]),
+    "llx_gemm_nt_bf16_swiglu_bwd_t": (c_int, [_P, _L, _P, _L, _P, _L, _L, _L, _L, _P, _L, _P, _L, _L, _P, _L, _P, _P, _L, _L, _P, _P, _P]),
+    "llx_skinny_tn_reduce_many_splits": (c_int, [_I, _P, _P, _P, _P, _P, _P, _P, _P, _P, _P, _P, _P, _P]),
     "llx_gemm_nt_bf16_splitk": (c_int, [_P, _L, _P, _L, _P, _L, _L, _L, _I, _P, _P]),
     "llx_splitk_combine": (c_int, [_P, _I, _L, _L, _P, _P, _P, _L, _P]),
     "llx_gemm_nt_bf16_rows": (c_int, [_P, _L, _P, _L, _P, _L, _L, _L, _L, _P, _L, _P, _L, _L, _I, _P, _L, _P, _P]),
diff --git a/llama-x_amd/llx/kernels.py b/llama-x_amd/llx/kernels.py
--- a/llama-x_amd/llx/kernels.py
+++ b/llama-x_amd/llx/kernels.py
@@ -15,6 +15,8 @@
 EPI_NONE, EPI_RESIDUAL, EPI_BIAS, EPI_BIAS_GELU, EPI_COLSCALE = 0, 1, 2, 3, 4
 EPI_SWIGLU_BWD = 6
 EPI_SWIGLU_FWD = 7
+EPI_SWIGLU_BWD_T = 12
+EPI_SWIGLU_FWD_T = 11
 SK_PAD = 64
 GEMM_TRACE = None
 ATTN_TRACE = None
@@ -41,7 +43,7 @@
 def gemm_kernel_launches(M: int, N: int, epilogue: int) -> int:
     gm, gn = -(-M // 256), -(-N // 256)
     tail = (gm * gn) % 256
-    split = epilogue != EPI_SWIGLU_FWD and N % 256 == 0 and gm * gn > 256 and 0 < tail <= 128 and tail % gm == 0
+    split = epilogue not in (EPI_SWIGLU_FWD, EPI_SWIGLU_FWD_T) and N % 256 == 0 and gm * gn > 256 and 0 < tail <= 128 and tail % gm == 0
     return 2 if split else 1
 
 
@@ -118,13 +120,14 @@
 
 def gemm_nt(a: Tensor, b: Tensor, *, out: Optional[Tensor] = None, a2: Optional[Tensor] = None, b2: Optional[Tensor] = None,
             epilogue: int = EPI_NONE, e: Optional[Tensor] = None, rope: Optional[tuple[Tensor, int, int]] = None,
-            k2_eff: Optional[float] = None, m_valid: Optional[Tensor] = None, m_expect: Optional[float] = None) -> Tensor:
+            k2_eff: Optional[float] = None, m_valid: Optional[Tensor] = None, m_expect: Optional[float] = None,
+            ta: Optional[Tensor] = None, tpart: Optional[Tensor] = None, bwd_t: Optional["SwigluBwdT"] = None) -> Tensor:
     _chk_bf16(a, b, a2, b2, e, out)
     assert a.dim() == 2 and b.dim() == 2 and a.shape[1] == b.shape[1], (a.shape, b.shape)
     assert a.stride(1) == 1 and b.stride(1) == 1
     M, K = a.shape
     N = b.shape[0]
-    if epilogue == EPI_SWIGLU_BWD:
+    if epilogue in (EPI_SWIGLU_BWD, EPI_SWIGLU_BWD_T):
         assert out is not None and e is not None and out.shape == (M, 2 * N) and e.shape == (M, 2 * N) and out.stride(1) == 1 and e.stride(1) == 1
     else:
         if out is None:
@@ -139,11 +142,17 @@
     if epilogue == EPI_RESIDUAL:
         assert e is not None and e.shape == (M, N) and e.stride(1) == 1
         lde = e.stride(0)
-    elif epilogue == EPI_SWIGLU_BWD:
+    elif epilogue in (EPI_SWIGLU_BWD, EPI_SWIGLU_BWD_T):
         lde = e.stride(0)
-    elif epilogue == EPI_SWIGLU_FWD:
+        assert (epilogue == EPI_SWIGLU_BWD_T) == (bwd_t is not None) and (bwd_t is None or (rope is None and m_valid is None))
+    elif epilogue in (EPI_SWIGLU_FWD, EPI_SWIGLU_FWD_T):
         assert e is not None and N % 256 == 0 and e.shape == (M, N // 2) and e.stride(1) == 1
         lde = e.stride(0)
+        if epilogue == EPI_SWIGLU_FWD_T:
+            assert rope is None and m_valid is None and ta is not None and tpart is not None
+            _chk_bf16(ta)
+            assert ta.dim() == 2 and 1 <= ta.shape[0] <= 16 and ta.shape[1] == N // 2 and ta.stride(1) == 1
+            assert tpart.dtype is torch.float32 and tpart.is_contiguous() and tpart.numel() * 4 >= _lib().llx_skinny_u_workspace_bytes(M, N)
     elif epilogue != EPI_NONE:
         assert e is not None and e.shape == (N,) and e.is_contiguous()
     ev = _trace_begin(GEMM_TRACE)
@@ -158,6 +167,16 @@
         L.check(_lib().llx_gemm_nt_bf16_rows(L.ptr(a), a.stride(0), L.ptr(b), b.stride(0), L.ptr(out), out.stride(0), M, N, K,
                                              L.ptr(a2), a2.stride(0) if a2 is not None else 0, L.ptr(b2), b2.stride(0) if b2 is not None else 0, K2,
                                              epilogue, L.ptr(e), lde, L.ptr(m_valid), L.stream()), "llx_gemm_nt_bf16_rows")
+    elif epilogue == EPI_SWIGLU_BWD_T:
+        assert bwd_t.M == M and bwd_t.N == N
+        L.check(_lib().llx_gemm_nt_bf16_swiglu_bwd_t(L.ptr(a), a.stride(0), L.ptr(b), b.stride(0), L.ptr(out), out.stride(0), M, N, K,
+                                                     L.ptr(a2), a2.stride(0) if a2 is not None else 0, L.ptr(b2), b2.stride(0) if b2 is not None else 0, K2,
+                                                     L.ptr(e), lde, L.ptr(bwd_t.t), L.ptr(bwd_t.bT), bwd_t.r1, bwd_t.r3, L.ptr(bwd_t.upart), L.ptr(bwd_t.ws),
+                                                     L.stream()), "llx_gemm_nt_bf16_swiglu_bwd_t")
+    elif epilogue == EPI_SWIGLU_FWD_T:
+        L.check(_lib().llx_gemm_nt_bf16_swiglu_t(L.ptr(a), a.stride(0), L.ptr(b), b.stride(0), L.ptr(out), out.stride(0), M, N, K,
+                                                 L.ptr(a2), a2.stride(0) if a2 is not None else 0, L.ptr(b2), b2.stride(0) if b2 is not None else 0, K2,
+                                                 L.ptr(e), lde, L.ptr(ta), ta.stride(0), ta.shape[0], L.ptr(tpart), L.stream()), "llx_gemm_nt_bf16_swiglu_t")
     else:
         L.check(_lib().llx_gemm_nt_bf16(L.ptr(a), a.stride(0), L.ptr(b), b.stride(0), L.ptr(out), out.stride(0), M, N, K,
                                         L.ptr(a2), a2.stride(0) if a2 is not None else 0, L.ptr(b2), b2.stride(0) if b2 is not None else 0, K2,
@@ -166,7 +185,7 @@
         kk = K + (K2 if k2_eff is None else min(float(k2_eff), K2))
         Mw = M if m_expect is None else float(m_expect)
         _trace_end(GEMM_TRACE, ev, 2.0 * Mw * N * kk, 2.0 * (Mw * kk + N * kk + Mw * N * (2 if epilogue == EPI_RESIDUAL else 1)), "bf16",
-                   gemm_kernel_launches(M, N, 8 if rope is not None else epilogue))
+                   gemm_kernel_launches(M, N, 8 if rope is not None else (EPI_SWIGLU_BWD if epilogue == EPI_SWIGLU_BWD_T else epilogue)))
     return out
 
 
@@ -1205,6 +1224,7 @@
     segs: Optional[ctypes.Array]
     n_segs: int
     upart: Optional[Tensor] = None
+    nsplit: int = 0
 
 
 def skinny_tn(u: Tensor, y: Tensor, R: int, scale_: float, out: Tensor, transpose_out: bool, accumulate: bool = False,
@@ -1257,6 +1277,59 @@
     return out
 
 
+@dataclass
+class SwigluBwdT:
+    t: Tensor
+    bT: Tensor
+    r1: int
+    r3: int
+    M: int
+    N: int
+    upart: Tensor
+    ws: Tensor
+
+
+def swiglu_bwd_t_operands(t: Tensor, bT: Tensor, r1: int, r3: int, M: int, N: int) -> SwigluBwdT:
+    _chk_bf16(t, bT)
+    assert 1 <= r1 <= 16 and 1 <= r3 <= 16 and t.shape == (M, SK_PAD) and t.is_contiguous() and bT.shape == (r1 + r3, 2 * N) and bT.is_contiguous()
+    upart = torch.empty(_lib().llx_gemm_swiglu_bwd_t_upart_bytes(M, N) // 4, device=t.device, dtype=torch.float32)
+    ws = torch.empty(_lib().llx_gemm_swiglu_bwd_t_wpart_bytes(M, N, r1 + r3), device=t.device, dtype=torch.uint8)
+    return SwigluBwdT(t, bT, r1, r3, M, N, upart, ws)
+
+
+def swiglu_bwd_t_u(op: SwigluBwdT) -> Tensor:
+    out = torch.empty(op.M, SK_PAD, device=op.upart.device, dtype=BF16)
+    tiles = op.upart.numel() // (64 * op.M)
+    L.check(_lib().llx_skinny_u_reduce(L.ptr(op.upart), L.ptr(out), op.M, 256 * tiles, op.r1 + op.r3, None, 0, L.stream()), "llx_skinny_u_reduce")
+    return out
+
+
+def swiglu_bwd_t_queue(op: SwigluBwdT, scale_: float, out: Tensor, transpose_out: bool, segs: Optional[Sequence[tuple[int, int, int, int]]],
+                       pending: list) -> None:
+    sp, ns = None, 0
+    R = op.r1 + op.r3
+    if segs is not None:
+        ns = len(segs)
+        assert 1 <= ns <= 4 and out.is_contiguous() and out.numel() == sum((b - a) * (d - c) for a, b, c, d in segs)
+        sp = (ctypes.c_int32 * (4 * ns))(*[int(v) for sgm in segs for v in sgm])
+    else:
+        assert out.shape == ((2 * op.N, R) if transpose_out else (R, 2 * op.N))
+    pending.append(TnQueued(op.ws, out, out.stride(0) if out.dim() == 2 else 0, op.M, 2 * op.N, R, scale_, int(transpose_out), 0, sp, ns,
+                            nsplit=-(-op.M // 256)))
+    if len(pending) == 4:
+        skinny_tn_flush(pending)
+
+
+def swiglu_t_workspace(M: int, N: int, device) -> Tensor:
+    return torch.empty(_lib().llx_skinny_u_workspace_bytes(M, N) // 4, device=device, dtype=torch.float32)
+
+
+def swiglu_t_reduce(tpart: Tensor, M: int, N: int, R: int) -> Tensor:
+    out = torch.empty(M, SK_PAD, device=tpart.device, dtype=BF16)
+    L.check(_lib().llx_skinny_u_reduce(L.ptr(tpart), L.ptr(out), M, N, R, None, 0, L.stream()), "llx_skinny_u_reduce")
+    return out
+
+
 def skinny_tn_flush(pending: list) -> None:
     while pending:
         chunk, pending[:] = pending[:4], pending[4:]
@@ -1272,4 +1345,5 @@
         AC = (ctypes.c_int * n)(*[q.accumulate for q in chunk])
         SG = (ctypes.c_void_p * n)(*[ctypes.cast(q.segs, ctypes.c_void_p).value if q.segs is not None else None for q in chunk])
         NS = (ctypes.c_int * n)(*[q.n_segs for q in chunk])
-        L.check(_lib().llx_skinny_tn_reduce_many(n, WS, OUT, LD, MM, NN, RR, SC, TR, AC, SG, NS, L.stream()), "llx_skinny_tn_reduce_many")
+        SP = (ctypes.c_int * n)(*[q.nsplit for q in chunk])
+        L.check(_lib().llx_skinny_tn_reduce_many_splits(n, WS, OUT, LD, MM, NN, RR, SC, TR, AC, SG, NS, SP, L.stream()), "llx_skinny_tn_reduce_many")
diff --git a/llama-x_amd/llx/ops.py b/llama-x_amd/llx/ops.py
--- a/llama-x_amd/llx/ops.py
+++ b/llama-x_amd/llx/ops.py
@@ -239,10 +239,10 @@
 
     def forward(self, x: Tensor, out: Optional[Tensor] = None, residual: Optional[Tensor] = None, swiglu_h: Optional[Tensor] = None,
                 rope: Optional[tuple[Tensor, int, int]] = None, xq: Optional[tuple[Tensor, Tensor]] = None, t_pre: Optional[Tensor] = None,
-                cached_scale: bool = False):
+                cached_scale: bool = False, swiglu_t: Optional[tuple[Tensor, Tensor]] = None):
         if out is None:
             out = torch.empty(x.shape[0], self.N, device=x.device, dtype=BF16)
-        return out, self._forward(x, out, residual, swiglu_h, rope, xq, t_pre, cached_scale)
+        return out, self._forward(x, out, residual, swiglu_h, rope, xq, t_pre, cached_scale, swiglu_t)
 
     def norm_can_make_t(self, dim: int) -> bool:
         return self.fused and self.R > 0 and self.packed is not None and K.rmsnorm_skinny_ok(dim)
@@ -256,9 +256,22 @@
     def swiglu_fusable(self) -> bool:
         return self.fused and (not self.int8 or self.dynamic) and not self.dora and len(self.members) == 2 and self.Ns[0] % 128 == 0
 
+    def swiglu_t_fusable(self, consumer: "GroupPlan") -> bool:
+        return (self.swiglu_fusable() and not self.int8 and consumer.fused and not consumer.int8 and not consumer.dora
+                and len(consumer.members) == 1 and 0 < consumer.R <= 16 and consumer.K == self.Ns[0]
+                and consumer.members[0].lora_a.is_contiguous())
+
+    def swiglu_bwd_t_fusable(self, needs: Sequence[bool]) -> bool:
+        if not (self.fused and not self.int8 and not self.dora and len(self.members) == 2 and all(0 < r <= 16 for r in self.ranks)
+                and self.Ns[0] == self.Ns[1] and self.Ns[0] % 256 == 0 and self._tn_segs() is not None):
+            return False
+        ni = iter(needs)
+        need = [[next(ni) for _ in m.tensors()] for m in self.members]
+        return any(nd[-1] for nd in need)
+
     def _forward(self, x: Tensor, out: Tensor, residual: Optional[Tensor], swiglu_h: Optional[Tensor] = None,
                  rope: Optional[tuple[Tensor, int, int]] = None, xq: Optional[tuple[Tensor, Tensor]] = None, t_pre: Optional[Tensor] = None,
-                 cached_scale: bool = False):
+                 cached_scale: bool = False, swiglu_t: Optional[tuple[Tensor, Tensor]] = None):
         if not self.fused:
             assert residual is None or len(self.members) == 1
             return [m.forward(x, out=out[:, o : o + n], residual=residual, cached_scale=cached_scale)[1]
@@ -279,6 +292,9 @@
         if not self.int8:
             if residual is not None:
                 K.gemm_nt(x, self.w_cat(), out=out, a2=t[0] if t else None, b2=b2, epilogue=K.EPI_RESIDUAL, e=residual, k2_eff=self.k2_fwd)
+            elif swiglu_t is not None:
+                K.gemm_nt(x, self.w_cat(), out=out, a2=t[0] if t else None, b2=b2, epilogue=K.EPI_SWIGLU_FWD_T, e=swiglu_h, k2_eff=self.k2_fwd,
+                          ta=swiglu_t[0], tpart=swiglu_t[1])
             elif swiglu_h is not None:
                 K.gemm_nt(x, self.w_cat(), out=out, a2=t[0] if t else None, b2=b2, epilogue=K.EPI_SWIGLU_FWD, e=swiglu_h, k2_eff=self.k2_fwd)
             else:
@@ -330,7 +346,7 @@
         return self._kr or None
 
     def backward(self, dy: Tensor, x: Tensor, saved, needs: Sequence[bool], need_dx: bool, dx_out: Optional[Tensor] = None,
-                 swiglu: Optional[tuple[Tensor, Tensor]] = None, pending: Optional[list] = None):
+                 swiglu: Optional[tuple[Tensor, Tensor]] = None, pending: Optional[list] = None, swiglu_t=None, first_stage=None):
         if not self.fused:
             grads, dx, first = [], None, True
             ni = 0
@@ -371,8 +387,12 @@
                 if self.int8 and need_dx:
                     g_scaled = torch.empty_like(dy)
                     sc = (self.scale_cat(), g_scaled)
-                K.skinny_tn(t, dy, self.R, self.scale, flat, transpose_out=True, segs=segs, pending=pending, u_from=bT, scaled=sc)
-                u = K.skinny_u_reduce(pending[-1])
+                if first_stage is not None:
+                    u = K.swiglu_bwd_t_u(first_stage)
+                    K.swiglu_bwd_t_queue(first_stage, self.scale, flat, True, segs, pending)
+                else:
+                    K.skinny_tn(t, dy, self.R, self.scale, flat, transpose_out=True, segs=segs, pending=pending, u_from=bT, scaled=sc)
+                    u = K.skinny_u_reduce(pending[-1])
                 gB_views, off = [], 0
                 for m_, (a, b, c_, d) in zip([m for m in self.members if m.rank > 0], segs):
                     gB_views.append(flat[off : off + (b - a) * (d - c_)].view(b - a, d - c_))
@@ -399,7 +419,8 @@
             else:
                 g = dy
             if swiglu is not None:
-                dx = K.gemm_nt(g, self.wt_cat(), out=swiglu[1], a2=u, b2=a2t if self.R > 0 else None, epilogue=K.EPI_SWIGLU_BWD, e=swiglu[0], k2_eff=self.R)
+                dx = K.gemm_nt(g, self.wt_cat(), out=swiglu[1], a2=u, b2=a2t if self.R > 0 else None, e=swiglu[0], k2_eff=self.R,
+                               epilogue=K.EPI_SWIGLU_BWD if swiglu_t is None else K.EPI_SWIGLU_BWD_T, bwd_t=swiglu_t)
             else:
                 dx = K.gemm_nt(g, self.wt_cat(), out=dx_out, a2=u, b2=a2t if self.R > 0 else None, k2_eff=self.R)
         grads: list[Optional[Tensor]] = []
@@ -678,13 +699,20 @@
         T, I = x2.shape[0], meta.w13.Ns[0]
         gu = torch.empty(T, 2 * I, device=x.device, dtype=BF16)
         infer = meta.no_grad or not any(ctx.needs_input_grad)
-        if meta.w13.swiglu_fusable():
+        t2_pre = None
+        if meta.w13.swiglu_t_fusable(meta.w2):
+            h = torch.empty(T, I, device=x.device, dtype=BF16)
+            a2 = meta.w2.packed[0] if meta.w2.packed is not None else meta.w2.members[0].lora_a.detach()
+            tpart = K.swiglu_t_workspace(T, 2 * I, x.device)
+            _, t13 = meta.w13.forward(xn, gu, swiglu_h=h, xq=xq, t_pre=t_pre, cached_scale=infer, swiglu_t=(a2, tpart))
+            t2_pre = K.swiglu_t_reduce(tpart, T, 2 * I, meta.w2.R)
+        elif meta.w13.swiglu_fusable():
             h = torch.empty(T, I, device=x.device, dtype=BF16)
             _, t13 = meta.w13.forward(xn, gu, swiglu_h=h, xq=xq, t_pre=t_pre, cached_scale=infer)
         else:
             _, t13 = meta.w13.forward(xn, gu, xq=xq, t_pre=t_pre, cached_scale=infer)
             h = K.swiglu_fwd(gu[:, :I], gu[:, I:])
-        y, t2 = meta.w2.forward(h, None, x2 if meta.fuse_residual else None, cached_scale=infer)
+        y, t2 = meta.w2.forward(h, None, x2 if meta.fuse_residual else None, t_pre=t2_pre, cached_scale=infer)
         ctx.meta = meta
         _save(ctx, x, norm_w, x2, xn if meta.fuse_norm else None, rstd, gu, h, t13, t2)
         return y.view(shape)
@@ -702,15 +730,18 @@
         n13, n2 = needs[:n_13], needs[n_13:]
         dgu = torch.empty(T, 2 * I, device=x.device, dtype=BF16)
         pend = []
+        first13 = None
+        if meta.w2.fused and not meta.w2.int8 and meta.w13.swiglu_bwd_t_fusable(n13):
+            first13 = K.swiglu_bwd_t_operands(t13[0], t13[1], meta.w13.ranks[0], meta.w13.ranks[1], T, I)
         if meta.w2.fused:
-            _, g_2 = meta.w2.backward(dy2, h, t2, n2, True, swiglu=(gu, dgu), pending=pend)
+            _, g_2 = meta.w2.backward(dy2, h, t2, n2, True, swiglu=(gu, dgu), pending=pend, swiglu_t=first13)
         else:
             dh, g_2 = meta.w2.backward(dy2, h, t2, n2, True)
             K.swiglu_bwd(dh, gu[:, :I], gu[:, I:], dgu[:, :I], dgu[:, I:])
         need_dx = ctx.needs_input_grad[0]
         need_dxn = need_dx or (meta.fuse_norm and ctx.needs_input_grad[1])
         dxn = torch.empty_like(x2) if need_dxn else None
-        _, g_13 = meta.w13.backward(dgu, xn, t13, n13, need_dxn, dxn, pending=pend)
+        _, g_13 = meta.w13.backward(dgu, xn, t13, n13, need_dxn, dxn, pending=pend, first_stage=first13)
         K.skinny_tn_flush(pend)
         dx, dnw = _norm_epilogue(dxn, x2, norm_w, rstd, ctx.needs_input_grad[1], dy2 if (need_dx and meta.fuse_residual) else None, meta.fuse_norm)
         return (dx.view(x.shape) if (dx is not None and need_dx) else None, dnw, None, *g_13, *g_2)
```

Result: no change. 32640 tokens/s, median of 6 (+0.6%).
